# Megvii-CSG/MegReader

Measured on AMD Instinct MI355X. Metric: training images/sec, CRNN-CTC 32x128 crops, batch 256 per GPU, higher is better.
Workload: dtype bf16; 1 GPU; CRNN + 1D-CTC training step (BASELINE.json configs[1]): 32x128 crops, T=33, C=38, Adam; global_batch=256, per_gpu_batch=256, parallelism=dp1, launch=hipGraph replay

## Files before the change

### include/megreader_hip.h

```cpp
#ifndef MEGREADER_HIP_H
#define MEGREADER_HIP_H

#include <hip/hip_runtime_api.h>

#ifdef __cplusplus
extern "C" {
#endif

#define MR_ABI_VERSION 3
#define MR_DTYPE_F32 0
#define MR_DTYPE_BF16 1

const char* mr_last_error(void);
int mr_abi_version(void);
int mr_phase_timer(int on);
int mr_phase_read(int id, double* total_ms, double* total_work);
int mr_init(void);

typedef struct mr_tuning {
  int nt_variant;
  int nt_deep;
  int nt_big;
  int nt_p8;
  int nt_force_bm;
  int nt_force_bn;
  int gemm_skinny;
  int tn_big;
  int tn_buf;
  int tn_taps;
  int tn_taps_group;
  int tn_group;
  int tn_fin;
  int tn_taps_fin;
  int tn_taps_w8;
  int tn_model;
  int tn_splits;
  int bn_fused;
  int lstm_persist;
  int lstm_fwd_bn;
  int lstm_bwd_bn;
  int dcn_fused;
  int dcn_v1_bwd;
  int bn_onepass;
  int skinny_depth;
  int nt_big_min_k;
  int tn_taps_min_p;
  int tn_defer;
  int pool_fixed;
  int ctc_linear;
  int nt_wide8;
  int nt_ksplit;
  int nt_m32;
  int nt_m32_opt;
  int dcn_gcol;
  int dcn_col_fwd;
  int decode_persist;
  int reserved[3];
} mr_tuning;
int mr_tuning_get(mr_tuning* out);
int mr_tuning_defaults(mr_tuning* out);
int mr_tuning_set(const mr_tuning* in);

int mr_gemm_nt(int dtype, const void* A, long long lda, const void* B, int ldb, void* C, long long ldc,
               const float* bias, int relu, int M, int N, int K, hipStream_t stream);
int mr_set_tn_taps_workspace(void* ws, long long bytes);
int mr_tn_taps_would_run(int N, int H, int W, int Cin, int ldx, int Cout, int lddy, int R, int S, int sh, int sw,
                         int ph, int pw, int dh, int dw, int Ho, int Wo);
int mr_nt_tile_code(int M, int N);
int mr_nt_kernel_code(int dtype, int M, int N, int K, int cg);
int mr_gemm_tn(int dtype, const void* A, long long lda, const void* B, long long ldb, float* C, int ldc, int P,
               int NA, int NB, int row_perm_h, float* colsum, hipStream_t stream);
int mr_gemm_tn2(int dtype, const void* A, long long lda, const void* B, long long ldb, float* C, int ldc, int P,
                int NA, int NB, int row_perm_h, float* colsum, float* colsum2, hipStream_t stream);

int mr_tn_defer(int on);
int mr_tn_pending(void);
int mr_tn_discard(void);
int mr_tn_flush(hipStream_t stream);
int mr_tn_flush_beside(hipStream_t stream);

int mr_conv2d_fwd(int dtype, const void* x, const void* w_krsc, const float* bias, void* y, int relu, int Nimg,
                  int H, int W, int Cin, int ldx, int Cout, int ldy, int R, int S, int sh, int sw, int ph, int pw,
                  int dh, int dw, int Ho, int Wo, hipStream_t stream);
int mr_conv2d_fwd_pool_ok(int dtype, int Nimg, int H, int W, int Cin, int ldx, int Cout, int R, int S, int sh, int sw, int ph, int pw,
                          int dh, int dw, int Ho, int Wo, int pkh, int pkw, int psh, int psw, int pph, int ppw);
int mr_conv2d_fwd_pool(int dtype, const void* x, const void* w_krsc, const float* bias, void* y_pool, unsigned char* idx, int relu,
                       int Nimg, int H, int W, int Cin, int ldx, int Cout, int R, int S, int sh, int sw, int ph, int pw, int dh,
                       int dw, int Ho, int Wo, int pkh, int pkw, int psh, int psw, int pph, int ppw, int PHo, int PWo,
                       hipStream_t stream);
int mr_conv2d_fwd_stats(int dtype, const void* x, const void* w_krsc, const float* bias, void* y, double* bn_sums, int Nimg,
                        int H, int W, int Cin, int ldx, int Cout, int R, int S, int sh, int sw, int ph, int pw, int dh,
                        int dw, int Ho, int Wo, hipStream_t stream);
int mr_conv2d_dgrad(int dtype, const void* dy, const void* w_crsk, void* dx, int Nimg, int H, int W, int Cin,
                    int lddx, int Cout, int lddy, int R, int S, int sh, int sw, int ph, int pw, int dh, int dw,
                    int Ho, int Wo, hipStream_t stream);
int mr_conv2d_dgrad_add(int dtype, const void* dy, const void* w_crsk, void* dx, const void* addend, int Nimg, int H, int W,
                        int Cin, int lddx, int Cout, int lddy, int R, int S, int sh, int sw, int ph, int pw, int dh, int dw,
                        int Ho, int Wo, hipStream_t stream);
int mr_conv2d_dgrad_bnb(int dtype, const void* dy, const void* w_crsk, void* dx, const void* addend, const void* bn_x,
                        const void* bn_y, const float* bn_mean, const float* bn_rstd, double* bn_sums, int* produced,
                        int Nimg, int H, int W, int Cin, int lddx, int Cout, int lddy, int R, int S, int sh, int sw, int ph,
                        int pw, int dh, int dw, int Ho, int Wo, hipStream_t stream);
int mr_conv2d_wgrad(int dtype, const void* dy, const void* x, float* dw_krsc, float* dbias, int Nimg, int H, int W,
                    int Cin, int ldx, int Cout, int lddy, int R, int S, int sh, int sw, int ph, int pw, int dh,
                    int dw, int Ho, int Wo, hipStream_t stream);
int mr_conv2d_wgrad_tab(int dtype, const void* dy, const void* x, float* dw_krsc, float* dbias, int N, int H, int W,
                        int Cin, int ldx, int Cout, int lddy, int R, int S, int sh, int sw, int ph, int pw, int dh,
                        int dw, int Ho, int Wo, void* rowtab, int build, hipStream_t stream);

long long mr_db_loss_ws_bytes(void);
int mr_db_head_tail_fwd(int dtype, const void* xb, const void* xt, float* binary, float* thresh, float* tbinary, long long n,
                        float k, hipStream_t stream);
int mr_db_head_tail_bwd(int dtype, const float* binary, const float* thresh, const float* tbinary, const float* gb,
                        const float* gt, const float* gtb, void* dxb, void* dxt, long long n, float k, hipStream_t stream);
int mr_db_loss_fwd(const float* binary, const float* thresh, const float* tbinary, const float* gt, const float* mask,
                   const float* tmap, const float* tmask, float* negloss, void* ws, float* out, int N, long long HW,
                   float negative_ratio, float eps, float l1_scale, float bce_scale, hipStream_t stream);
int mr_db_loss_bwd(const float* binary, const float* thresh, const float* tbinary, const float* gt, const float* mask,
                   const float* tmap, const float* tmask, const float* out, const float* gloss, float* g_binary,
                   float* g_thresh, float* g_tbinary, int N, long long HW, float l1_scale, float bce_scale,
                   hipStream_t stream);

int mr_nchw_to_nhwc(int dtype, const float* src, void* dst, int N, int C, int H, int W, int Cpad,
                    hipStream_t stream);
int mr_nhwc_to_nchw(int dtype, const void* src, float* dst, int N, int C, int H, int W, int ld, hipStream_t stream);
int mr_cast(int src_dtype, const void* src, int dst_dtype, void* dst, long long n, hipStream_t stream);
int mr_relu_bwd(int dtype, const void* dy, const void* y, void* dx, long long n, hipStream_t stream);
int mr_add(int dtype, const void* a, const void* b, void* out, long long n, int relu, hipStream_t stream);
int mr_colsum(int dtype, const void* x, float* out, int P, int C, long long ld, int perm_h, hipStream_t stream);
int mr_permute_021(int dtype, const void* src, void* dst, int A, int B, int C, hipStream_t stream);
int mr_prep_conv_weight(int dtype, const float* src, long long sk, long long sc, long long sr, long long ss,
                        void* dst_krsc, void* dst_crsk, int K, int C, int R, int S, int Cpad, int ldk,
                        hipStream_t stream);
int mr_prep_matrix(int dtype, const float* src, int lds, void* dst_n, int ldn, void* dst_t, int ldt, int R, int C,
                   int perm_h, hipStream_t stream);
int mr_prep_bias(const float* a, const float* b, float* dst, int R, int perm_h, hipStream_t stream);

#define MR_PREP_CONV 0
#define MR_PREP_MATRIX 1
#define MR_PREP_BIAS 2
#define MR_PREP_STEM 3
typedef struct mr_prep_job {
  const float* src;
  const float* src2;
  void* dst_a;
  void* dst_b;
  long long s0, s1, s2, s3;
  int kind;
  int d0, d1, d2, d3;
  int pad, ld_b, perm_h;
  int block_start, reserved;
} mr_prep_job;
int mr_prep_batch(int dtype, const mr_prep_job* jobs_device, int njobs, long long total_blocks, float* tick,
                  hipStream_t stream);
int mr_sizeof_prep_job(void);

#define MR_MAX_SEGMENTS 8
int mr_accumulate_multi(int count, float* const* dst, const float* const* src, const long long* n,
                        hipStream_t stream);
int mr_zero_multi(int count, void* const* dst, const long long* bytes, hipStream_t stream);

int mr_opt_tick(float* hyper, hipStream_t stream);
int mr_adam_step(float* p, const float* g, float* m, float* v, long long n, float* hyper, hipStream_t stream);
int mr_sgd_step(float* p, const float* g, float* buf, long long n, float* hyper, hipStream_t stream);

long long mr_bn_scratch_doubles(int C);
int mr_bn_fwd_train(int dtype, const void* x, void* y, const float* gamma, const float* beta, float* running_mean,
                    float* running_var, float* save_mean, float* save_rstd, double* sums, const void* residual,
                    int relu, long long P, int C, float eps, float momentum, long long* num_batches_tracked,
                    hipStream_t stream);
int mr_bn_stats(int dtype, const void* x, double* sums, long long P, int C, hipStream_t stream);
int mr_bn_fwd_eval(int dtype, const void* x, void* y, const float* gamma, const float* beta,
                   const float* running_mean, const float* running_var, float* tmp_mean, float* tmp_rstd,
                   const void* residual, int relu, long long P, int C, float eps, hipStream_t stream);
int mr_bn_bwd(int dtype, const void* dy, const void* x, const void* y, const float* gamma, const float* save_mean,
              const float* save_rstd, double* sums, void* dx, void* dres, float* dgamma, float* dbeta, int flags,
              long long P, int C, hipStream_t stream);
int mr_maxpool_fwd(int dtype, const void* x, void* y, unsigned char* idx, int N, int H, int W, int C, int kh,
                   int kw, int sh, int sw, int ph, int pw, int Ho, int Wo, hipStream_t stream);
int mr_maxpool_bwd(int dtype, const void* dy, const unsigned char* idx, const void* relu_y, void* dx, int N, int H,
                   int W, int C, int kh, int kw, int sh, int sw, int ph, int pw, int Ho, int Wo,
                   hipStream_t stream);

long long mr_stem_bwd_workspace(int Cin);
int mr_stem_pack(const float* w, long long wsk, long long wsc, long long wsr, long long wss, void* wpack, int Cin,
                 hipStream_t stream);
int mr_stem_fwd(int dtype, const float* x, const float* w, long long wsk, long long wsc, long long wsr,
                long long wss, const void* wpack, const float* bias, void* y, unsigned char* code, int N, int Cin,
                int H, int W, hipStream_t stream);
int mr_stem_bwd(int dtype, const void* dy, const unsigned char* code, const float* x, float* workspace, float* dw,
                long long dsk, long long dsc, long long dsr, long long dss, float* dbias, int N, int Cin, int H,
                int W, hipStream_t stream);

int mr_lstm_fwd(int dtype, const void* xproj, const void* whh, void* out, float* cbuf, void* gates, int T, int N,
                int H, void* ws, long long ws_bytes, hipStream_t stream);
int mr_lstm_bwd(int dtype, const void* dout, const void* whhT, const float* cbuf, void* gates, float* dc, int T,
                int N, int H, void* ws, long long ws_bytes, hipStream_t stream);
long long mr_lstm_ws_bytes(int dtype, int T, int N, int H);
int mr_lstm_debug_buffer(float* p);

int mr_ctc_fwd(int dtype, const void* logits, int ldl, const void* targets, int targets_i64,
               const void* input_lengths, const void* target_lengths, int lengths_i64, int T, int N, int C, int S,
               int blank, int zero_infinity, float* log_probs, double* alpha, double* beta, double* nll,
               double* loss, double* log_probs_f64, hipStream_t stream);
int mr_ctc_bwd(int dtype, const float* log_probs, const double* alpha, const double* beta, const double* nll,
               const void* targets, int targets_i64, const void* input_lengths, const void* target_lengths,
               int lengths_i64, const double* grad_out, int T, int N, int C, int S, int blank, int zero_infinity,
               void* grad_logits, int ldg, hipStream_t stream);
int mr_ctc_wide(int C, int S);

int mr_ctc2d_fwd(int dtype, const void* log_probs, const long long* targets, const long long* input_lengths,
                 const long long* target_lengths, int T, int H, int N, int C, int S, int blank, float* nll,
                 float* alpha, hipStream_t stream);
int mr_ctc2d_bwd(int dtype, const float* grad_out, const void* log_probs, const long long* targets,
                 const long long* input_lengths, const long long* target_lengths, const float* nll,
                 const float* alpha, float* beta, void* grad, int T, int H, int N, int C, int S, int blank,
                 hipStream_t stream);

int mr_adaptive_avgpool_fwd(int dtype, const void* x, void* y, int N, int H, int W, int C, int OH, int OW,
                            hipStream_t stream);
int mr_adaptive_avgpool_bwd(int dtype, const void* dy, void* dx, int N, int H, int W, int C, int OH, int OW,
                            hipStream_t stream);
int mr_adaptive_avgpool_multi_fwd(int dtype, const void* x, void* const* ys, const int* oh, const int* ow, int nscales, int N,
                                  int H, int W, int C, hipStream_t stream);
int mr_adaptive_avgpool_multi_bwd(int dtype, void* const* dys, const int* oh, const int* ow, int nscales, void* dx, int N, int H,
                                  int W, int C, hipStream_t stream);
int mr_bilinear_fwd(int dtype, const void* x, void* y, int N, int H, int W, int C, int OH, int OW, int ldy, int coff,
                    int accumulate, hipStream_t stream);
int mr_bilinear_bwd(int dtype, const void* dy, void* dx, int N, int H, int W, int C, int OH, int OW, int lddy,
                    int coff, hipStream_t stream);
int mr_nearest_up_fwd(int dtype, const void* x, const void* add, void* y, int N, int H, int W, int C, int s, int ldy,
                      int coff, hipStream_t stream);
int mr_nearest_up_bwd(int dtype, const void* dy, void* dx, int N, int H, int W, int C, int s, int lddy, int coff,
                      hipStream_t stream);
int mr_deconv2x2_d2s(int dtype, const void* y2, int ld2, const float* bias, void* y, int N, int H, int W, int C,
                     hipStream_t stream);
int mr_deconv2x2_s2d(int dtype, const void* dy, void* dy2, int ld2, int N, int H, int W, int C, hipStream_t stream);
int mr_copy_channels(int dtype, const void* src, int lds, int soff, void* dst, int ldd, int doff, long long P, int C,
                     hipStream_t stream);
int mr_scatter_strided(int dtype, const void* dxs, void* dx, int N, int H, int W, int C, int sh, int sw, int Ho, int Wo,
                       hipStream_t stream);
int mr_scale_channels(int dtype, const void* x, const float* scale, void* y, int N, long long HW, int C,
                      hipStream_t stream);
int mr_ctc2d_head_fwd(int dtype, const void* mask_logits, int lda, const void* cls_logits, int ldz, float* lp,
                      float* mask_prob, float* cls_prob, int N, int H, int W, int C, float tiny, hipStream_t stream);
int mr_ctc2d_head_bwd(int dtype, const float* grad_lp, const float* mask_prob, const float* cls_prob, void* dmask,
                      int ldda, void* dcls, int lddz, int N, int H, int W, int C, float tiny, hipStream_t stream);

int mr_dcn2_im2col(int dtype, const void* x, const float* offset, long long off_bs, const float* mask,
                   long long msk_bs, void* col, int N, int H, int W, int C, int kh, int kw, int stride, int pad,
                   int dil, int Ho, int Wo, hipStream_t stream);
int mr_dcn2_coord_grad(int dtype, const void* gcol, const void* x, const float* offset, long long off_bs,
                       const float* mask, long long msk_bs, float* doffset, float* dmask, int N, int H, int W,
                       int C, int kh, int kw, int stride, int pad, int dil, int Ho, int Wo, hipStream_t stream);
int mr_dcn2_col2im(int dtype, const void* gcol, const float* offset, long long off_bs, const float* mask,
                   long long msk_bs, float* dx, int N, int H, int W, int C, int kh, int kw, int stride, int pad,
                   int dil, int Ho, int Wo, hipStream_t stream);

long long mr_dcn2_ws_bytes(int dtype, int N, int H, int W, int C, int Co, int kh, int kw, int Ho, int Wo, int backward);
int mr_dcn2_fwd(int dtype, const void* x, const void* w_n, const float* bias, const float* offset, long long off_bs,
                const float* mask, long long msk_bs, void* y, void* col_ws, int N, int H, int W, int C, int Co, int kh,
                int kw, int stride, int pad, int dil, int Ho, int Wo, hipStream_t stream);
int mr_dcn2_bwd(int dtype, const void* dy, const void* x, const void* w_t, const float* offset, long long off_bs,
                const float* mask, long long msk_bs, void* col_ws, float* dx32, float* doffset, float* dmask, float* dw,
                float* dbias, int N, int H, int W, int C, int Co, int kh, int kw, int stride, int pad, int dil, int Ho,
                int Wo, hipStream_t stream);
int mr_dcn2_fused(int dtype, int H, int W, int C, int Co, int kh, int kw);
int mr_dcn2_dx_direct(int dtype, int N, int H, int W, int C, int Co, int kh, int kw);
int mr_dcn2_bwd2(int dtype, const void* dy, const void* x, const void* w_t, const float* offset, long long off_bs,
                 const float* mask, long long msk_bs, void* col_ws, float* dx32, void* dx_t, int flags, float* doffset,
                 float* dmask, float* dw, float* dbias, int N, int H, int W, int C, int Co, int kh, int kw, int stride, int pad,
                 int dil, int Ho, int Wo, hipStream_t stream);
int mr_dcn2_col_saved(int dtype, int H, int W, int C, int Co, int kh, int kw);
int mr_dcn2_bwd3(int dtype, const void* dy, const void* x, const void* w_t, const float* offset, long long off_bs,
                 const float* mask, long long msk_bs, void* col_ws, float* dx32, void* dx_t, int flags, float* doffset,
                 float* dmask, float* dw, float* dbias, const void* col_saved, int N, int H, int W, int C, int Co, int kh, int kw,
                 int stride, int pad, int dil, int Ho, int Wo, hipStream_t stream);
int mr_dcn_unpack(int dtype, const void* raw, int ld, float* offset, float* mask, int N, int HW, int n_offset, int n_mask,
                  hipStream_t stream);
int mr_dcn_pack_grad(int dtype, const float* doffset, const float* dmask, const float* mask, void* graw, int ld, int N,
                     int HW, int n_offset, int n_mask, hipStream_t stream);

int mr_deform_psroi_fwd(const float* data, const float* rois, const float* trans, float* out, float* top_count, int B,
                        int C, int H, int W, int R, int channels_trans, int no_trans, float spatial_scale,
                        int output_dim, int group_size, int pooled_size, int part_size, int sample_per_part,
                        float trans_std, hipStream_t stream);
int mr_deform_psroi_bwd(const float* out_grad, const float* data, const float* rois, const float* trans,
                        const float* top_count, float* data_diff, float* trans_diff, int B, int C, int H, int W, int R,
                        int channels_trans, int no_trans, float spatial_scale, int output_dim, int group_size,
                        int pooled_size, int part_size, int sample_per_part, float trans_std, hipStream_t stream);

int mr_db_components(const float* prob, float thresh, int* labels, void* points, int* count, int cap, int N, int H, int W,
                     hipStream_t stream);
int mr_db_box_scores(const float* prob, const float* boxes, float* out, int B, int N, int H, int W, hipStream_t stream);

int mr_attn_step_fwd(int dtype, const void* hproj, const void* eproj, const float* v, const void* enc, float* weights,
                     void* context, int N, int T, int Hd, int Ep, hipStream_t stream);
int mr_attn_step_bwd(int dtype, const void* dcontext, const float* dweights, const void* hproj, const void* eproj,
                     const float* v, const void* enc, const float* weights, void* dhproj, float* deproj, float* dv,
                     float* denc, int N, int T, int Hd, int Ep, hipStream_t stream);
int mr_gru_gates_fwd(int dtype, const void* gi_a, const void* gi_b, const void* gh, const void* h, void* hnew,
                     float* save, int N, int H, hipStream_t stream);
int mr_gru_gates_bwd(int dtype, const void* dhnew, const float* save, const void* gh, const void* h, void* dgi,
                     void* dgh, void* dh, int N, int H, hipStream_t stream);
int mr_nll_step_fwd(int dtype, const void* logits, int ldl, const long long* target, long long tstride,
                    const float* mask, float* lp, float* loss, long long* argmax, int N, int C, int accumulate,
                    int softmax_out, hipStream_t stream);
int mr_nll_step_feed_fwd(int dtype, const void* logits, int ldl, const long long* target, long long tstride,
                         const float* mask, float* lp, float* loss, long long* argmax, const int* feed_flag,
                         long long* feed_idx, int N, int C, int accumulate, hipStream_t stream);
int mr_nll_step_bwd(int dtype, const float* gloss, const float* lp, const long long* target, long long tstride,
                    const float* mask, void* dlogits, int ldd, int N, int C, hipStream_t stream);
int mr_embed_rows_fwd(int dtype, const long long* idx, const float* table, void* out, int N, int V, int D, int ldo,
                      hipStream_t stream);
int mr_embed_rows_bwd(int dtype, const long long* idx, const void* dout, float* dtable, int N, int V, int D, int ldo,
                      hipStream_t stream);
int mr_attn_fwd2(int dtype, const void* hproj, long long ldh, const void* eproj, const float* v, const void* enc,
                 float* weights, void* context, int N, int Tn, int Hd, int Ep, hipStream_t stream);
int mr_attn_bwd2(int dtype, const void* dcontext, const float* dweights, long long ldw, const void* hproj, long long ldh,
                 const void* eproj, const float* v, const void* enc, const float* weights, void* dhproj, long long lddh,
                 float* deproj, float* dv, int N, int Tn, int Hd, int Ep, hipStream_t stream);
int mr_attn_denc(int dtype, const float* weights, const void* dcontext, void* denc, int S, int N, int Tn, int Ep,
                 hipStream_t stream);
int mr_gru_fwd2(int dtype, const void* gi_a, long long lda, const long long* idx, const void* gi_b, const void* gh,
                long long ldgh, const void* h, void* hnew, float* save, int N, int H, hipStream_t stream);
int mr_gru_bwd2(int dtype, const void* dh_a, const void* dh_b, const void* dh_c, const float* save, const void* gh,
                long long ldgh, const void* h, void* dgi, void* dgh, long long lddgh, void* dh_prev, int N, int H,
                hipStream_t stream);
int mr_rows_scatter_add(int dtype, const long long* idx, const void* rows, long long ldr, float* dtable, int R, int V,
                        int D, hipStream_t stream);

int mr_decode_persist_ok(int dtype, int N, int T, int H, int Ep);
long long mr_decode_persist_ws_bytes(int N);
int mr_decode_persist_fwd(const void* cat_w, const float* cat_b, const void* ic_w, long long ldic, const void* G, long long ldG,
                          long long* idx, const int* flags, const void* out_w, const float* out_b, int C, const void* eproj,
                          const void* enc, const float* v, void* H_all, void* HC_all, float* W_att, void* CTX_all,
                          float* SAVE_all, void* ws, long long ws_bytes, int S, int N, int T, int Ep, hipStream_t stream);
int mr_decode_persist_bwd_ok(int dtype, int N, int T, int H, int Ep);
long long mr_decode_persist_bwd_ws_bytes(int N);
int mr_decode_persist_bwd(const void* cat_wt, const void* ic_wt, long long ldict, const void* eproj, const void* enc,
                          const float* v, const void* H_all, const void* HC_all, const float* W_att, const float* SAVE_all,
                          const void* DHO_all, const float* ga, long long ldga, void* DGI_all, void* DHC_all, void* DCTX_all,
                          float* deproj, float* dv, void* denc, void* ws, long long ws_bytes, int S, int N, int T, int Ep,
                          hipStream_t stream);
int mr_decode_greedy_ok(int dtype, int N, int T, int H, int Ep, int C);
int mr_decode_greedy_fwd(const void* cat_w, const float* cat_b, const void* ic_w, long long ldic, const void* G, long long ldG,
                         const void* out_w, const float* out_b, int C, const void* eproj, const void* enc, const float* v,
                         const void* h0, int start_word, int* pred, long long ldp, void* H_all, void* ws, long long ws_bytes,
                         int S, int N, int T, int Ep, hipStream_t stream);
int mr_decode_greedy_trim(int* pred, long long ldp, int N, int S, int blank, hipStream_t stream);

int mr_gemm_gru_fwd(int dtype, const void* ctx, long long ldc, const void* w_ic, long long ldw, const void* G, long long ldG,
                    const long long* idx, const void* gh, long long ldgh, const void* h, void* hnew, float* save, int M, int H,
                    int K, hipStream_t stream);
int mr_gemm_gru_bwd(int dtype, const void* dhc, long long lda, const void* w_t, long long ldw, const void* dh_b,
                    const void* dh_c, const float* save, const void* gh, long long ldgh, const void* h, void* dgi, void* dgh,
                    long long lddgh, void* dh_prev, int M, int H, int K, hipStream_t stream);
int mr_out_nll_fwd(int dtype, const void* h, long long ldh, const void* W, long long ldw, const float* bias,
                   const long long* target, long long tstride, const float* mask, float* lp, float* loss, long long* argmax,
                   const int* feed_flag, long long* feed_idx, int N, int C, int K, int accumulate, hipStream_t stream);

int mr_softmax_nc1t(int dtype, const void* logits, int ldl, float* out, int T, int N, int C, hipStream_t stream);

int mr_ctc_greedy_decode(int dtype, const void* pred, long long sn, long long sc, long long st, int N, int C, int T,
                         int blank, int unknown, int* out, int* out_len, hipStream_t stream);
int mr_ctc2d_greedy_decode(const float* classify, long long cn, long long cc, long long ch, long long cw,
                           const float* mask, long long mn, long long mh, long long mw, int N, int C, int H, int W,
                           int blank, int unknown, int* out, int* out_len, hipStream_t stream);
int mr_seq_measure(const int* labels, int S, const int* preds, int S2, int N, int blank, int unknown, const int* fold,
                   int* acc, int* ed, int* label_len, double* score, hipStream_t stream);

int mr_sizeof_img_desc(void);
int mr_resize_normalize(const unsigned char* src, const void* desc, int N, int H, int W, double mean0, double mean1,
                        double mean2, float* dst, hipStream_t stream);
int mr_encode_labels(const int* codepoints, const long long* offsets, int N, int max_size, const int* table_cp,
                     const int* table_id, int ntab, int unknown, int* label, int* length, hipStream_t stream);

#ifdef __cplusplus
}
#endif
#endif
```

### megreader_amd/backbones/crnn.py

```python
import torch.nn as nn

from ..nn import Conv2d, BatchNorm2d, MaxPool2d, FusedReLU
from ..nn import functional as F


class _Stem(nn.Sequential):

    def forward(self, input):
        conv, pool = self[0][0], self[1]
        if F.stem_eligible(input, conv.weight, conv.stride, conv.padding, conv.dilation, _pair(pool.kernel_size),
                           _pair(pool.stride), _pair(pool.padding)):
            return F.stem_conv_relu_pool(input, conv.weight, conv.bias)
        return super().forward(input)


class _ConvReluPool(nn.Sequential):

    def forward(self, input):
        conv, pool = self[0][0], self[1]
        if F.conv_relu_pool_eligible(input, conv.weight, conv.stride, conv.padding, conv.dilation, _pair(pool.kernel_size),
                                     _pair(pool.stride), _pair(pool.padding)):
            return F.conv_relu_pool(input, conv.weight, conv.bias, conv.padding, _pair(pool.kernel_size), _pair(pool.stride),
                                    _pair(pool.padding))
        return super().forward(input)


def _pair(v):
    return tuple(v) if isinstance(v, (tuple, list)) else (v, v)


class CRNN(nn.Module):

    def __init__(self, imgH, nc, nclass, nh):
        super(CRNN, self).__init__()
        assert imgH % 16 == 0, 'imgH has to be a multiple of 16'

        self.kernels = [3, 3, 3, 3, 3, 3, 2]
        self.paddings = [1, 1, 1, 1, 1, 1, 0]
        self.strides = [1, 1, 1, 1, 1, 1, 1]
        self.channels = [64, 128, 256, 256, 512, 512, 512, nc]

        conv0 = _Stem(self._make_layer(0, pooled=True), MaxPool2d((2, 2), relu_input=True))
        conv1 = _ConvReluPool(self._make_layer(1, pooled=True), MaxPool2d((2, 2), relu_input=True))
        conv2 = self._make_layer(2, True)
        conv3 = _ConvReluPool(self._make_layer(3, pooled=True), MaxPool2d((2, 2), (2, 1), (0, 1), relu_input=True))
        conv4 = self._make_layer(4, True)
        conv5 = _ConvReluPool(self._make_layer(5, pooled=True), MaxPool2d((2, 2), (2, 1), (0, 1), relu_input=True))
        conv6 = self._make_layer(6, True)

        self.cnn = nn.Sequential(conv0, conv1, conv2, conv3, conv4, conv5, conv6)
        conv3[0][0].sole_consumer_of_bn = True
        conv5[0][0].sole_consumer_of_bn = True

    def _make_layer(self, i, batch_normalization=False, pooled=False):
        in_channel = self.channels[i - 1]
        out_channel = self.channels[i]
        layer = list()
        layer.append(Conv2d(in_channel, out_channel, self.kernels[i], self.strides[i], self.paddings[i],
                            fuse_relu=not batch_normalization,
                            relu_grad_downstream=pooled and not batch_normalization))
        if batch_normalization:
            layer.append(BatchNorm2d(out_channel))
        else:
            layer.append(FusedReLU())
        return nn.Sequential(*layer)

    def forward(self, input):
        return self.cnn(input)


def crnn_backbone(imgH=32, nc=3, nclass=37, nh=256):
    return CRNN(imgH, nc, nclass, nh)
```

### megreader_amd/csrc/norm_pool.hip

```cpp
#include "device.h"
#include "../../include/megreader_hip.h"


namespace mr {

template <typename T>
__global__ void bn_stats_kernel(const T* __restrict__ x, double* __restrict__ sums, int P, int C, long long ld,
                                int rows_per_block) {
  __shared__ float red[2][4][64];
  const int lane = threadIdx.x & 63, wave = threadIdx.x >> 6;
  const int c = blockIdx.x * 64 + lane;
  const int p0 = blockIdx.y * rows_per_block;
  const int p1 = min(P, p0 + rows_per_block);
  float s = 0.f, q = 0.f;
  if (c < C)
    for (int p = p0 + wave; p < p1; p += 4) {
      const float v = to_f32(x[(long long)p * ld + c]);
      s += v;
      q += v * v;
    }
  red[0][wave][lane] = s;
  red[1][wave][lane] = q;
  __syncthreads();
  if (wave == 0 && c < C) {
    const double ds = (double)red[0][0][lane] + red[0][1][lane] + red[0][2][lane] + red[0][3][lane];
    const double dq = (double)red[1][0][lane] + red[1][1][lane] + red[1][2][lane] + red[1][3][lane];
    atomicAdd(sums + c, ds);
    atomicAdd(sums + C + c, dq);
  }
}

template <typename T, int MODE>
__global__ __launch_bounds__(256) void bn_reduce_vec_kernel(const T* __restrict__ a, const T* __restrict__ xin,
                                                            const T* __restrict__ yin,
                                                            const float* __restrict__ mean,
                                                            const float* __restrict__ rstd,
                                                            double* __restrict__ sums, int relu, int P, int C,
                                                            int rows_per_block, int ncopy) {
  constexpr int VEC = VecOf<T>::N;
  __shared__ float red[2][256 * VEC];
  sums += (size_t)(blockIdx.x % ncopy) * 2 * C;
  const int cv = C / VEC;
  const int groups = 256 / cv;
  const int g = threadIdx.x / cv, v = threadIdx.x - g * cv;
  const int p0 = blockIdx.x * rows_per_block;
  const int p1 = min(P, p0 + rows_per_block);
  float s[VEC], q[VEC], mu[VEC], rs[VEC];
#pragma unroll
  for (int j = 0; j < VEC; ++j) {
    s[j] = q[j] = 0.f;
    mu[j] = 0.f;
    rs[j] = 1.f;
  }
  if (g < groups) {
    if (MODE == 1) {
#pragma unroll
      for (int j = 0; j < VEC; ++j) {
        mu[j] = mean[v * VEC + j];
        rs[j] = rstd[v * VEC + j];
      }
    }
#pragma unroll 4
    for (int p = p0 + g; p < p1; p += groups) {
      const long long i = (long long)p * cv + v;
      const uint4 av = ((const uint4*)a)[i];
      const T* pa = (const T*)&av;
      if (MODE == 0) {
#pragma unroll
        for (int j = 0; j < VEC; ++j) {
          const float x = to_f32(pa[j]);
          s[j] += x;
          q[j] += x * x;
        }
      } else {
        const uint4 xv = ((const uint4*)xin)[i];
        const T* px = (const T*)&xv;
        uint4 yv = make_uint4(0, 0, 0, 0);
        if (relu) yv = ((const uint4*)yin)[i];
        const T* py = (const T*)&yv;
#pragma unroll
        for (int j = 0; j < VEC; ++j) {
          float gd = to_f32(pa[j]);
          if (relu && !(to_f32(py[j]) > 0.f)) gd = 0.f;
          s[j] += gd;
          q[j] += gd * (to_f32(px[j]) - mu[j]) * rs[j];
        }
      }
    }
#pragma unroll
    for (int j = 0; j < VEC; ++j) {
      red[0][g * C + v * VEC + j] = s[j];
      red[1][g * C + v * VEC + j] = q[j];
    }
  }
  __syncthreads();
  for (int c = threadIdx.x; c < C; c += 256) {
    double ds = 0, dq = 0;
    for (int gg = 0; gg < groups; ++gg) {
      ds += (double)red[0][gg * C + c];
      dq += (double)red[1][gg * C + c];
    }
    atomicAdd(sums + c, ds);
    atomicAdd(sums + C + c, dq);
  }
}

__global__ void bn_finalize_kernel(const double* __restrict__ sums, int ncopy, int P, int C, float eps,
                                   float momentum, float* __restrict__ mean, float* __restrict__ rstd,
                                   float* __restrict__ running_mean, float* __restrict__ running_var,
                                   long long* __restrict__ num_batches_tracked) {
  const int c = blockIdx.x * blockDim.x + threadIdx.x;
  if (c == 0 && num_batches_tracked) *num_batches_tracked += 1;
  if (c >= C) return;
  double s1 = 0, s2 = 0;
  for (int k = 0; k < ncopy; ++k) {
    s1 += sums[(size_t)k * 2 * C + c];
    s2 += sums[(size_t)k * 2 * C + C + c];
  }
  const double m = s1 / P;
  double var = s2 / P - m * m;
  if (var < 0) var = 0;
  mean[c] = (float)m;
  rstd[c] = (float)(1.0 / sqrt(var + (double)eps));
  if (running_mean) {
    const double unb = P > 1 ? var * ((double)P / (P - 1)) : var;
    running_mean[c] = (1.f - momentum) * running_mean[c] + momentum * (float)m;
    running_var[c] = (1.f - momentum) * running_var[c] + momentum * (float)unb;
  }
}

template <typename T>
__global__ void bn_apply_kernel(const T* __restrict__ x, T* __restrict__ y, const float* __restrict__ mean,
                                const float* __restrict__ rstd, const float* __restrict__ gamma,
                                const float* __restrict__ beta, const T* __restrict__ residual, int relu,
                                long long P, int C) {
  constexpr int VEC = VecOf<T>::N;
  const int cv = C / VEC;
  const long long total = P * cv;
  for (long long i = blockIdx.x * (long long)blockDim.x + threadIdx.x; i < total;
       i += (long long)gridDim.x * blockDim.x) {
    const int c0 = (int)(i % cv) * VEC;
    uint4 a = ((const uint4*)x)[i];
    T* pa = (T*)&a;
    uint4 r = make_uint4(0, 0, 0, 0);
    if (residual) r = ((const uint4*)residual)[i];
    const T* pr = (const T*)&r;
#pragma unroll
    for (int j = 0; j < VEC; ++j) {
      const int c = c0 + j;
      float v = (to_f32(pa[j]) - mean[c]) * rstd[c] * gamma[c] + beta[c];
      if (residual) v += to_f32(pr[j]);
      if (relu) v = fmaxf(v, 0.f);
      pa[j] = from_f32<T>(v);
    }
    ((uint4*)y)[i] = a;
  }
}

template <typename T>
__global__ void bn_bwd_reduce_kernel(const T* __restrict__ dy, const T* __restrict__ x, const T* __restrict__ y,
                                     const float* __restrict__ mean, const float* __restrict__ rstd,
                                     double* __restrict__ sums, int relu, int P, int C, int rows_per_block) {
  __shared__ float red[2][4][64];
  const int lane = threadIdx.x & 63, wave = threadIdx.x >> 6;
  const int c = blockIdx.x * 64 + lane;
  const int p0 = blockIdx.y * rows_per_block;
  const int p1 = min(P, p0 + rows_per_block);
  float s = 0.f, q = 0.f;
  if (c < C) {
    const float mu = mean[c], rs = rstd[c];
    for (int p = p0 + wave; p < p1; p += 4) {
      const long long idx = (long long)p * C + c;
      float g = to_f32(dy[idx]);
      if (relu && !(to_f32(y[idx]) > 0.f)) g = 0.f;
      s += g;
      q += g * (to_f32(x[idx]) - mu) * rs;
    }
  }
  red[0][wave][lane] = s;
  red[1][wave][lane] = q;
  __syncthreads();
  if (wave == 0 && c < C) {
    const double ds = (double)red[0][0][lane] + red[0][1][lane] + red[0][2][lane] + red[0][3][lane];
    const double dq = (double)red[1][0][lane] + red[1][1][lane] + red[1][2][lane] + red[1][3][lane];
    atomicAdd(sums + c, ds);
    atomicAdd(sums + C + c, dq);
  }
}

__global__ void bn_bwd_finalize_kernel(const double* __restrict__ sums, int ncopy, long long P, int C,
                                       float* __restrict__ sbg, float* __restrict__ dgamma,
                                       float* __restrict__ dbeta, int accumulate) {
  const int c = blockIdx.x * blockDim.x + threadIdx.x;
  if (c >= C) return;
  double s1 = 0, s2 = 0;
  for (int k = 0; k < ncopy; ++k) {
    s1 += sums[(size_t)k * 2 * C + c];
    s2 += sums[(size_t)k * 2 * C + C + c];
  }
  const float invP = 1.f / (float)P;
  sbg[c] = (float)s1 * invP;
  sbg[C + c] = (float)s2 * invP;
  dbeta[c] = (accumulate ? dbeta[c] : 0.f) + (float)s1;
  dgamma[c] = (accumulate ? dgamma[c] : 0.f) + (float)s2;
}

template <typename T>
__global__ void bn_bwd_apply_kernel(const T* __restrict__ dy, const T* __restrict__ x, const T* __restrict__ y,
                                    const float* __restrict__ mean, const float* __restrict__ rstd,
                                    const float* __restrict__ gamma, const float* __restrict__ sbg,
                                    T* __restrict__ dx, T* __restrict__ dres, int relu, long long P, int C) {
  constexpr int VEC = VecOf<T>::N;
  const int cv = C / VEC;
  const long long total = P * cv;
  for (long long i = blockIdx.x * (long long)blockDim.x + threadIdx.x; i < total;
       i += (long long)gridDim.x * blockDim.x) {
    const int c0 = (int)(i % cv) * VEC;
    uint4 g = ((const uint4*)dy)[i];
    uint4 a = ((const uint4*)x)[i];
    uint4 o = make_uint4(0, 0, 0, 0);
    if (relu) o = ((const uint4*)y)[i];
    T* pg = (T*)&g;
    const T* pa = (const T*)&a;
    const T* po = (const T*)&o;
    uint4 out;
    T* pout = (T*)&out;
#pragma unroll
    for (int j = 0; j < VEC; ++j) {
      const int c = c0 + j;
      float gv = to_f32(pg[j]);
      if (relu && !(to_f32(po[j]) > 0.f)) gv = 0.f;
      pg[j] = from_f32<T>(gv);
      const float xh = (to_f32(pa[j]) - mean[c]) * rstd[c];
      const float sb = sbg[c], sg = sbg[C + c];
      pout[j] = from_f32<T>(gamma[c] * rstd[c] * (gv - sb - xh * sg));
    }
    ((uint4*)dx)[i] = out;
    if (dres) ((uint4*)dres)[i] = g;
  }
}

template <typename T>
__global__ __launch_bounds__(256) void bn_apply_fused_kernel(
    const T* __restrict__ x, T* __restrict__ y, const double* __restrict__ sums, int ncopy, float eps, float momentum,
    float* __restrict__ save_mean, float* __restrict__ save_rstd, float* __restrict__ running_mean,
    float* __restrict__ running_var, long long* __restrict__ num_batches_tracked, const float* __restrict__ gamma,
    const float* __restrict__ beta, const T* __restrict__ residual, int relu, int P, int C) {
  constexpr int VEC = VecOf<T>::N, LANES = 64 / VEC, ROWS = 256 / LANES;
  __shared__ float s_mean[64], s_rstd[64], s_gamma[64], s_beta[64];
  const int cbase = blockIdx.y * 64;
  if (threadIdx.x < 64) {
    const int c = cbase + threadIdx.x;
    double s1 = 0, s2 = 0;
    for (int k = 0; k < ncopy; ++k) {
      s1 += sums[(size_t)k * 2 * C + c];
      s2 += sums[(size_t)k * 2 * C + C + c];
    }
    const double m = s1 / P;
    double var = s2 / P - m * m;
    if (var < 0) var = 0;
    const float mf = (float)m, rf = (float)(1.0 / sqrt(var + (double)eps));
    s_mean[threadIdx.x] = mf;
    s_rstd[threadIdx.x] = rf;
    s_gamma[threadIdx.x] = gamma[c];
    s_beta[threadIdx.x] = beta[c];
    if (blockIdx.x == 0) {
      if (c == 0 && num_batches_tracked) *num_batches_tracked += 1;
      save_mean[c] = mf;
      save_rstd[c] = rf;
      if (running_mean) {
        const double unb = P > 1 ? var * ((double)P / (P - 1)) : var;
        running_mean[c] = (1.f - momentum) * running_mean[c] + momentum * (float)m;
        running_var[c] = (1.f - momentum) * running_var[c] + momentum * (float)unb;
      }
    }
  }
  __syncthreads();
  const int v = threadIdx.x % LANES, r0 = threadIdx.x / LANES;
  const int cv = C / VEC;
  float mu[VEC], rs[VEC], ga[VEC], be[VEC];
#pragma unroll
  for (int j = 0; j < VEC; ++j) {
    mu[j] = s_mean[v * VEC + j];
    rs[j] = s_rstd[v * VEC + j];
    ga[j] = s_gamma[v * VEC + j];
    be[j] = s_beta[v * VEC + j];
  }
  for (int p = blockIdx.x * ROWS + r0; p < P; p += gridDim.x * ROWS) {
    const long long i = (long long)p * cv + blockIdx.y * LANES + v;
    uint4 a = ((const uint4*)x)[i];
    T* pa = (T*)&a;
    uint4 r = make_uint4(0, 0, 0, 0);
    if (residual) r = ((const uint4*)residual)[i];
    const T* pr = (const T*)&r;
#pragma unroll
    for (int j = 0; j < VEC; ++j) {
      float val = (to_f32(pa[j]) - mu[j]) * rs[j] * ga[j] + be[j];
      if (residual) val += to_f32(pr[j]);
      if (relu) val = fmaxf(val, 0.f);
      pa[j] = from_f32<T>(val);
    }
    ((uint4*)y)[i] = a;
  }
}

template <typename T>
__global__ __launch_bounds__(256) void bn_bwd_apply_fused_kernel(
    const T* __restrict__ dy, const T* __restrict__ x, const T* __restrict__ y, const float* __restrict__ mean,
    const float* __restrict__ rstd, const float* __restrict__ gamma, const double* __restrict__ sums, int ncopy,
    float* __restrict__ dgamma, float* __restrict__ dbeta, int accumulate, T* __restrict__ dx, T* __restrict__ dres,
    int relu, int P, int C) {
  constexpr int VEC = VecOf<T>::N, LANES = 64 / VEC, ROWS = 256 / LANES;
  __shared__ float s_mean[64], s_k[64], s_rstd[64], s_sb[64], s_sg[64];
  const int cbase = blockIdx.y * 64;
  if (threadIdx.x < 64) {
    const int c = cbase + threadIdx.x;
    double s1 = 0, s2 = 0;
    for (int k = 0; k < ncopy; ++k) {
      s1 += sums[(size_t)k * 2 * C + c];
      s2 += sums[(size_t)k * 2 * C + C + c];
    }
    const float invP = 1.f / (float)P;
    s_sb[threadIdx.x] = (float)s1 * invP;
    s_sg[threadIdx.x] = (float)s2 * invP;
    s_mean[threadIdx.x] = mean[c];
    s_rstd[threadIdx.x] = rstd[c];
    s_k[threadIdx.x] = gamma[c] * rstd[c];
    if (blockIdx.x == 0) {
      dbeta[c] = (accumulate ? dbeta[c] : 0.f) + (float)s1;
      dgamma[c] = (accumulate ? dgamma[c] : 0.f) + (float)s2;
    }
  }
  __syncthreads();
  const int v = threadIdx.x % LANES, r0 = threadIdx.x / LANES;
  const int cv = C / VEC;
  float mu[VEC], rs[VEC], kk[VEC], sb[VEC], sg[VEC];
#pragma unroll
  for (int j = 0; j < VEC; ++j) {
    mu[j] = s_mean[v * VEC + j];
    rs[j] = s_rstd[v * VEC + j];
    kk[j] = s_k[v * VEC + j];
    sb[j] = s_sb[v * VEC + j];
    sg[j] = s_sg[v * VEC + j];
  }
  for (int p = blockIdx.x * ROWS + r0; p < P; p += gridDim.x * ROWS) {
    const long long i = (long long)p * cv + blockIdx.y * LANES + v;
    uint4 g = ((const uint4*)dy)[i];
    uint4 a = ((const uint4*)x)[i];
    uint4 o = make_uint4(0, 0, 0, 0);
    if (relu) o = ((const uint4*)y)[i];
    T* pg = (T*)&g;
    const T* pa = (const T*)&a;
    const T* po = (const T*)&o;
    uint4 out;
    T* pout = (T*)&out;
#pragma unroll
    for (int j = 0; j < VEC; ++j) {
      float gv = to_f32(pg[j]);
      if (relu && !(to_f32(po[j]) > 0.f)) gv = 0.f;
      pg[j] = from_f32<T>(gv);
      const float xh = (to_f32(pa[j]) - mu[j]) * rs[j];
      pout[j] = from_f32<T>(kk[j] * (gv - sb[j] - xh * sg[j]));
    }
    ((uint4*)dx)[i] = out;
    if (dres) ((uint4*)dres)[i] = g;
  }
}

template <typename T, int R>
__global__ __launch_bounds__(256) void bn_bwd_onepass_kernel(
    const T* __restrict__ dy, const T* __restrict__ x, const T* __restrict__ y, const float* __restrict__ mean,
    const float* __restrict__ rstd, const float* __restrict__ gamma, double* __restrict__ sums, int ncopy,
    unsigned* __restrict__ counters, float* __restrict__ dgamma, float* __restrict__ dbeta, int accumulate,
    T* __restrict__ dx, T* __restrict__ dres, int relu, int P, int C) {
  constexpr int VEC = VecOf<T>::N, LANES = 64 / VEC, ROWS = 256 / LANES;
  typedef __attribute__((ext_vector_type(4))) unsigned u32x4;
  __shared__ float red[2][ROWS][64];
  __shared__ float s_sb[64], s_sg[64];
  __shared__ int s_dead;
  const int tid = threadIdx.x;
  const int cbase = blockIdx.y * 64;
  const int v = tid % LANES, r0 = tid / LANES;
  const int cv = C / VEC;
  const int bytes = (int)((long long)P * C * (long long)sizeof(T));
  const __amdgpu_buffer_rsrc_t r_g = __builtin_amdgcn_make_buffer_rsrc((void*)dy, (short)0, bytes, 0x00020000);
  const __amdgpu_buffer_rsrc_t r_x = __builtin_amdgcn_make_buffer_rsrc((void*)x, (short)0, bytes, 0x00020000);
  const __amdgpu_buffer_rsrc_t r_y = __builtin_amdgcn_make_buffer_rsrc((void*)(relu ? y : x), (short)0, bytes, 0x00020000);
  const __amdgpu_buffer_rsrc_t r_dx = __builtin_amdgcn_make_buffer_rsrc((void*)dx, (short)0, bytes, 0x00020000);
  const __amdgpu_buffer_rsrc_t r_dr = __builtin_amdgcn_make_buffer_rsrc((void*)(dres ? dres : dx), (short)0, bytes, 0x00020000);
  const int voff = (r0 * cv + blockIdx.y * LANES + v) * 16;
  const int row_bytes = cv * 16;
  const int sbase = blockIdx.x * (ROWS * R) * row_bytes;
  float mu[VEC], rs[VEC];
#pragma unroll
  for (int j = 0; j < VEC; ++j) {
    mu[j] = mean[cbase + v * VEC + j];
    rs[j] = rstd[cbase + v * VEC + j];
  }
  u32x4 gq[R], xq[R];
#pragma unroll
  for (int k = 0; k < R; ++k) {
    gq[k] = __builtin_amdgcn_raw_buffer_load_b128(r_g, voff + sbase + k * ROWS * row_bytes, 0, 0);
    xq[k] = __builtin_amdgcn_raw_buffer_load_b128(r_x, voff + sbase + k * ROWS * row_bytes, 0, 0);
  }
  float s[VEC], q[VEC];
#pragma unroll
  for (int j = 0; j < VEC; ++j) s[j] = q[j] = 0.f;
  constexpr int RB = R < 4 ? R : 4;
#pragma unroll
  for (int kb = 0; kb < R; kb += RB) {
    u32x4 yq[RB];
    if (relu) {
#pragma unroll
      for (int u = 0; u < RB; ++u)
        yq[u] = __builtin_amdgcn_raw_buffer_load_b128(r_y, voff + sbase + (kb + u) * ROWS * row_bytes, 0, 0);
    }
#pragma unroll
    for (int u = 0; u < RB; ++u) {
      const int k = kb + u;
      T* pg = (T*)&gq[k];
      const T* pa = (const T*)&xq[k];
      const T* po = (const T*)&yq[u];
#pragma unroll
      for (int j = 0; j < VEC; ++j) {
        float gd = to_f32(pg[j]);
        if (relu && !(to_f32(po[j]) > 0.f)) {
          gd = 0.f;
          pg[j] = from_f32<T>(0.f);
        }
        s[j] += gd;
        q[j] += gd * (to_f32(pa[j]) - mu[j]) * rs[j];
      }
      __builtin_amdgcn_sched_barrier(0);
    }
  }
#pragma unroll
  for (int k = 0; k < R; ++k) asm volatile("" : "+v"(gq[k]), "+v"(xq[k]));
#pragma unroll
  for (int j = 0; j < VEC; ++j) {
    red[0][r0][v * VEC + j] = s[j];
    red[1][r0][v * VEC + j] = q[j];
  }
  if (tid == 0) s_dead = 0;
  __syncthreads();
  double* mine = sums + (size_t)(blockIdx.x % ncopy) * 2 * C;
  if (tid < 128) {
    const int c = tid & 63, which = tid >> 6;
    double d = 0;
#pragma unroll 8
    for (int r = 0; r < ROWS; ++r) d += (double)red[which][r][c];
    atomicAdd(mine + which * C + cbase + c, d);
  }
  asm volatile("s_waitcnt vmcnt(0)" ::: "memory");
  __syncthreads();
  unsigned* ctr = counters + blockIdx.y * 128;
  if (tid == 0) {
    __hip_atomic_fetch_add(ctr, 1u, __ATOMIC_RELAXED, __HIP_MEMORY_SCOPE_AGENT);
    const unsigned want = gridDim.x;
    const long long t0 = wall_clock64();
    unsigned spins = 0;
    while (__hip_atomic_load(ctr, __ATOMIC_RELAXED, __HIP_MEMORY_SCOPE_AGENT) < want) {
      __builtin_amdgcn_s_sleep(2);
      if ((++spins & 255u) == 0 && wall_clock64() - t0 > 200000000ll) {
        s_dead = 1;
        break;
      }
    }
  }
  __syncthreads();
  const bool dead = s_dead != 0;
  if (tid < 64) {
    const int c = cbase + tid;
    double s1 = 0, s2 = 0;
    for (int k = 0; k < ncopy; ++k) {
      s1 += __hip_atomic_load(sums + (size_t)k * 2 * C + c, __ATOMIC_RELAXED, __HIP_MEMORY_SCOPE_AGENT);
      s2 += __hip_atomic_load(sums + (size_t)k * 2 * C + C + c, __ATOMIC_RELAXED, __HIP_MEMORY_SCOPE_AGENT);
    }
    if (dead) s1 = s2 = (double)__builtin_nanf("");
    const float invP = 1.f / (float)P;
    s_sb[tid] = (float)s1 * invP;
    s_sg[tid] = (float)s2 * invP;
    if (blockIdx.x == 0) {
      dbeta[c] = (accumulate ? dbeta[c] : 0.f) + (float)s1;
      dgamma[c] = (accumulate ? dgamma[c] : 0.f) + (float)s2;
    }
  }
  __syncthreads();
  float sb[VEC], sg[VEC];
#pragma unroll
  for (int j = 0; j < VEC; ++j) {
    sb[j] = s_sb[v * VEC + j];
    sg[j] = s_sg[v * VEC + j];
  }
#pragma unroll
  for (int k = 0; k < R; ++k) {
    const T* pg = (const T*)&gq[k];
    const T* pa = (const T*)&xq[k];
    u32x4 out;
    T* pout = (T*)&out;
#pragma unroll
    for (int j = 0; j < VEC; ++j) {
      const float xh = (to_f32(pa[j]) - mu[j]) * rs[j];
      const float kj = gamma[cbase + v * VEC + j] * rs[j];
      pout[j] = from_f32<T>(kj * (to_f32(pg[j]) - sb[j] - xh * sg[j]));
    }
    __builtin_amdgcn_raw_buffer_store_b128(out, r_dx, voff + sbase + k * ROWS * row_bytes, 0, 0);
    if (dres) __builtin_amdgcn_raw_buffer_store_b128(gq[k], r_dr, voff + sbase + k * ROWS * row_bytes, 0, 0);
    __builtin_amdgcn_sched_barrier(0);
  }
}

__global__ void bn_eval_coeff_kernel(const float* __restrict__ rm, const float* __restrict__ rv, float eps,
                                     float* __restrict__ mean, float* __restrict__ rstd, int C) {
  const int c = blockIdx.x * blockDim.x + threadIdx.x;
  if (c >= C) return;
  mean[c] = rm[c];
  rstd[c] = 1.f / sqrtf(rv[c] + eps);
}

template <typename T>
__global__ void maxpool_fwd_kernel(const T* __restrict__ x, T* __restrict__ y, unsigned char* __restrict__ idx,
                                   int N, int H, int W, int C, int kh, int kw, int sh, int sw, int ph, int pw,
                                   int Ho, int Wo) {
  constexpr int VEC = VecOf<T>::N;
  const int cv = C / VEC;
  const long long total = (long long)N * Ho * Wo * cv;
  for (long long t = blockIdx.x * (long long)blockDim.x + threadIdx.x; t < total;
       t += (long long)gridDim.x * blockDim.x) {
    const int c = (int)(t % cv);
    long long q = t / cv;
    const int wo = (int)(q % Wo);
    q /= Wo;
    const int ho = (int)(q % Ho);
    const int n = (int)(q / Ho);
    float best[VEC];
    unsigned char bi[VEC];
#pragma unroll
    for (int j = 0; j < VEC; ++j) { best[j] = -INFINITY; bi[j] = 0; }
    bool first = true;
    for (int i = 0; i < kh; ++i) {
      const int h = ho * sh - ph + i;
      if ((unsigned)h >= (unsigned)H) continue;
      for (int jx = 0; jx < kw; ++jx) {
        const int w = wo * sw - pw + jx;
        if ((unsigned)w >= (unsigned)W) continue;
        const uint4 v = ((const uint4*)x)[(((long long)n * H + h) * W + w) * cv + c];
        const T* pv = (const T*)&v;
        const unsigned char code = (unsigned char)(i * kw + jx);
#pragma unroll
        for (int j = 0; j < VEC; ++j) {
          const float f = to_f32(pv[j]);
          if (first || f > best[j] || f != f) { best[j] = f; bi[j] = code; }
        }
        first = false;
      }
    }
    uint4 o;
    T* po = (T*)&o;
#pragma unroll
    for (int j = 0; j < VEC; ++j) po[j] = from_f32<T>(best[j]);
    ((uint4*)y)[t] = o;
    unsigned char* pi = idx + t * VEC;
#pragma unroll
    for (int j = 0; j < VEC; ++j) pi[j] = bi[j];
  }
}

template <typename T>
__global__ void maxpool_bwd_kernel(const T* __restrict__ dy, const unsigned char* __restrict__ idx,
                                   const T* __restrict__ relu_y, T* __restrict__ dx, int N, int H, int W, int C,
                                   int kh, int kw, int sh, int sw, int ph, int pw, int Ho, int Wo) {
  constexpr int VEC = VecOf<T>::N;
  const int cv = C / VEC;
  const long long total = (long long)N * H * W * cv;
  for (long long t = blockIdx.x * (long long)blockDim.x + threadIdx.x; t < total;
       t += (long long)gridDim.x * blockDim.x) {
    const int c = (int)(t % cv);
    long long q = t / cv;
    const int w = (int)(q % W);
    q /= W;
    const int h = (int)(q % H);
    const int n = (int)(q / H);
    float acc[VEC];
#pragma unroll
    for (int j = 0; j < VEC; ++j) acc[j] = 0.f;
    for (int i = 0; i < kh; ++i) {
      const int hn = h + ph - i;
      if (hn < 0) continue;
      const int ho = hn / sh;
      if (ho * sh != hn || ho >= Ho) continue;
      for (int jx = 0; jx < kw; ++jx) {
        const int wn = w + pw - jx;
        if (wn < 0) continue;
        const int wo = wn / sw;
        if (wo * sw != wn || wo >= Wo) continue;
        const long long o = (((long long)n * Ho + ho) * Wo + wo) * cv + c;
        const uint4 g = ((const uint4*)dy)[o];
        const T* pg = (const T*)&g;
        const unsigned char* pi = idx + o * VEC;
        const unsigned char code = (unsigned char)(i * kw + jx);
        if (relu_y) {
          const uint4 yv = ((const uint4*)relu_y)[o];
          const T* py = (const T*)&yv;
#pragma unroll
          for (int j = 0; j < VEC; ++j)
            if (pi[j] == code && to_f32(py[j]) > 0.f) acc[j] += to_f32(pg[j]);
        } else {
#pragma unroll
          for (int j = 0; j < VEC; ++j)
            if (pi[j] == code) acc[j] += to_f32(pg[j]);
        }
      }
    }
    uint4 out;
    T* po = (T*)&out;
#pragma unroll
    for (int j = 0; j < VEC; ++j) po[j] = from_f32<T>(acc[j]);
    ((uint4*)dx)[t] = out;
  }
}

template <typename T, int KH, int KW, int SH, int SW>
__global__ __launch_bounds__(256) void maxpool_bwd_fixed_kernel(const T* __restrict__ dy,
                                                                 const unsigned char* __restrict__ idx,
                                                                 const T* __restrict__ relu_y, T* __restrict__ dx,
                                                                 int H, int W, int cv, int ph, int pw, int Ho,
                                                                 int Wo) {
  constexpr int VEC = VecOf<T>::N;
  const int t = blockIdx.x * 256 + threadIdx.x;
  if (t >= W * cv) return;
  const int w = t / cv, c = t - w * cv;
  const int n = blockIdx.y / H, h = blockIdx.y - n * H;
  float acc[VEC];
#pragma unroll
  for (int j = 0; j < VEC; ++j) acc[j] = 0.f;
#pragma unroll
  for (int i = 0; i < KH; ++i) {
    const int hn = h + ph - i;
    const int ho = hn / SH;
    if (hn < 0 || ho * SH != hn || ho >= Ho) continue;
#pragma unroll
    for (int jx = 0; jx < KW; ++jx) {
      const int wn = w + pw - jx;
      const int wo = wn / SW;
      if (wn < 0 || wo * SW != wn || wo >= Wo) continue;
      const long long o = (((long long)n * Ho + ho) * Wo + wo) * cv + c;
      const uint4 g = ((const uint4*)dy)[o];
      const T* pg = (const T*)&g;
      unsigned char code[8];
      if (VEC == 8) *(uint2*)code = *(const uint2*)(idx + o * VEC);
      else *(unsigned*)code = *(const unsigned*)(idx + o * VEC);
      const unsigned char want = (unsigned char)(i * KW + jx);
      if (relu_y) {
        const uint4 yv = ((const uint4*)relu_y)[o];
        const T* py = (const T*)&yv;
#pragma unroll
        for (int j = 0; j < VEC; ++j)
          if (code[j] == want && to_f32(py[j]) > 0.f) acc[j] += to_f32(pg[j]);
      } else {
#pragma unroll
        for (int j = 0; j < VEC; ++j)
          if (code[j] == want) acc[j] += to_f32(pg[j]);
      }
    }
  }
  uint4 out;
  T* po = (T*)&out;
#pragma unroll
  for (int j = 0; j < VEC; ++j) po[j] = from_f32<T>(acc[j]);
  ((uint4*)dx)[((long long)blockIdx.y * W + w) * cv + c] = out;
}

template <typename T, int KH, int KW, int SH, int SW>
__global__ __launch_bounds__(256) void maxpool_fwd_fixed_kernel(const T* __restrict__ x, T* __restrict__ y,
                                                                 unsigned char* __restrict__ idx, int H, int W, int cv,
                                                                 int ph, int pw, int Ho, int Wo) {
  constexpr int VEC = VecOf<T>::N;
  const int t = blockIdx.x * 256 + threadIdx.x;
  if (t >= Wo * cv) return;
  const int wo = t / cv, c = t - wo * cv;
  const int n = blockIdx.y / Ho, ho = blockIdx.y - n * Ho;
  uint4 v[KH * KW];
  bool ok[KH * KW];
#pragma unroll
  for (int i = 0; i < KH; ++i)
#pragma unroll
    for (int jx = 0; jx < KW; ++jx) {
      const int h = ho * SH - ph + i, w = wo * SW - pw + jx;
      ok[i * KW + jx] = (unsigned)h < (unsigned)H && (unsigned)w < (unsigned)W;
      v[i * KW + jx] = ok[i * KW + jx] ? ((const uint4*)x)[(((long long)n * H + h) * W + w) * cv + c] : make_uint4(0, 0, 0, 0);
    }
  float best[VEC];
  unsigned char bi[8] = {0, 0, 0, 0, 0, 0, 0, 0};
#pragma unroll
  for (int j = 0; j < VEC; ++j) best[j] = -INFINITY;
  bool first = true;
#pragma unroll
  for (int k = 0; k < KH * KW; ++k) {
    if (!ok[k]) continue;
    const T* pv = (const T*)&v[k];
#pragma unroll
    for (int j = 0; j < VEC; ++j) {
      const float f = to_f32(pv[j]);
      if (first || f > best[j] || f != f) { best[j] = f; bi[j] = (unsigned char)k; }
    }
    first = false;
  }
  uint4 o;
  T* po = (T*)&o;
#pragma unroll
  for (int j = 0; j < VEC; ++j) po[j] = from_f32<T>(best[j]);
  const long long q = (((long long)n * Ho + ho) * Wo + wo) * cv + c;
  ((uint4*)y)[q] = o;
  if (VEC == 8) *(uint2*)(idx + q * VEC) = *(const uint2*)bi;
  else *(unsigned*)(idx + q * VEC) = *(const unsigned*)bi;
}

template <typename T>
__global__ __launch_bounds__(256) void maxpool_bwd_2x2s2_kernel(const T* __restrict__ dy,
                                                                 const unsigned char* __restrict__ idx,
                                                                 const T* __restrict__ relu_y, T* __restrict__ dx, int H,
                                                                 int W, int cv, int Ho, int Wo) {
  constexpr int VEC = VecOf<T>::N;
  const int t = blockIdx.x * 256 + threadIdx.x;
  if (t >= Wo * cv) return;
  const int wo = t / cv, c = t - wo * cv;
  const int n = blockIdx.y / Ho, ho = blockIdx.y - n * Ho;
  const long long o = (((long long)n * Ho + ho) * Wo + wo) * cv + c;
  const uint4 g = ((const uint4*)dy)[o];
  unsigned char code[8];
  if (VEC == 8) *(uint2*)code = *(const uint2*)(idx + o * VEC);
  else *(unsigned*)code = *(const unsigned*)(idx + o * VEC);
  const T* pg = (const T*)&g;
  T gm[VEC];
  if (relu_y) {
    const uint4 yv = ((const uint4*)relu_y)[o];
    const T* py = (const T*)&yv;
#pragma unroll
    for (int j = 0; j < VEC; ++j) gm[j] = to_f32(py[j]) > 0.f ? pg[j] : from_f32<T>(0.f);
  } else {
#pragma unroll
    for (int j = 0; j < VEC; ++j) gm[j] = pg[j];
  }
#pragma unroll
  for (int k = 0; k < 4; ++k) {
    uint4 out;
    T* po = (T*)&out;
#pragma unroll
    for (int j = 0; j < VEC; ++j) po[j] = code[j] == k ? from_f32<T>(0.f + to_f32(gm[j])) : from_f32<T>(0.f);
    ((uint4*)dx)[(((long long)n * H + 2 * ho + (k >> 1)) * W + 2 * wo + (k & 1)) * cv + c] = out;
  }
}

template <typename T>
__global__ __launch_bounds__(256) void maxpool_bwd_2x2s21_kernel(const T* __restrict__ dy,
                                                                  const unsigned char* __restrict__ idx,
                                                                  const T* __restrict__ relu_y, T* __restrict__ dx, int H,
                                                                  int W, int cv, int pw, int Ho, int Wo) {
  constexpr int VEC = VecOf<T>::N;
  const int t = blockIdx.x * 256 + threadIdx.x;
  if (t >= W * cv) return;
  const int w = t / cv, c = t - w * cv;
  const int n = blockIdx.y / Ho, ho = blockIdx.y - n * Ho;
  float acc[2][VEC];
#pragma unroll
  for (int j = 0; j < VEC; ++j) acc[0][j] = acc[1][j] = 0.f;
#pragma unroll
  for (int jx = 0; jx < 2; ++jx) {
    const int wo = w + pw - jx;
    if (wo < 0 || wo >= Wo) continue;
    const long long o = (((long long)n * Ho + ho) * Wo + wo) * cv + c;
    const uint4 g = ((const uint4*)dy)[o];
    const T* pg = (const T*)&g;
    unsigned char code[8];
    if (VEC == 8) *(uint2*)code = *(const uint2*)(idx + o * VEC);
    else *(unsigned*)code = *(const unsigned*)(idx + o * VEC);
    uint4 yv = make_uint4(0, 0, 0, 0);
    if (relu_y) yv = ((const uint4*)relu_y)[o];
    const T* py = (const T*)&yv;
#pragma unroll
    for (int j = 0; j < VEC; ++j) {
      const bool live = !relu_y || to_f32(py[j]) > 0.f;
      if (live && code[j] == jx) acc[0][j] += to_f32(pg[j]);
      if (live && code[j] == 2 + jx) acc[1][j] += to_f32(pg[j]);
    }
  }
#pragma unroll
  for (int i = 0; i < 2; ++i) {
    uint4 out;
    T* po = (T*)&out;
#pragma unroll
    for (int j = 0; j < VEC; ++j) po[j] = from_f32<T>(acc[i][j]);
    ((uint4*)dx)[(((long long)n * H + 2 * ho + i) * W + w) * cv + c] = out;
  }
}

#define g_bn_fused MR_TUNE(bn_fused)
static inline int bn_fused_grid_x(long long P, int rows, int slabs) {
  static int groups = 0, capw = 0;
  if (!groups) {
    const char* e = getenv("MEGREADER_BN_GROUPS");
    groups = e && atoi(e) > 0 ? atoi(e) : 4;
    const char* c = getenv("MEGREADER_BN_CAP");
    capw = c && atoi(c) > 0 ? atoi(c) : 4096;
  }
  long long gx = (P + (long long)rows * groups - 1) / ((long long)rows * groups);
  const long long cap = capw / slabs > 1 ? capw / slabs : 1;
  if (gx > cap) gx = cap;
  if (gx < 1) gx = 1;
  return (int)gx;
}

#define g_bn_onepass MR_TUNE(bn_onepass)
static int bn_onepass_cap() {
  static int cap = -1;
  if (cap >= 0) return cap;
  const int cus = device_cus();
  int occ_b = 0, occ_f = 0;
  if (cus == 0 ||
      hipOccupancyMaxActiveBlocksPerMultiprocessor(&occ_b, bn_bwd_onepass_kernel<bf16_t, 8>, 256, 0) != hipSuccess ||
      hipOccupancyMaxActiveBlocksPerMultiprocessor(&occ_f, bn_bwd_onepass_kernel<float, 8>, 256, 0) != hipSuccess) {
    (void)hipGetLastError();
    return cap = 0;
  }
  int occ = occ_b < occ_f ? occ_b : occ_f;
  if (occ > 4) occ = 4;
  cap = occ >= 1 ? cus * occ - cus / 4 : 0;
  return cap;
}

static inline int grid_for(long long n, int block, int max_blocks = 16384) {
  long long b = (n + block - 1) / block;
  if (b > max_blocks) b = max_blocks;
  if (b < 1) b = 1;
  return (int)b;
}

}

using namespace mr;

#define DISPATCH_T(dtype, ...)                                   \
  if ((dtype) == MR_F32) { typedef float T; __VA_ARGS__; }       \
  else if ((dtype) == MR_BF16) { typedef bf16_t T; __VA_ARGS__; } \
  else { mr::set_error("bad dtype %d", (dtype)); return MR_ERR_DTYPE; }

static int split_rows(int P, int C, int& rpb) {
  const int colg = cdiv(C, 64);
  int splits = 2048 / colg;
  if (splits < 1) splits = 1;
  if (splits > cdiv(P, 32)) splits = cdiv(P, 32);
  rpb = cdiv(P, splits);
  return cdiv(P, rpb);
}

static int split_rows_vec(int P, int cv, int& rpb) {
  const int groups = 256 / cv;
  int splits = 512;
  if (splits > cdiv(P, 4 * groups)) splits = cdiv(P, 4 * groups);
  if (splits < 1) splits = 1;
  rpb = cdiv(P, splits);
  return cdiv(P, rpb);
}

extern "C" {

long long mr_bn_scratch_doubles(int C) { return 2ll * C * MR_BN_COPIES + C; }


int mr_bn_stats(int dtype, const void* x, double* sums, long long P, int C, hipStream_t stream) {
  const int vec = dtype == MR_F32 ? 4 : 8;
  MR_CHECK_ARG(C % vec == 0, "mr_bn_stats: C (%d) must be a multiple of %d", C, vec);
  MR_CHECK_ARG(P > 0 && P < (1ll << 31), "mr_bn_stats: bad P");
  int rpb;
  if (C / vec <= 256 && 256 % (C / vec) == 0) {
    const int splits = split_rows_vec((int)P, C / vec, rpb);
    DISPATCH_T(dtype, hipLaunchKernelGGL((bn_reduce_vec_kernel<T, 0>), dim3(splits), dim3(256), 0, stream,
                                         (const T*)x, (const T*)nullptr, (const T*)nullptr, (const float*)nullptr,
                                         (const float*)nullptr, sums, 0, (int)P, C, rpb, MR_BN_COPIES));
  } else {
    const int splits = split_rows((int)P, C, rpb);
    DISPATCH_T(dtype, hipLaunchKernelGGL((bn_stats_kernel<T>), dim3(cdiv(C, 64), splits), dim3(256), 0, stream,
                                         (const T*)x, sums, (int)P, C, (long long)C, rpb));
  }
  MR_CHECK_LAUNCH();
  return MR_OK;
}

int mr_bn_fwd_train(int dtype, const void* x, void* y, const float* gamma, const float* beta, float* running_mean,
                    float* running_var, float* save_mean, float* save_rstd, double* sums, const void* residual,
                    int relu, long long P, int C, float eps, float momentum, long long* num_batches_tracked,
                    hipStream_t stream) {
  const int vec = dtype == MR_F32 ? 4 : 8;
  MR_CHECK_ARG(C % vec == 0, "mr_bn_fwd_train: C (%d) must be a multiple of %d", C, vec);
  MR_CHECK_ARG(P > 0 && P < (1ll << 31), "mr_bn_fwd_train: bad P");
  const int presum_zero = (relu >> 2) & 1;
  const int have_stats = (relu >> 3) & 1;
  relu &= 1;
  if (!presum_zero && !have_stats) (void)hipMemsetAsync(sums, 0, sizeof(double) * 2 * C * MR_BN_COPIES, stream);
  int rpb, ncopy = 1;
  if (have_stats) {
    ncopy = MR_BN_COPIES;
  } else if (C / vec <= 256 && 256 % (C / vec) == 0) {
    const int splits = split_rows_vec((int)P, C / vec, rpb);
    ncopy = MR_BN_COPIES;
    DISPATCH_T(dtype, hipLaunchKernelGGL((bn_reduce_vec_kernel<T, 0>), dim3(splits), dim3(256), 0, stream,
                                         (const T*)x, (const T*)nullptr, (const T*)nullptr, (const float*)nullptr,
                                         (const float*)nullptr, sums, 0, (int)P, C, rpb, ncopy));
  } else {
    const int splits = split_rows((int)P, C, rpb);
    DISPATCH_T(dtype, hipLaunchKernelGGL((bn_stats_kernel<T>), dim3(cdiv(C, 64), splits), dim3(256), 0, stream,
                                         (const T*)x, sums, (int)P, C, (long long)C, rpb));
  }
  if (g_bn_fused && C % 64 == 0) {
    const int rows = 256 / (64 / vec);
    const dim3 grid(bn_fused_grid_x(P, rows, C / 64), C / 64);
    DISPATCH_T(dtype, hipLaunchKernelGGL((bn_apply_fused_kernel<T>), grid, dim3(256), 0, stream, (const T*)x, (T*)y,
                                         (const double*)sums, ncopy, eps, momentum, save_mean, save_rstd, running_mean,
                                         running_var, num_batches_tracked, gamma, beta, (const T*)residual, relu,
                                         (int)P, C));
    MR_CHECK_LAUNCH();
    return MR_OK;
  }
  hipLaunchKernelGGL(bn_finalize_kernel, dim3(cdiv(C, 256)), dim3(256), 0, stream, (const double*)sums, ncopy, (int)P, C,
                     eps, momentum, save_mean, save_rstd, running_mean, running_var, num_batches_tracked);
  DISPATCH_T(dtype, hipLaunchKernelGGL((bn_apply_kernel<T>), dim3(grid_for(P * (C / vec), 256)), dim3(256), 0,
                                       stream, (const T*)x, (T*)y, (const float*)save_mean, (const float*)save_rstd,
                                       gamma, beta, (const T*)residual, relu, P, C));
  MR_CHECK_LAUNCH();
  return MR_OK;
}

int mr_bn_fwd_eval(int dtype, const void* x, void* y, const float* gamma, const float* beta,
                   const float* running_mean, const float* running_var, float* tmp_mean, float* tmp_rstd,
                   const void* residual, int relu, long long P, int C, float eps, hipStream_t stream) {
  const int vec = dtype == MR_F32 ? 4 : 8;
  MR_CHECK_ARG(C % vec == 0, "mr_bn_fwd_eval: C (%d) must be a multiple of %d", C, vec);
  hipLaunchKernelGGL(bn_eval_coeff_kernel, dim3(cdiv(C, 256)), dim3(256), 0, stream, running_mean, running_var, eps,
                     tmp_mean, tmp_rstd, C);
  DISPATCH_T(dtype, hipLaunchKernelGGL((bn_apply_kernel<T>), dim3(grid_for(P * (C / vec), 256)), dim3(256), 0,
                                       stream, (const T*)x, (T*)y, (const float*)tmp_mean, (const float*)tmp_rstd,
                                       gamma, beta, (const T*)residual, relu, P, C));
  MR_CHECK_LAUNCH();
  return MR_OK;
}

int mr_bn_bwd(int dtype, const void* dy, const void* x, const void* y, const float* gamma, const float* save_mean,
              const float* save_rstd, double* sums, void* dx, void* dres, float* dgamma, float* dbeta, int flags,
              long long P, int C, hipStream_t stream) {
  const int relu = flags & 1, accumulate = (flags >> 1) & 1, presum_zero = (flags >> 2) & 1;
  const int have_stats = (flags >> 3) & 1;
  const int vec = dtype == MR_F32 ? 4 : 8;
  MR_CHECK_ARG(C % vec == 0, "mr_bn_bwd: C (%d) must be a multiple of %d", C, vec);
  MR_CHECK_ARG(P > 0 && P < (1ll << 31), "mr_bn_bwd: bad P");
  if (!have_stats && g_bn_onepass && C % 64 == 0) {
    const int rows = 256 / (64 / vec);
    const int slabs = C / 64;
    const int cap = bn_onepass_cap();
    const long long g8 = (P + rows * 8 - 1) / (rows * 8), g2 = (P + rows * 2 - 1) / (rows * 2);
    const int rr = (g8 * slabs >= 256 || g2 * slabs > cap) ? 8 : 2;
    const long long gx = rr == 8 ? g8 : g2;
    if (cap > 0 && gx * slabs <= cap && P * C * (dtype == MR_F32 ? 4 : 2) < (1ll << 31)) {
      unsigned* counters = (unsigned*)(sums + (size_t)2 * C * MR_BN_COPIES);
      if (!presum_zero) (void)hipMemsetAsync(sums, 0, sizeof(double) * (2 * C * MR_BN_COPIES + C), stream);
      const dim3 grid((unsigned)gx, slabs);
      if (rr == 8) {
        DISPATCH_T(dtype, hipLaunchKernelGGL((bn_bwd_onepass_kernel<T, 8>), grid, dim3(256), 0, stream, (const T*)dy,
                                             (const T*)x, (const T*)y, save_mean, save_rstd, gamma, sums, MR_BN_COPIES,
                                             counters, dgamma, dbeta, accumulate, (T*)dx, (T*)dres, relu, (int)P, C));
      } else {
        DISPATCH_T(dtype, hipLaunchKernelGGL((bn_bwd_onepass_kernel<T, 2>), grid, dim3(256), 0, stream, (const T*)dy,
                                             (const T*)x, (const T*)y, save_mean, save_rstd, gamma, sums, MR_BN_COPIES,
                                             counters, dgamma, dbeta, accumulate, (T*)dx, (T*)dres, relu, (int)P, C));
      }
      MR_CHECK_LAUNCH();
      return MR_OK;
    }
  }
  if (!presum_zero && !have_stats) (void)hipMemsetAsync(sums, 0, sizeof(double) * 2 * C * MR_BN_COPIES, stream);
  int rpb, ncopy = 1;
  if (have_stats) {
    ncopy = MR_BN_COPIES;
  } else if (C / vec <= 256 && 256 % (C / vec) == 0) {
    const int splits = split_rows_vec((int)P, C / vec, rpb);
    ncopy = MR_BN_COPIES;
    DISPATCH_T(dtype, hipLaunchKernelGGL((bn_reduce_vec_kernel<T, 1>), dim3(splits), dim3(256), 0, stream,
                                         (const T*)dy, (const T*)x, (const T*)y, save_mean, save_rstd, sums, relu,
                                         (int)P, C, rpb, ncopy));
  } else {
    const int splits = split_rows((int)P, C, rpb);
    DISPATCH_T(dtype, hipLaunchKernelGGL((bn_bwd_reduce_kernel<T>), dim3(cdiv(C, 64), splits), dim3(256), 0, stream,
                                         (const T*)dy, (const T*)x, (const T*)y, save_mean, save_rstd, sums, relu,
                                         (int)P, C, rpb));
  }
  if (g_bn_fused && C % 64 == 0) {
    const int rows = 256 / (64 / vec);
    const dim3 grid(bn_fused_grid_x(P, rows, C / 64), C / 64);
    DISPATCH_T(dtype, hipLaunchKernelGGL((bn_bwd_apply_fused_kernel<T>), grid, dim3(256), 0, stream, (const T*)dy,
                                         (const T*)x, (const T*)y, save_mean, save_rstd, gamma, (const double*)sums, ncopy,
                                         dgamma, dbeta, accumulate, (T*)dx, (T*)dres, relu, (int)P, C));
    MR_CHECK_LAUNCH();
    return MR_OK;
  }
  float* sbg = (float*)(sums + (size_t)2 * C * MR_BN_COPIES);
  hipLaunchKernelGGL(bn_bwd_finalize_kernel, dim3(cdiv(C, 256)), dim3(256), 0, stream, (const double*)sums, ncopy, P, C,
                     sbg, dgamma, dbeta, accumulate);
  DISPATCH_T(dtype, hipLaunchKernelGGL((bn_bwd_apply_kernel<T>), dim3(grid_for(P * (C / vec), 256)), dim3(256), 0,
                                       stream, (const T*)dy, (const T*)x, (const T*)y, save_mean, save_rstd, gamma,
                                       (const float*)sbg, (T*)dx, (T*)dres, relu, P, C));
  MR_CHECK_LAUNCH();
  return MR_OK;
}

int mr_maxpool_fwd(int dtype, const void* x, void* y, unsigned char* idx, int N, int H, int W, int C, int kh,
                   int kw, int sh, int sw, int ph, int pw, int Ho, int Wo, hipStream_t stream) {
  const int vec = dtype == MR_F32 ? 4 : 8;
  MR_CHECK_ARG(C % vec == 0, "mr_maxpool_fwd: C (%d) must be a multiple of %d", C, vec);
  MR_CHECK_ARG(kh * kw <= 255, "mr_maxpool_fwd: window too large");
  MR_CHECK_ARG(Ho == (H + 2 * ph - kh) / sh + 1 && Wo == (W + 2 * pw - kw) / sw + 1,
               "mr_maxpool_fwd: output size inconsistent");
  const long long total = (long long)N * Ho * Wo * (C / vec);
  if ((long long)N * Ho <= 65535 && MR_TUNE(pool_fixed)) {
    const int cv = C / vec;
    const dim3 grid(cdiv(Wo * cv, 256), N * Ho);
#define MR_POOL_FIXED(KH_, KW_, SH_, SW_)                                                                            \
  if (kh == KH_ && kw == KW_ && sh == SH_ && sw == SW_) {                                                            \
    DISPATCH_T(dtype, hipLaunchKernelGGL((maxpool_fwd_fixed_kernel<T, KH_, KW_, SH_, SW_>), grid, dim3(256), 0,       \
                                         stream, (const T*)x, (T*)y, idx, H, W, cv, ph, pw, Ho, Wo));                \
    MR_CHECK_LAUNCH();                                                                                               \
    return MR_OK;                                                                                                    \
  }
    MR_POOL_FIXED(2, 2, 2, 2) MR_POOL_FIXED(2, 2, 2, 1) MR_POOL_FIXED(3, 3, 2, 2)
#undef MR_POOL_FIXED
  }
  DISPATCH_T(dtype, hipLaunchKernelGGL((maxpool_fwd_kernel<T>), dim3(grid_for(total, 256)), dim3(256), 0, stream,
                                       (const T*)x, (T*)y, idx, N, H, W, C, kh, kw, sh, sw, ph, pw, Ho, Wo));
  MR_CHECK_LAUNCH();
  return MR_OK;
}

int mr_maxpool_bwd(int dtype, const void* dy, const unsigned char* idx, const void* relu_y, void* dx, int N, int H,
                   int W, int C, int kh, int kw, int sh, int sw, int ph, int pw, int Ho, int Wo,
                   hipStream_t stream) {
  const int vec = dtype == MR_F32 ? 4 : 8;
  MR_CHECK_ARG(C % vec == 0, "mr_maxpool_bwd: C (%d) must be a multiple of %d", C, vec);
  const long long total = (long long)N * H * W * (C / vec);
  const int cv = C / vec;
  if (kh == 2 && kw == 2 && sh == 2 && sw == 2 && ph == 0 && pw == 0 && H == 2 * Ho && W == 2 * Wo &&
      (long long)N * Ho <= 65535 && MR_TUNE(pool_fixed)) {
    DISPATCH_T(dtype, hipLaunchKernelGGL((maxpool_bwd_2x2s2_kernel<T>), dim3(cdiv(Wo * cv, 256), N * Ho), dim3(256), 0, stream,
                                         (const T*)dy, idx, (const T*)relu_y, (T*)dx, H, W, cv, Ho, Wo));
    MR_CHECK_LAUNCH();
    return MR_OK;
  }
  if (kh == 2 && kw == 2 && sh == 2 && sw == 1 && ph == 0 && (pw == 0 || pw == 1) && H == 2 * Ho && Wo == W + 2 * pw - 1 &&
      (long long)N * Ho <= 65535 && MR_TUNE(pool_fixed)) {
    DISPATCH_T(dtype, hipLaunchKernelGGL((maxpool_bwd_2x2s21_kernel<T>), dim3(cdiv(W * cv, 256), N * Ho), dim3(256), 0, stream,
                                         (const T*)dy, idx, (const T*)relu_y, (T*)dx, H, W, cv, pw, Ho, Wo));
    MR_CHECK_LAUNCH();
    return MR_OK;
  }
  if ((long long)N * H <= 65535) {
    const dim3 grid(cdiv(W * cv, 256), N * H);
#define MR_POOL_FIXED(KH_, KW_, SH_, SW_)                                                                            \
  if (kh == KH_ && kw == KW_ && sh == SH_ && sw == SW_) {                                                            \
    DISPATCH_T(dtype, hipLaunchKernelGGL((maxpool_bwd_fixed_kernel<T, KH_, KW_, SH_, SW_>), grid, dim3(256), 0,       \
                                         stream, (const T*)dy, idx, (const T*)relu_y, (T*)dx, H, W, cv, ph, pw, Ho,  \
                                         Wo));                                                                       \
    MR_CHECK_LAUNCH();                                                                                               \
    return MR_OK;                                                                                                    \
  }
    MR_POOL_FIXED(2, 2, 2, 2) MR_POOL_FIXED(2, 2, 2, 1) MR_POOL_FIXED(3, 3, 2, 2)
#undef MR_POOL_FIXED
  }
  DISPATCH_T(dtype, hipLaunchKernelGGL((maxpool_bwd_kernel<T>), dim3(grid_for(total, 256)), dim3(256), 0, stream,
                                       (const T*)dy, idx, (const T*)relu_y, (T*)dx, N, H, W, C, kh, kw, sh, sw, ph,
                                       pw, Ho, Wo));
  MR_CHECK_LAUNCH();
  return MR_OK;
}

}
```

### megreader_amd/nn/functional.py

```python
import ctypes
import os

import torch
from torch.autograd import Function

from .. import get_compute_dtype
from . import prep
from .._lib import call, dtype_code, load, ptr, require_cuda, vec_of

_ESIZE = {torch.float32: 4, torch.bfloat16: 2}


def _ceil_to(x, m):
    return (x + m - 1) // m * m


def grad_sink(param, physical_shape=None):
    sink = getattr(param, "_mr_grad_sink", None)
    if sink is None or sink.dtype != torch.float32 or not sink.is_cuda:
        return None
    if param.grad is None or param.grad.data_ptr() != sink.data_ptr():
        return None
    if physical_shape == "strided":
        return sink
    if physical_shape is not None:
        if len(physical_shape) == 4:
            phys = sink.permute(0, 2, 3, 1)
            if tuple(phys.shape) != tuple(physical_shape) or not phys.is_contiguous():
                return None
        elif tuple(sink.shape) != tuple(physical_shape) or not sink.is_contiguous():
            return None
    elif not sink.is_contiguous():
        return None
    return sink


def notify_grad_ready(param):
    for hook in getattr(param, "_mr_grad_ready_hooks", ()):
        hook(param)


class ZeroArena(object):
    SIZE = 1 << 24
    arenas = {}

    def __init__(self, device):
        self.buf = torch.zeros((ZeroArena.SIZE,), dtype=torch.float64, device=device)
        self.offset = 0

    @staticmethod
    def take(device, n):
        a = ZeroArena.arenas.get(device)
        if a is None:
            a = ZeroArena.arenas[device] = ZeroArena(device)
        n = (n + 31) // 32 * 32
        if a.offset + n > ZeroArena.SIZE:
            return None
        out = a.buf[a.offset:a.offset + n]
        a.offset += n
        return out

    @staticmethod
    def reset(device):
        a = ZeroArena.arenas.get(device)
        if a is not None and a.offset:
            a.buf[:a.offset].zero_()
            a.offset = 0

    @staticmethod
    def rewind(device):
        a = ZeroArena.arenas.get(device)
        if a is None or not a.offset:
            return None
        used = a.offset
        a.offset = 0
        return a.buf.data_ptr(), used * 8


def zero_segments(segments):
    for i in range(0, len(segments), 8):
        chunk = segments[i:i + 8]
        n = len(chunk)
        call("mr_zero_multi", n, (ctypes.c_void_p * n)(*[p for p, _ in chunk]), (ctypes.c_longlong * n)(*[b for _, b in chunk]))


def accumulate_multi(pairs):
    for i in range(0, len(pairs), 8):
        chunk = pairs[i:i + 8]
        n = len(chunk)
        dst = (ctypes.c_void_p * n)(*[d.data_ptr() for d, _ in chunk])
        src = (ctypes.c_void_p * n)(*[s.data_ptr() for _, s in chunk])
        cnt = (ctypes.c_longlong * n)(*[s.numel() for _, s in chunk])
        call("mr_accumulate_multi", n, dst, src, cnt)


class _TnDefer(object):
    enabled = os.environ.get("MEGREADER_TN_DEFER", "1") != "0"
    MAX = 12
    keep = []
    notify = []
    queued = False
    task = -1
    mark = 0

    @staticmethod
    def _task_id():
        fn = getattr(torch._C, "_current_graph_task_id", None)
        return fn() if fn is not None else -1

    @staticmethod
    def abort():
        lib = load()
        lib.mr_tn_defer(0)
        lib.mr_tn_discard()
        del _TnDefer.keep[:]
        del _TnDefer.notify[:]
        _TnDefer.queued = False
        _TnDefer.task = -1

    @staticmethod
    def begin():
        if not _TnDefer.enabled:
            return False
        tid = _TnDefer._task_id()
        if _TnDefer.queued and tid != _TnDefer.task:
            _TnDefer.abort()
        if not _TnDefer.queued:
            try:
                torch.autograd.Variable._execution_engine.queue_callback(_TnDefer.flush)
            except RuntimeError:
                return False
            _TnDefer.queued = True
            _TnDefer.task = tid
        lib = load()
        _TnDefer.mark = lib.mr_tn_pending()
        lib.mr_tn_defer(1)
        return True

    @staticmethod
    def record(launch, tensors, params):
        try:
            launch()
        except BaseException:
            _TnDefer.abort()
            raise
        return _TnDefer.end(tensors, params)

    @staticmethod
    def end(tensors, params):
        lib = load()
        lib.mr_tn_defer(0)
        n = lib.mr_tn_pending()
        if n == _TnDefer.mark:
            return False
        _TnDefer.keep.extend(t for t in tensors if t is not None)
        _TnDefer.notify.extend(params)
        if n >= _TnDefer.MAX:
            _TnDefer.flush(final=False)
        return True

    @staticmethod
    def flush(final=True):
        if load().mr_tn_pending():
            call("mr_tn_flush")
        ready, _TnDefer.notify = _TnDefer.notify, []
        del _TnDefer.keep[:]
        if final:
            _TnDefer.queued = False
            _TnDefer.task = -1
        for p in ready:
            notify_grad_ready(p)


def _wgrad(launch, may_defer, keep, params, immediate=None):
    if may_defer and _TnDefer.begin():
        return _TnDefer.record(launch, keep, params)
    (immediate or launch)()
    return False


def discard_deferred_wgrads():
    _TnDefer.abort()


def flush_deferred_wgrads():
    _TnDefer.flush(final=False)


def to_internal(x, dtype):
    N, C, H, W = x.shape
    v = vec_of(dtype)
    xp = x.permute(0, 2, 3, 1)
    if x.dtype == dtype and xp.is_contiguous() and C % v == 0:
        return xp
    if xp.is_contiguous() and C % v == 0 and x.dtype in _ESIZE:
        out = torch.empty(xp.shape, dtype=dtype, device=x.device)
        call("mr_cast", dtype_code(x.dtype), ptr(xp), dtype_code(dtype), ptr(out), out.numel())
        return out
    xs = x.detach()
    if xs.dtype != torch.float32:
        xs = xs.float()
    xs = xs.contiguous()
    Cp = _ceil_to(C, v)
    out = torch.empty((N, H, W, Cp), dtype=dtype, device=x.device)
    call("mr_nchw_to_nhwc", dtype_code(dtype), ptr(xs), ptr(out), N, C, H, W, Cp)
    return out


def _grad_internal(g, dtype):
    gp = g.permute(0, 2, 3, 1)
    if g.dtype == dtype and gp.is_contiguous():
        return gp
    return to_internal(g, dtype)


def mark_zero_padded(t):
    t._mr_zero_padded = True
    return t


def _zero_padded_base(gy, shape, dtype):
    base = gy._base
    if base is None or not getattr(base, "_mr_zero_padded", False):
        return None
    N, Ho, Wo, Kp = shape
    if base.dtype != dtype or tuple(base.shape) != (N, Ho, Wo, Kp) or not base.is_contiguous():
        return None
    if gy.data_ptr() != base.data_ptr() or gy.shape[0] != N or tuple(gy.shape[2:]) != (Ho, Wo) or \
            tuple(gy.stride()) != (Ho * Wo * Kp, 1, Wo * Kp, Kp):
        return None
    return base


def _zero_padded_rows(gy, M, Nout, Np, dtype):
    base = gy._base
    if base is None or not getattr(base, "_mr_zero_padded", False):
        return None
    if base.dtype != dtype or not base.is_contiguous() or base.shape[-1] != Np or base.numel() != M * Np:
        return None
    if gy.data_ptr() != base.data_ptr() or gy.shape[-1] != Nout or tuple(gy.shape[:-1]) != tuple(base.shape[:-1]) or \
            tuple(gy.stride()) != tuple(base.stride()):
        return None
    return base.view(M, Np)


def _conv_out(size, k, s, p, d):
    return (size + 2 * p - d * (k - 1) - 1) // s + 1


_ROWTABS = {}


def _wgrad_rowtab(device, geom, vector_k=True):
    key = (device, geom, bool(vector_k))
    tab = _ROWTABS.get(key)
    if tab is not None:
        return tab, 0
    n, ho, wo = geom[0], geom[-2], geom[-1]
    if len(_ROWTABS) > 256:
        _ROWTABS.clear()
    tab = _ROWTABS[key] = torch.empty((n * ho * wo, 2), dtype=torch.int32, device=device)
    return tab, 1


from .._lib import ensure_tn_workspace as ensure_tn_taps_workspace


def set_tn_taps(mode):
    from .._lib import load
    old = load().mr_set_tn_taps(int(mode))
    _ROWTABS.clear()
    return old


def _conv_operands(weight, bias, dtype, Cp, Kp, need_dx):
    K, C, R, S = weight.shape
    dev = weight.device

    def build(old):
        if old is None:
            alloc = torch.zeros if Kp != K else torch.empty
            w_krsc = alloc((Kp, R, S, Cp), dtype=dtype, device=dev)
            w_crsk = alloc((C, R, S, Kp), dtype=dtype, device=dev) if need_dx else None
            bias_p = torch.zeros((Kp,), dtype=torch.float32, device=dev) if (bias is not None and Kp != K) else None
        else:
            w_krsc, w_crsk, bias_p = old
        jobs = [prep.conv_job(ptr(weight), weight.stride(), ptr(w_krsc), ptr(w_crsk), K, C, R, S, Cp, Kp)]
        if bias_p is not None:
            jobs.append(prep.bias_job(ptr(bias), 0, ptr(bias_p), K, 0))
        return (w_krsc, w_crsk, bias_p), jobs

    w_krsc, w_crsk, bias_p = prep.prepared((weight, bias), ("conv", Cp, Kp, bool(need_dx)), build, dtype)
    return w_krsc, w_crsk, (bias_p if bias_p is not None else bias)


class Conv2dFn(Function):
    @staticmethod
    def forward(ctx, x, weight, bias, stride, padding, dilation, relu, relu_grad_downstream=False, bn_sums=None,
                fork=False, bnb_link=None):
        require_cuda(x, weight, bias)
        ctx.bnb_link = bnb_link
        dtype = get_compute_dtype()
        dt = dtype_code(dtype)
        v = vec_of(dtype)
        xi = to_internal(x, dtype)
        N, H, W, Cp = xi.shape
        K, C, R, S = weight.shape
        if C > Cp or weight.dtype != torch.float32:
            raise RuntimeError("conv weight %s does not match input channels %d" % (tuple(weight.shape), Cp))
        Kp = _ceil_to(K, v)
        sh, sw = stride
        ph, pw = padding
        dh, dw = dilation
        Ho, Wo = _conv_out(H, R, sh, ph, dh), _conv_out(W, S, sw, pw, dw)
        need_dx = ctx.needs_input_grad[0]
        if need_dx and Cp != C:
            raise RuntimeError("input gradient requested for a channel-padded convolution input")
        w_krsc, w_crsk, bias_k = _conv_operands(weight, bias, dtype, Cp, Kp, need_dx)
        y = torch.empty((N, Ho, Wo, Kp), dtype=dtype, device=x.device)
        if bn_sums is not None and not relu and Kp == K:
            call("mr_conv2d_fwd_stats", dt, ptr(xi), ptr(w_krsc), ptr(bias_k), ptr(y), ptr(bn_sums), N, H, W, Cp, Cp, Kp,
                 R, S, sh, sw, ph, pw, dh, dw, Ho, Wo)
        else:
            call("mr_conv2d_fwd", dt, ptr(xi), ptr(w_krsc), ptr(bias_k), ptr(y), int(relu), N, H, W, Cp, Cp, Kp, Kp, R,
                 S, sh, sw, ph, pw, dh, dw, Ho, Wo)
        ctx.save_for_backward(xi, w_crsk, y if (relu and not relu_grad_downstream) else None)
        ctx.params = (weight, bias)
        ctx.geom = (N, H, W, Cp, C, K, Kp, R, S, sh, sw, ph, pw, dh, dw, Ho, Wo)
        ctx.relu = relu and not relu_grad_downstream
        ctx.has_bias = bias is not None
        ctx.dtype = dtype
        out = (y if Kp == K else y[..., :K]).permute(0, 3, 1, 2)
        if fork:
            return out, x.view_as(x)
        return out

    @staticmethod
    def backward(ctx, gy, g_fork=None):
        xi, w_crsk, y = ctx.saved_tensors
        N, H, W, Cp, C, K, Kp, R, S, sh, sw, ph, pw, dh, dw, Ho, Wo = ctx.geom
        dtype = ctx.dtype
        dt = dtype_code(dtype)
        if Kp == K:
            g = _grad_internal(gy, dtype)
        else:
            g = _zero_padded_base(gy, (N, Ho, Wo, Kp), dtype)
            if g is None:
                g = torch.zeros((N, Ho, Wo, Kp), dtype=dtype, device=gy.device)
                g[..., :K] = gy.permute(0, 2, 3, 1)
        if ctx.relu:
            gm = torch.empty_like(g)
            call("mr_relu_bwd", dt, ptr(g), ptr(y), ptr(gm), g.numel())
            g = gm
        dx = dwt = db = None
        if ctx.needs_input_grad[0]:
            dxi = torch.empty((N, H, W, C), dtype=dtype, device=g.device)
            ga = None
            if g_fork is not None:
                ga = _grad_internal(g_fork, dtype)
                if tuple(ga.shape) != (N, H, W, C) or not ga.is_contiguous():
                    ga = ga.contiguous()
            link = ctx.bnb_link
            fused_bnb = False
            if link is not None and link.xi is not None and link.dtype == dtype and tuple(link.xi.shape) == (N, H, W, C) and \
                    BNB_EPILOGUE:
                sums = ZeroArena.take(g.device, load().mr_bn_scratch_doubles(C))
                if sums is not None:
                    produced = ctypes.c_int(0)
                    call("mr_conv2d_dgrad_bnb", dt, ptr(g), ptr(w_crsk), ptr(dxi), ptr(ga), ptr(link.xi), ptr(link.y),
                         ptr(link.mean), ptr(link.rstd), ptr(sums), ctypes.byref(produced), N, H, W, C, C, Kp, Kp, R, S, sh,
                         sw, ph, pw, dh, dw, Ho, Wo)
                    fused_bnb = True
                    if produced.value:
                        link.sums, link.grad_ptr = sums, dxi.data_ptr()
            if fused_bnb:
                pass
            elif ga is not None:
                call("mr_conv2d_dgrad_add", dt, ptr(g), ptr(w_crsk), ptr(dxi), ptr(ga), N, H, W, C, C, Kp, Kp, R, S, sh, sw,
                     ph, pw, dh, dw, Ho, Wo)
            elif POINTWISE_STRIDED_DGRAD and R == 1 and S == 1 and (sh > 1 or sw > 1) and ph == 0 and pw == 0:
                dxs = torch.empty((N, Ho, Wo, C), dtype=dtype, device=g.device)
                call("mr_conv2d_dgrad", dt, ptr(g), ptr(w_crsk), ptr(dxs), N, Ho, Wo, C, C, Kp, Kp, 1, 1, 1, 1, 0, 0, 1, 1, Ho,
                     Wo)
                call("mr_scatter_strided", dt, ptr(dxs), ptr(dxi), N, H, W, C, sh, sw, Ho, Wo)
            else:
                call("mr_conv2d_dgrad", dt, ptr(g), ptr(w_crsk), ptr(dxi), N, H, W, C, C, Kp, Kp, R, S, sh, sw, ph, pw,
                     dh, dw, Ho, Wo)
            dx = dxi.permute(0, 3, 1, 2)
        elif g_fork is not None:
            raise RuntimeError("conv2d_fork: the forked input received a gradient but the convolution input needs none")
        weight_p, bias_p = ctx.params
        want_db = ctx.has_bias and ctx.needs_input_grad[2]
        w_sink = grad_sink(weight_p, (K, R, S, C)) if (ctx.needs_input_grad[1] and Cp == C) else None
        b_sink = grad_sink(bias_p, (K,)) if want_db else None
        Kw = K if (w_sink is not None or b_sink is not None) else Kp
        if want_db:
            db = b_sink if b_sink is not None else torch.zeros((Kp,), dtype=torch.float32, device=g.device)
        if ctx.needs_input_grad[1]:
            gw = w_sink if w_sink is not None else torch.zeros((Kp, R, S, Cp), dtype=torch.float32, device=g.device)
            tab, build = (None, 0)
            if dtype == torch.bfloat16 and R * S <= 32:
                tab, build = _wgrad_rowtab(g.device, (N, H, W, Cp, R, S, sh, sw, ph, pw, dh, dw, Ho, Wo), Kw % 8 == 0)
            def wgrad_launch():
                call("mr_conv2d_wgrad_tab", dt, ptr(g), ptr(xi), ptr(gw), ptr(db) if want_db else 0, N, H, W, Cp, Cp, Kw,
                     Kp, R, S, sh, sw, ph, pw, dh, dw, Ho, Wo, ptr(tab), build)
            if _wgrad(wgrad_launch, w_sink is not None and (not want_db or b_sink is not None), (g, xi, tab),
                      [weight_p] + ([bias_p] if want_db else [])):
                return dx, None, None, None, None, None, None, None, None, None, None
            if w_sink is not None:
                dwt = None
                notify_grad_ready(weight_p)
            else:
                if Cp != C or Kp != K:
                    gw = gw[:K, :, :, :C]
                dwt = gw.permute(0, 3, 1, 2)
        elif want_db:
            call("mr_colsum", dt, ptr(g), ptr(db), N * Ho * Wo, Kw, Kp, 0)
        if want_db:
            if b_sink is not None:
                db = None
                notify_grad_ready(bias_p)
            elif Kp != K:
                db = db[:K]
        return dx, dwt, db, None, None, None, None, None, None, None, None


POINTWISE_STRIDED_DGRAD = os.environ.get("MEGREADER_POINTWISE_STRIDED_DGRAD", "1") != "0"

BNB_EPILOGUE = os.environ.get("MEGREADER_BNB_EPILOGUE", "0") == "1"


_DIST_GUARD = {"done": False}


def _no_resident_grids_beside_collectives():
    if _DIST_GUARD["done"]:
        return
    import torch.distributed as dist
    if dist.is_available() and dist.is_initialized():
        from ..runtime import no_resident_grid_kernels_beside_collectives
        no_resident_grid_kernels_beside_collectives(dist.get_world_size())
        _DIST_GUARD["done"] = True


class BnBwdLink(object):
    __slots__ = ("xi", "y", "mean", "rstd", "dtype", "sums", "grad_ptr")

    def __init__(self):
        self.xi = self.y = self.mean = self.rstd = self.dtype = self.sums = self.grad_ptr = None


class BnStatsHandoff(object):
    __slots__ = ("sums", "data_ptr", "dtype", "P", "C")

    def __init__(self, sums, data_ptr, dtype, P, C):
        self.sums, self.data_ptr, self.dtype, self.P, self.C = sums, data_ptr, dtype, P, C


def conv2d(x, weight, bias=None, stride=(1, 1), padding=(0, 0), dilation=(1, 1), relu=False,
           relu_grad_downstream=False, bn_stats=False, fork=False, sole_consumer_of_bn=False):
    sums = None
    if bn_stats and not relu and x.is_cuda:
        K = weight.shape[0]
        if K % vec_of(get_compute_dtype()) == 0:
            sums = ZeroArena.take(x.device, load().mr_bn_scratch_doubles(K))
    want_fork = bool(fork)
    fork = want_fork and x.requires_grad and torch.is_grad_enabled()
    link = getattr(x, "_mr_bnb_link", None) if (sole_consumer_of_bn and x.requires_grad and torch.is_grad_enabled()) else None
    y = Conv2dFn.apply(x, weight, bias, tuple(stride), tuple(padding), tuple(dilation), bool(relu),
                       bool(relu_grad_downstream), sums, fork, link)
    x_fork = x
    if fork:
        y, x_fork = y
    if sums is not None:
        y._mr_bn_sums = BnStatsHandoff(sums, y.data_ptr(), get_compute_dtype(), y.shape[0] * y.shape[2] * y.shape[3],
                                       y.shape[1])
    return (y, x_fork) if want_fork else y


class BatchNormFn(Function):
    @staticmethod
    def forward(ctx, x, gamma, beta, running_mean, running_var, training, momentum, eps, relu, residual,
                num_batches_tracked=None, pre=None, link=None):
        require_cuda(x, gamma, beta)
        dtype = get_compute_dtype()
        dt = dtype_code(dtype)
        xi = to_internal(x, dtype)
        N, H, W, C = xi.shape
        if C != gamma.numel():
            raise RuntimeError("BatchNorm2d: channel mismatch (%d vs %d)" % (C, gamma.numel()))
        P = N * H * W
        ri = to_internal(residual, dtype) if residual is not None else None
        y = torch.empty_like(xi)
        mean = torch.empty((C,), dtype=torch.float32, device=x.device)
        rstd = torch.empty((C,), dtype=torch.float32, device=x.device)
        if training:
            nsum = load().mr_bn_scratch_doubles(C)
            have = (pre is not None and pre.data_ptr == xi.data_ptr() and pre.dtype == dtype and pre.P == P and
                    pre.C == C)
            if have:
                sums, prezeroed = pre.sums, True
            else:
                sums = ZeroArena.take(x.device, nsum)
                prezeroed = sums is not None
                if not prezeroed:
                    sums = torch.empty((nsum,), dtype=torch.float64, device=x.device)
            call("mr_bn_fwd_train", dt, ptr(xi), ptr(y), ptr(gamma), ptr(beta), ptr(running_mean),
                 ptr(running_var), ptr(mean), ptr(rstd), ptr(sums), ptr(ri),
                 int(relu) | (4 if prezeroed else 0) | (8 if have else 0), P, C, float(eps), float(momentum),
                 ptr(num_batches_tracked))
        else:
            call("mr_bn_fwd_eval", dt, ptr(xi), ptr(y), ptr(gamma), ptr(beta), ptr(running_mean), ptr(running_var),
                 ptr(mean), ptr(rstd), ptr(ri), int(relu), P, C, float(eps))
        ctx.save_for_backward(xi, y if relu else None, gamma, mean, rstd)
        ctx.params = (gamma, beta)
        ctx.relu = relu
        ctx.has_res = residual is not None
        ctx.dtype = dtype
        ctx.training_mode = training
        ctx.bnb_link = None
        if link is not None and training:
            link.xi, link.y, link.mean, link.rstd, link.dtype = xi, (y if relu else None), mean, rstd, dtype
            ctx.bnb_link = link
        return y.permute(0, 3, 1, 2)

    @staticmethod
    def backward(ctx, gy):
        if not ctx.training_mode:
            raise NotImplementedError("backward through eval-mode BatchNorm is not on the training hot path")
        _no_resident_grids_beside_collectives()
        xi, y, gamma, mean, rstd = ctx.saved_tensors
        dtype = ctx.dtype
        dt = dtype_code(dtype)
        g = _grad_internal(gy, dtype)
        N, H, W, C = xi.shape
        P = N * H * W
        dx = torch.empty_like(xi)
        dres = torch.empty_like(xi) if ctx.has_res else None
        nsum = load().mr_bn_scratch_doubles(C)
        link = ctx.bnb_link
        have = link is not None and link.sums is not None and link.grad_ptr == g.data_ptr()
        if have:
            sums, prezeroed = link.sums, True
        else:
            sums = ZeroArena.take(g.device, nsum)
            prezeroed = sums is not None
            if not prezeroed:
                sums = torch.empty((nsum,), dtype=torch.float64, device=g.device)
        if link is not None:
            link.xi = link.y = link.mean = link.rstd = link.sums = None
        gamma_p, beta_p = ctx.params
        g_sink, b_sink = grad_sink(gamma_p, (C,)), grad_sink(beta_p, (C,))
        sunk = g_sink is not None and b_sink is not None and ctx.needs_input_grad[1] and ctx.needs_input_grad[2]
        if sunk:
            dgamma, dbeta = g_sink, b_sink
        else:
            dgamma = torch.empty((C,), dtype=torch.float32, device=g.device)
            dbeta = torch.empty((C,), dtype=torch.float32, device=g.device)
        call("mr_bn_bwd", dt, ptr(g), ptr(xi), ptr(y), ptr(gamma), ptr(mean), ptr(rstd), ptr(sums), ptr(dx),
             ptr(dres), ptr(dgamma), ptr(dbeta),
             int(ctx.relu) | (2 if sunk else 0) | (4 if prezeroed else 0) | (8 if have else 0), P, C)
        gres = dres.permute(0, 3, 1, 2) if ctx.has_res else None
        if sunk:
            notify_grad_ready(gamma_p)
            notify_grad_ready(beta_p)
            dgamma = dbeta = None
        return dx.permute(0, 3, 1, 2), dgamma, dbeta, None, None, None, None, None, None, gres, None, None, None


def batch_norm(x, gamma, beta, running_mean, running_var, training, momentum, eps, relu=False, residual=None,
               num_batches_tracked=None):
    if num_batches_tracked is not None and (num_batches_tracked.dtype != torch.int64 or not training):
        num_batches_tracked = None
    pre = getattr(x, "_mr_bn_sums", None) if training else None
    link = BnBwdLink() if (training and BNB_EPILOGUE and torch.is_grad_enabled() and x.requires_grad) else None
    out = BatchNormFn.apply(x, gamma, beta, running_mean, running_var, bool(training), momentum, eps, bool(relu),
                            residual, num_batches_tracked, pre, link)
    if link is not None and link.xi is not None:
        out._mr_bnb_link = link
    return out


class SyncBatchNormFn(Function):
    @staticmethod
    def forward(ctx, x, gamma, beta, running_mean, running_var, momentum, eps, relu, residual, num_batches_tracked,
                all_reduce):
        require_cuda(x, gamma, beta)
        dtype = get_compute_dtype()
        dt = dtype_code(dtype)
        xi = to_internal(x, dtype)
        N, H, W, C = xi.shape
        P = N * H * W
        dev = x.device
        ri = to_internal(residual, dtype) if residual is not None else None
        sums = torch.zeros((load().mr_bn_scratch_doubles(C),), dtype=torch.float64, device=dev)
        call("mr_bn_stats", dt, ptr(xi), ptr(sums), P, C)
        packed = torch.cat([sums[:16 * C].view(8, 2 * C).sum(dim=0), torch.full((1,), float(P), dtype=torch.float64,
                                                                                 device=dev)])
        all_reduce(packed)
        total = packed[2 * C]
        mean64 = packed[:C] / total
        var64 = (packed[C:2 * C] / total - mean64 * mean64).clamp_(min=0.0)
        mean_g, var_g = mean64.float(), var64.float()
        if running_mean is not None:
            with torch.no_grad():
                unbiased = var64 * (total / (total - 1.0).clamp(min=1.0))
                running_mean.mul_(1.0 - momentum).add_(mean_g, alpha=momentum)
                running_var.mul_(1.0 - momentum).add_(unbiased.float(), alpha=momentum)
                if num_batches_tracked is not None:
                    num_batches_tracked.add_(1)
        y = torch.empty_like(xi)
        mean = torch.empty((C,), dtype=torch.float32, device=dev)
        rstd = torch.empty((C,), dtype=torch.float32, device=dev)
        call("mr_bn_fwd_eval", dt, ptr(xi), ptr(y), ptr(gamma), ptr(beta), ptr(mean_g), ptr(var_g), ptr(mean), ptr(rstd),
             ptr(ri), int(relu), P, C, float(eps))
        ctx.save_for_backward(xi, y if relu else None, gamma, mean, rstd)
        ctx.total = total
        ctx.relu = relu
        ctx.has_res = residual is not None
        ctx.dtype = dtype
        ctx.all_reduce = all_reduce
        return y.permute(0, 3, 1, 2)

    @staticmethod
    def backward(ctx, gy):
        xi, y, gamma, mean, rstd = ctx.saved_tensors
        dtype = ctx.dtype
        dt = dtype_code(dtype)
        g = _grad_internal(gy, dtype)
        N, H, W, C = xi.shape
        P = N * H * W
        dev = g.device
        dx = torch.empty_like(xi)
        dres = torch.empty_like(xi) if ctx.has_res else None
        sums = torch.zeros((load().mr_bn_scratch_doubles(C),), dtype=torch.float64, device=dev)
        dgamma = torch.empty((C,), dtype=torch.float32, device=dev)
        dbeta = torch.empty((C,), dtype=torch.float32, device=dev)
        call("mr_bn_bwd", dt, ptr(g), ptr(xi), ptr(y), ptr(gamma), ptr(mean), ptr(rstd), ptr(sums), ptr(dx), ptr(dres),
             ptr(dgamma), ptr(dbeta), int(ctx.relu) | 4, P, C)
        glob = torch.cat([dbeta, dgamma]).double()
        ctx.all_reduce(glob)
        total = ctx.total
        d1 = dbeta.double() / P - glob[:C] / total
        d2 = dgamma.double() / P - glob[C:] / total
        k = gamma.detach().double() * rstd.double()
        slope = (k * d2 * rstd.double())
        alpha = (k * d1 - slope * mean.double()).to(dtype)
        dx = torch.addcmul(dx + alpha, xi, slope.to(dtype))
        gres = dres.permute(0, 3, 1, 2) if ctx.has_res else None
        return dx.permute(0, 3, 1, 2), dgamma, dbeta, None, None, None, None, None, gres, None, None


def sync_batch_norm(x, gamma, beta, running_mean, running_var, momentum, eps, relu=False, residual=None,
                    num_batches_tracked=None, all_reduce=None):
    if all_reduce is None:
        import torch.distributed as dist

        def all_reduce(t):
            dist.all_reduce(t, op=dist.ReduceOp.SUM)
    return SyncBatchNormFn.apply(x, gamma, beta, running_mean, running_var, momentum, eps, bool(relu), residual,
                                 num_batches_tracked, all_reduce)


def stem_eligible(x, weight, stride, padding, dilation, pool_kernel, pool_stride, pool_padding):
    return (x.is_cuda and x.dim() == 4 and not x.requires_grad and x.shape[1] in (1, 3) and
            tuple(weight.shape) == (64, x.shape[1], 3, 3) and tuple(stride) == (1, 1) and tuple(padding) == (1, 1) and
            tuple(dilation) == (1, 1) and tuple(pool_kernel) == (2, 2) and tuple(pool_stride) == (2, 2) and
            tuple(pool_padding) == (0, 0) and x.shape[2] % 2 == 0 and x.shape[3] % 2 == 0 and
            16 * (x.shape[3] + 2) * x.shape[1] <= 48 * 1024)


class StemConvReluPoolFn(Function):
    @staticmethod
    def forward(ctx, x, weight, bias):
        require_cuda(x, weight, bias)
        dtype = get_compute_dtype()
        dt = dtype_code(dtype)
        if x.dtype != torch.float32 or not x.is_contiguous():
            x = x.float().contiguous()
        N, C, H, W = x.shape
        y = torch.empty((N, H // 2, W // 2, 64), dtype=dtype, device=x.device)
        code = torch.empty((N, H // 2, W // 2, 64), dtype=torch.uint8, device=x.device)
        sk, sc, sr, ss = weight.stride()
        wpack = None
        if dtype == torch.bfloat16:
            def build(old):
                buf = old[0] if old is not None else torch.empty((64, 32), dtype=dtype, device=x.device)
                return (buf,), [prep.stem_job(ptr(weight), (sk, sc, sr, ss), ptr(buf), C)]

            wpack = prep.prepared((weight,), ("stem", C), build, dtype)[0]
        call("mr_stem_fwd", dt, ptr(x), ptr(weight), sk, sc, sr, ss, ptr(wpack), ptr(bias), ptr(y), ptr(code), N, C,
             H, W)
        ctx.save_for_backward(x, code)
        ctx.params = (weight, bias)
        ctx.dtype = dtype
        return y.permute(0, 3, 1, 2)

    @staticmethod
    def backward(ctx, gy):
        x, code = ctx.saved_tensors
        weight_p, bias_p = ctx.params
        dtype = ctx.dtype
        N, C, H, W = x.shape
        g = _grad_internal(gy, dtype)
        want_dw = ctx.needs_input_grad[1]
        want_db = bias_p is not None and ctx.needs_input_grad[2]
        w_sink = grad_sink(weight_p, "strided") if want_dw else None
        b_sink = grad_sink(bias_p, (64,)) if want_db else None
        dw = db = None
        if want_dw:
            dw = w_sink if w_sink is not None else torch.zeros_like(weight_p)
        if want_db:
            db = b_sink if b_sink is not None else torch.zeros((64,), dtype=torch.float32, device=g.device)
        if dw is not None or db is not None:
            ws = torch.empty((load().mr_stem_bwd_workspace(C),), dtype=torch.float32, device=g.device)
            sk, sc, sr, ss = dw.stride() if dw is not None else (0, 0, 0, 0)
            call("mr_stem_bwd", dtype_code(dtype), ptr(g), ptr(code), ptr(x), ptr(ws), ptr(dw), sk, sc, sr, ss, ptr(db),
                 N, C, H, W)
        if w_sink is not None:
            notify_grad_ready(weight_p)
            dw = None
        if b_sink is not None:
            notify_grad_ready(bias_p)
            db = None
        return None, dw, db


def stem_conv_relu_pool(x, weight, bias):
    return StemConvReluPoolFn.apply(x, weight, bias)


class ConvReluPoolFn(Function):

    @staticmethod
    def forward(ctx, x, weight, bias, padding, pool_kernel, pool_stride, pool_padding):
        require_cuda(x, weight, bias)
        dtype = get_compute_dtype()
        dt = dtype_code(dtype)
        xi = to_internal(x, dtype)
        N, H, W, Cp = xi.shape
        K, C, R, S = weight.shape
        ph, pw = padding
        Ho, Wo = _conv_out(H, R, 1, ph, 1), _conv_out(W, S, 1, pw, 1)
        kh, kw = pool_kernel
        psh, psw = pool_stride
        pph, ppw = pool_padding
        PHo, PWo = (Ho + 2 * pph - kh) // psh + 1, (Wo + 2 * ppw - kw) // psw + 1
        need_dx = ctx.needs_input_grad[0]
        w_krsc, w_crsk, bias_k = _conv_operands(weight, bias, dtype, Cp, K, need_dx)
        y = torch.empty((N, PHo, PWo, K), dtype=dtype, device=x.device)
        idx = torch.empty((N, PHo, PWo, K), dtype=torch.uint8, device=x.device)
        call("mr_conv2d_fwd_pool", dt, ptr(xi), ptr(w_krsc), ptr(bias_k), ptr(y), ptr(idx), 1, N, H, W, Cp, Cp, K, R, S, 1, 1, ph, pw,
             1, 1, Ho, Wo, kh, kw, psh, psw, pph, ppw, PHo, PWo)
        ctx.save_for_backward(xi, w_crsk, idx, y)
        ctx.params = (weight, bias)
        ctx.geom = (N, H, W, Cp, C, K, K, R, S, 1, 1, ph, pw, 1, 1, Ho, Wo)
        ctx.pool = (kh, kw, psh, psw, pph, ppw, PHo, PWo)
        ctx.has_bias = bias is not None
        ctx.dtype = dtype
        return y.permute(0, 3, 1, 2)

    @staticmethod
    def backward(ctx, gy):
        xi, w_crsk, idx, y = ctx.saved_tensors
        N, H, W, Cp, C, K, Kp, R, S, sh, sw, ph, pw, dh, dw, Ho, Wo = ctx.geom
        kh, kw, psh, psw, pph, ppw, PHo, PWo = ctx.pool
        dtype = ctx.dtype
        g = _grad_internal(gy, dtype)
        dz = torch.empty((N, Ho, Wo, K), dtype=dtype, device=g.device)
        call("mr_maxpool_bwd", dtype_code(dtype), ptr(g), ptr(idx), ptr(y), ptr(dz), N, Ho, Wo, K, kh, kw, psh, psw, pph, ppw,
             PHo, PWo)

        class _ConvCtx(object):
            pass
        c = _ConvCtx()
        c.saved_tensors = (xi, w_crsk, None)
        c.geom, c.dtype, c.params, c.has_bias = ctx.geom, dtype, ctx.params, ctx.has_bias
        c.relu, c.bnb_link = False, None
        c.needs_input_grad = (ctx.needs_input_grad[0], ctx.needs_input_grad[1], ctx.needs_input_grad[2]) + (False,) * 8
        grads = Conv2dFn.backward(c, dz.permute(0, 3, 1, 2))
        return grads[0], grads[1], grads[2], None, None, None, None


def conv_relu_pool_eligible(x, weight, stride, padding, dilation, pool_kernel, pool_stride, pool_padding):
    if not x.is_cuda or get_compute_dtype() != torch.bfloat16 or tuple(stride) != (1, 1) or tuple(dilation) != (1, 1):
        return False
    if os.environ.get("MEGREADER_CONV_POOL", "1") == "0":
        return False
    N, C, H, W = x.shape
    K, Cw, R, S = weight.shape
    if C != Cw or C % 8 != 0 or K % 8 != 0:
        return False
    ph, pw = padding
    Ho, Wo = _conv_out(H, R, 1, ph, 1), _conv_out(W, S, 1, pw, 1)
    return bool(load().mr_conv2d_fwd_pool_ok(dtype_code(torch.bfloat16), N, H, W, C, C, K, R, S, 1, 1, ph, pw, 1, 1, Ho, Wo,
                                             pool_kernel[0], pool_kernel[1], pool_stride[0], pool_stride[1],
                                             pool_padding[0], pool_padding[1]))


def conv_relu_pool(x, weight, bias, padding, pool_kernel, pool_stride, pool_padding):
    return ConvReluPoolFn.apply(x, weight, bias, tuple(padding), tuple(pool_kernel), tuple(pool_stride), tuple(pool_padding))


class MaxPoolFn(Function):
    @staticmethod
    def forward(ctx, x, kernel, stride, padding, relu_input=False):
        require_cuda(x)
        dtype = get_compute_dtype()
        dt = dtype_code(dtype)
        xi = to_internal(x, dtype)
        N, H, W, C = xi.shape
        kh, kw = kernel
        sh, sw = stride
        ph, pw = padding
        Ho, Wo = (H + 2 * ph - kh) // sh + 1, (W + 2 * pw - kw) // sw + 1
        y = torch.empty((N, Ho, Wo, C), dtype=dtype, device=x.device)
        idx = torch.empty((N, Ho, Wo, C), dtype=torch.uint8, device=x.device)
        call("mr_maxpool_fwd", dt, ptr(xi), ptr(y), ptr(idx), N, H, W, C, kh, kw, sh, sw, ph, pw, Ho, Wo)
        ctx.save_for_backward(idx, y if relu_input else None)
        ctx.geom = (N, H, W, C, kh, kw, sh, sw, ph, pw, Ho, Wo)
        ctx.dtype = dtype
        return y.permute(0, 3, 1, 2)

    @staticmethod
    def backward(ctx, gy):
        idx, relu_y = ctx.saved_tensors
        N, H, W, C, kh, kw, sh, sw, ph, pw, Ho, Wo = ctx.geom
        dtype = ctx.dtype
        g = _grad_internal(gy, dtype)
        dx = torch.empty((N, H, W, C), dtype=dtype, device=g.device)
        call("mr_maxpool_bwd", dtype_code(dtype), ptr(g), ptr(idx), ptr(relu_y), ptr(dx), N, H, W, C, kh, kw, sh, sw,
             ph, pw, Ho, Wo)
        return dx.permute(0, 3, 1, 2), None, None, None, None


def max_pool2d(x, kernel, stride=None, padding=(0, 0), relu_input=False):
    stride = kernel if stride is None else stride
    return MaxPoolFn.apply(x, tuple(kernel), tuple(stride), tuple(padding), bool(relu_input))


class MapToSequenceFn(Function):
    @staticmethod
    def forward(ctx, x):
        require_cuda(x)
        dtype = get_compute_dtype()
        xi = to_internal(x, dtype)
        N, H, W, C = xi.shape
        if H != 1:
            raise AssertionError("the height of conv must be 1")
        out = torch.empty((W, N, C), dtype=dtype, device=x.device)
        call("mr_permute_021", dtype_code(dtype), ptr(xi), ptr(out), N, W, C)
        ctx.shape = (N, W, C)
        ctx.dtype = dtype
        return out

    @staticmethod
    def backward(ctx, g):
        N, W, C = ctx.shape
        dtype = ctx.dtype
        if g.dtype != dtype or not g.is_contiguous():
            g = g.to(dtype).contiguous()
        dx = torch.empty((N, 1, W, C), dtype=dtype, device=g.device)
        call("mr_permute_021", dtype_code(dtype), ptr(g), ptr(dx), W, N, C)
        return dx.permute(0, 3, 1, 2)


def map_to_sequence(x):
    return MapToSequenceFn.apply(x)


class LinearFn(Function):
    @staticmethod
    def forward(ctx, x, weight, bias):
        require_cuda(x, weight, bias)
        dtype = get_compute_dtype()
        dt = dtype_code(dtype)
        v = vec_of(dtype)
        lead = x.shape[:-1]
        K = x.shape[-1]
        x2 = x.reshape(-1, K)
        if x2.dtype != dtype or not x2.is_contiguous():
            x2 = x2.to(dtype).contiguous()
        M = x2.shape[0]
        Nout = weight.shape[0]
        Np = _ceil_to(Nout, v)
        if weight.dim() != 2 or weight.stride() != (K, 1):
            raise RuntimeError("linear: weight must be a dense row-major [out_features, in_features] tensor "
                               "(got strides %s); call .contiguous() on views" % (tuple(weight.stride()),))
        if K % v:
            raise RuntimeError("Linear: in_features (%d) must be a multiple of %d" % (K, v))
        def build(old):
            if old is None:
                w_n_ = torch.empty((Nout, K), dtype=dtype, device=x.device)
                w_t_ = (torch.zeros if Np != Nout else torch.empty)((K, Np), dtype=dtype, device=x.device)
            else:
                w_n_, w_t_ = old
            return (w_n_, w_t_), [prep.matrix_job(ptr(weight), K, ptr(w_n_), K, ptr(w_t_), Np, Nout, K, 0)]

        w_n, w_t = prep.prepared((weight,), ("linear", Np), build, dtype)
        y = torch.empty((M, Np), dtype=dtype, device=x.device)
        call("mr_gemm_nt", dt, ptr(x2), K, ptr(w_n), K, ptr(y), Np, ptr(bias), 0, M, Nout, K)
        ctx.save_for_backward(x2, w_t)
        ctx.params = (weight, bias)
        ctx.dims = (M, K, Nout, Np)
        ctx.lead = lead
        ctx.has_bias = bias is not None
        ctx.dtype = dtype
        return y[:, :Nout].view(*lead, Nout) if Np == Nout else y.view(*lead, Np)[..., :Nout]

    @staticmethod
    def backward(ctx, gy):
        x2, w_t = ctx.saved_tensors
        M, K, Nout, Np = ctx.dims
        dtype = ctx.dtype
        dt = dtype_code(dtype)
        g2 = gy.reshape(-1, Nout) if gy.shape[-1] == Nout else gy
        if Np != Nout:
            gp = _zero_padded_rows(gy, M, Nout, Np, dtype)
            if gp is None:
                gp = torch.zeros((M, Np), dtype=dtype, device=gy.device)
                gp[:, :Nout] = g2
        else:
            gp = g2 if (g2.dtype == dtype and g2.is_contiguous()) else g2.to(dtype).contiguous()
        dx = dw = db = None
        dx_fn = None
        if ctx.needs_input_grad[0]:
            dx2 = torch.empty((M, K), dtype=dtype, device=gy.device)
            dx_fn = lambda: call("mr_gemm_nt", dt, ptr(gp), Np, ptr(w_t), Np, ptr(dx2), K, 0, 0, M, K, Np)
            dx = dx2.view(*ctx.lead, K)
        weight_p, bias_p = ctx.params
        want_db = ctx.has_bias and ctx.needs_input_grad[2]
        w_sink = grad_sink(weight_p, (Nout, K)) if ctx.needs_input_grad[1] else None
        b_sink = grad_sink(bias_p, (Nout,)) if (want_db and (w_sink is not None or not ctx.needs_input_grad[1])) else None
        NA = Nout if (w_sink is not None or (not ctx.needs_input_grad[1] and b_sink is not None)) else Np
        gb = None
        if want_db:
            gb = b_sink if b_sink is not None else torch.zeros((Np,), dtype=torch.float32, device=gy.device)
        if ctx.needs_input_grad[1]:
            gw = w_sink if w_sink is not None else torch.zeros((Np, K), dtype=torch.float32, device=gy.device)
            def lin_launch():
                if dx_fn is not None:
                    dx_fn()
                call("mr_gemm_tn", dt, ptr(gp), Np, ptr(x2), K, ptr(gw), K, M, NA, K, 0, ptr(gb))
            if _wgrad(lin_launch, w_sink is not None and (gb is None or b_sink is not None) and dtype == torch.bfloat16,
                      (gp, x2), [weight_p] + ([bias_p] if want_db else [])):
                return dx, None, None
            dx_fn = None
            if w_sink is not None:
                notify_grad_ready(weight_p)
            else:
                dw = gw[:Nout]
        elif want_db:
            call("mr_colsum", dt, ptr(gp), ptr(gb), M, NA, Np, 0)
        if dx_fn is not None:
            dx_fn()
        if want_db:
            if b_sink is not None:
                notify_grad_ready(bias_p)
            else:
                db = gb[:Nout]
        return dx, dw, db


def linear(x, weight, bias=None):
    return LinearFn.apply(x, weight, bias)


class ConvTranspose2x2Fn(Function):
    @staticmethod
    def forward(ctx, x, weight, bias):
        require_cuda(x, weight, bias)
        dtype = get_compute_dtype()
        dt = dtype_code(dtype)
        v = vec_of(dtype)
        xi = to_internal(x, dtype)
        N, H, W, Cin = xi.shape
        if tuple(weight.shape[2:]) != (2, 2) or weight.shape[0] != Cin or not weight.is_contiguous():
            raise RuntimeError("conv_transpose2x2: weight must be a dense [Cin, Cout, 2, 2] tensor matching the input")
        Cout = weight.shape[1]
        K4 = 4 * Cout
        ld2 = _ceil_to(K4, v)
        P = N * H * W
        dev = x.device

        def build(old):
            if old is None:
                w_n_ = (torch.zeros if ld2 != K4 else torch.empty)((Cin, ld2), dtype=dtype, device=dev)
                w_t_ = torch.empty((K4, Cin), dtype=dtype, device=dev)
            else:
                w_n_, w_t_ = old
            return (w_n_, w_t_), [prep.matrix_job(ptr(weight), K4, ptr(w_n_), ld2, ptr(w_t_), Cin, Cin, K4, 0)]

        w_n, w_t = prep.prepared((weight,), ("deconv2x2", ld2), build, dtype)
        x2 = xi.reshape(P, Cin)
        y2 = torch.empty((P, ld2), dtype=dtype, device=dev)
        call("mr_gemm_nt", dt, ptr(x2), Cin, ptr(w_t), Cin, ptr(y2), ld2, 0, 0, P, K4, Cin)
        y = torch.empty((N, 2 * H, 2 * W, Cout), dtype=dtype, device=dev)
        call("mr_deconv2x2_d2s", dt, ptr(y2), ld2, ptr(bias), ptr(y), N, H, W, Cout)
        ctx.save_for_backward(x2, w_n)
        ctx.params = (weight, bias)
        ctx.geom = (N, H, W, Cin, Cout, ld2)
        ctx.dtype = dtype
        return y.permute(0, 3, 1, 2)

    @staticmethod
    def backward(ctx, gy):
        x2, w_n = ctx.saved_tensors
        N, H, W, Cin, Cout, ld2 = ctx.geom
        dtype = ctx.dtype
        dt = dtype_code(dtype)
        P, K4 = N * H * W, 4 * Cout
        dev = gy.device
        if Cout % vec_of(dtype) == 0:
            g = _grad_internal(gy, dtype)
            if not g.is_contiguous():
                g = g.contiguous()
        else:
            g = gy.permute(0, 2, 3, 1).contiguous().to(dtype)
        dy2 = torch.empty((P, ld2), dtype=dtype, device=dev)
        call("mr_deconv2x2_s2d", dt, ptr(g), ptr(dy2), ld2, N, H, W, Cout)
        weight_p, bias_p = ctx.params
        dx = dw = db = None
        if ctx.needs_input_grad[0]:
            dxi = torch.empty((N, H, W, Cin), dtype=dtype, device=dev)
            call("mr_gemm_nt", dt, ptr(dy2), ld2, ptr(w_n), ld2, ptr(dxi), Cin, 0, 0, P, Cin, ld2)
            dx = dxi.permute(0, 3, 1, 2)
        want_db = bias_p is not None and ctx.needs_input_grad[2]
        if want_db:
            b_sink = grad_sink(bias_p, (Cout,))
            gb = b_sink if b_sink is not None else torch.zeros((Cout,), dtype=torch.float32, device=dev)
            call("mr_colsum", dt, ptr(g), ptr(gb), N * 4 * H * W, Cout, Cout, 0)
            if b_sink is not None:
                notify_grad_ready(bias_p)
            else:
                db = gb
        if ctx.needs_input_grad[1]:
            w_sink = grad_sink(weight_p)
            if ld2 != K4:
                tmp = torch.zeros((Cin, ld2), dtype=torch.float32, device=dev)
                call("mr_gemm_tn", dt, ptr(x2), Cin, ptr(dy2), ld2, ptr(tmp), ld2, P, Cin, ld2, 0, 0)
                if w_sink is not None:
                    w_sink.view(Cin, K4).add_(tmp[:, :K4])
                    notify_grad_ready(weight_p)
                else:
                    dw = tmp[:, :K4].reshape(Cin, Cout, 2, 2)
            else:
                gw = w_sink if w_sink is not None else torch.zeros((Cin, K4), dtype=torch.float32, device=dev)

                def deconv_launch():
                    call("mr_gemm_tn", dt, ptr(x2), Cin, ptr(dy2), ld2, ptr(gw), K4, P, Cin, K4, 0, 0)
                if _wgrad(deconv_launch, w_sink is not None and dtype == torch.bfloat16, (x2, dy2), [weight_p]):
                    pass
                elif w_sink is not None:
                    notify_grad_ready(weight_p)
                else:
                    dw = gw.view(Cin, Cout, 2, 2)
        return dx, dw, db


class DBHeadTailFn(Function):

    @staticmethod
    def forward(ctx, xb, xt, k):
        require_cuda(xb, xt)
        if xb.dtype != xt.dtype or xb.dtype not in _ESIZE or xb.shape != xt.shape:
            raise RuntimeError("db_head_tail: the two logit maps must share shape and dtype (float32 / bfloat16)")
        xbc = xb if xb.is_contiguous() or xb.permute(0, 2, 3, 1).is_contiguous() else xb.contiguous()
        xtc = xt if xt.is_contiguous() or xt.permute(0, 2, 3, 1).is_contiguous() else xt.contiguous()
        n = xb.numel()
        shape = tuple(xb.shape)
        binary = torch.empty(shape, dtype=torch.float32, device=xb.device)
        thresh = torch.empty(shape, dtype=torch.float32, device=xb.device)
        tbinary = torch.empty(shape, dtype=torch.float32, device=xb.device)
        call("mr_db_head_tail_fwd", dtype_code(xb.dtype), ptr(xbc), ptr(xtc), ptr(binary), ptr(thresh), ptr(tbinary), n, float(k))
        ctx.save_for_backward(binary, thresh, tbinary)
        ctx.meta = (xb.dtype, shape, float(k))
        ctx.set_materialize_grads(False)
        return binary, thresh, tbinary

    @staticmethod
    def backward(ctx, gb, gt, gtb):
        binary, thresh, tbinary = ctx.saved_tensors
        dtype, shape, k = ctx.meta
        gs = [None if g is None else (g if (g.dtype == torch.float32 and g.is_contiguous()) else g.float().contiguous())
              for g in (gb, gt, gtb)]
        dxb = torch.empty(shape, dtype=dtype, device=binary.device)
        dxt = torch.empty(shape, dtype=dtype, device=binary.device)
        call("mr_db_head_tail_bwd", dtype_code(dtype), ptr(binary), ptr(thresh), ptr(tbinary), ptr(gs[0]), ptr(gs[1]), ptr(gs[2]),
             ptr(dxb), ptr(dxt), binary.numel(), k)
        return dxb, dxt, None


def db_head_tail(xb, xt, k):
    return DBHeadTailFn.apply(xb, xt, k)


def conv_transpose2x2(x, weight, bias=None):
    return ConvTranspose2x2Fn.apply(x, weight, bias)


LSTM_STATUS = None
LSTM_LOCAL = None


def _lstm_workspace(dt, T, N, H, dev):
    nbytes = load().mr_lstm_ws_bytes(dt, T, N, H)
    if nbytes <= 0:
        return None, 0
    size = nbytes
    arena = ZeroArena.take(dev, (nbytes + 7) // 8)
    if arena is not None:
        ws = arena.view(torch.uint8)[:nbytes]
        size = -nbytes
    else:
        ws = torch.empty((nbytes,), dtype=torch.uint8, device=dev)
    if LSTM_STATUS is not None:
        LSTM_STATUS.append(ws[nbytes - 256:nbytes - 252])
    if LSTM_LOCAL is not None:
        LSTM_LOCAL.append(ws[nbytes - 252:nbytes - 248])
    return ws, size


class BiLSTMFn(Function):
    @staticmethod
    def forward(ctx, x, w_ih, w_hh, b_ih, b_hh, w_ih_r, w_hh_r, b_ih_r, b_hh_r):
        require_cuda(x, w_ih)
        dtype = get_compute_dtype()
        dt = dtype_code(dtype)
        v = vec_of(dtype)
        es = _ESIZE[dtype]
        if x.dtype != dtype or not x.is_contiguous():
            x = x.to(dtype).contiguous()
        T, N, I = x.shape
        H = w_hh.shape[1]
        if I % v or H % v:
            raise RuntimeError("LSTM: input (%d) and hidden (%d) sizes must be multiples of %d" % (I, H, v))
        dev = x.device
        sources = (w_ih, w_hh, b_ih, b_hh, w_ih_r, w_hh_r, b_ih_r, b_hh_r)

        def build(old):
            if old is None:
                wcat_ = torch.empty((8 * H, I), dtype=dtype, device=dev)
                wcat_t_ = torch.empty((I, 8 * H), dtype=dtype, device=dev)
                whh_ = torch.empty((2, 4 * H, H), dtype=dtype, device=dev)
                whh_t_ = torch.empty((2, H, 4 * H), dtype=dtype, device=dev)
                bcat_ = torch.empty((8 * H,), dtype=torch.float32, device=dev)
            else:
                wcat_, wcat_t_, whh_, whh_t_, bcat_ = old
            jobs = []
            for d, (wi, wh, bi, bh) in enumerate(((w_ih, w_hh, b_ih, b_hh), (w_ih_r, w_hh_r, b_ih_r, b_hh_r))):
                jobs.append(prep.matrix_job(ptr(wi), I, ptr(wcat_) + d * 4 * H * I * es, I,
                                            ptr(wcat_t_) + d * 4 * H * es, 8 * H, 4 * H, I, H))
                jobs.append(prep.matrix_job(ptr(wh), H, ptr(whh_) + d * 4 * H * H * es, H,
                                            ptr(whh_t_) + d * 4 * H * H * es, 4 * H, 4 * H, H, H))
                jobs.append(prep.bias_job(ptr(bi), ptr(bh), ptr(bcat_) + d * 4 * H * 4, 4 * H, H))
            return (wcat_, wcat_t_, whh_, whh_t_, bcat_), jobs

        wcat, wcat_t, whh, whh_t, bcat = prep.prepared(sources, ("bilstm",), build, dtype)
        xproj = torch.empty((T * N, 8 * H), dtype=dtype, device=dev)
        call("mr_gemm_nt", dt, ptr(x), I, ptr(wcat), I, ptr(xproj), 8 * H, ptr(bcat), 0, T * N, 8 * H, I)
        out = torch.empty((T, N, 2 * H), dtype=dtype, device=dev)
        cbuf = torch.empty((T, N, 2 * H), dtype=torch.float32, device=dev)
        gates = torch.empty((T, N, 8 * H), dtype=dtype, device=dev)
        ws, ws_size = _lstm_workspace(dt, T, N, H, dev)
        call("mr_lstm_fwd", dt, ptr(xproj), ptr(whh), ptr(out), ptr(cbuf), ptr(gates), T, N, H, ptr(ws), ws_size)
        ctx.save_for_backward(x, wcat_t, whh_t, out, cbuf, gates)
        ctx.params = sources
        ctx.dims = (T, N, I, H)
        ctx.dtype = dtype
        return out

    @staticmethod
    def backward(ctx, gout):
        x, wcat_t, whh_t, out, cbuf, gates = ctx.saved_tensors
        T, N, I, H = ctx.dims
        dtype = ctx.dtype
        dt = dtype_code(dtype)
        es = _ESIZE[dtype]
        dev = gout.device
        if gout.dtype != dtype or not gout.is_contiguous():
            gout = gout.to(dtype).contiguous()
        ws, ws_size = _lstm_workspace(dt, T, N, H, dev)
        dc = torch.empty((N, 2 * H), dtype=torch.float32, device=dev) if ws is None else None
        call("mr_lstm_bwd", dt, ptr(gout), ptr(whh_t), ptr(cbuf), ptr(gates), ptr(dc), T, N, H, ptr(ws), ws_size)
        dgates = gates
        sinks = [grad_sink(p, tuple(p.shape)) for p in ctx.params]
        use_sinks = all(s is not None for s in sinks)
        dx = dx_fn = None
        if ctx.needs_input_grad[0]:
            dx = torch.empty((T, N, I), dtype=dtype, device=dev)
            dx_fn = lambda: call("mr_gemm_nt", dt, ptr(dgates), 8 * H, ptr(wcat_t), 8 * H, ptr(dx), I, 0, 0, T * N, I,
                                 8 * H)
        P = (T - 1) * N
        grads = (None,) * 8

        def lstm_grouped():
            if dx_fn is not None:
                dx_fn()
            for d in range(2):
                call("mr_gemm_tn2", dt, ptr(dgates) + d * 4 * H * es, 8 * H, ptr(x), I, ptr(sinks[4 * d]), I, T * N, 4 * H, I,
                     H, ptr(sinks[4 * d + 2]), ptr(sinks[4 * d + 3]))
            call("mr_gemm_tn", dt, ptr(dgates) + N * 8 * H * es, 8 * H, ptr(out), 2 * H, ptr(sinks[1]), H, P, 4 * H, H, H, 0)
            call("mr_gemm_tn", dt, ptr(dgates) + 4 * H * es, 8 * H, ptr(out) + (N * 2 * H + H) * es, 2 * H, ptr(sinks[5]), H,
                 P, 4 * H, H, H, 0)

        def lstm_immediate():
            nonlocal grads
            if dx_fn is not None:
                dx_fn()
            nfl = 2 * 4 * H * (I + 1)
            arena = ZeroArena.take(dev, (nfl + 1) // 2) if use_sinks else None
            scratch = (arena.view(torch.float32)[:nfl] if arena is not None else
                       torch.zeros((nfl,), dtype=torch.float32, device=dev))
            gw_ih = scratch[:2 * 4 * H * I].view(2, 4 * H, I)
            gb = scratch[2 * 4 * H * I:].view(2, 4 * H)
            if use_sinks:
                g_hh = (sinks[1], sinks[5])
            else:
                gw_hh = torch.zeros((2, 4 * H, H), dtype=torch.float32, device=dev)
                g_hh = (gw_hh[0], gw_hh[1])
            call("mr_gemm_tn", dt, ptr(dgates), 8 * H, ptr(x), I, ptr(gw_ih), I, T * N, 8 * H, I, H, ptr(gb))
            if T > 1:
                call("mr_gemm_tn", dt, ptr(dgates) + N * 8 * H * es, 8 * H, ptr(out), 2 * H, ptr(g_hh[0]), H, P, 4 * H, H, H, 0)
                call("mr_gemm_tn", dt, ptr(dgates) + 4 * H * es, 8 * H, ptr(out) + (N * 2 * H + H) * es, 2 * H, ptr(g_hh[1]),
                     H, P, 4 * H, H, H, 0)
            if use_sinks:
                accumulate_multi([(sinks[0], gw_ih[0]), (sinks[4], gw_ih[1]), (sinks[2], gb[0]), (sinks[3], gb[0]),
                                  (sinks[6], gb[1]), (sinks[7], gb[1])])
            else:
                grads = (gw_ih[0], g_hh[0], gb[0], gb[0].clone(), gw_ih[1], g_hh[1], gb[1], gb[1].clone())

        if _wgrad(lstm_grouped, use_sinks and dtype == torch.bfloat16 and T > 1, (dgates, x, out), list(ctx.params),
                  immediate=lstm_immediate):
            _TnDefer.flush(final=False)
        elif use_sinks:
            for p in ctx.params:
                notify_grad_ready(p)
        return (dx,) + grads


def bilstm(x, w_ih, w_hh, b_ih, b_hh, w_ih_r, w_hh_r, b_ih_r, b_hh_r):
    return BiLSTMFn.apply(x, w_ih, w_hh, b_ih, b_hh, w_ih_r, w_hh_r, b_ih_r, b_hh_r)


_FULL_LENGTHS = {}


class CTCLossFn(Function):
    @staticmethod
    def forward(ctx, logits, targets, input_lengths, target_lengths, blank, zero_infinity, want_f64=False):
        require_cuda(logits, targets, target_lengths)
        T, N, C = logits.shape
        dtype = logits.dtype
        if dtype not in _ESIZE:
            raise TypeError("ctc_loss: logits must be float32 or bfloat16")
        if logits.stride(2) != 1 or logits.stride(1) * N != logits.stride(0):
            logits = logits.contiguous()
        ldl = logits.stride(1)
        if targets.dim() != 2 or targets.shape[0] != N:
            raise RuntimeError("ctc_loss: targets must be padded [N, S]")
        S = targets.shape[1]
        targets = targets.contiguous()
        if targets.dtype not in (torch.int32, torch.int64):
            targets = targets.long()
        if input_lengths is None:
            key = (N, T, logits.device)
            input_lengths = _FULL_LENGTHS.get(key)
            if input_lengths is None:
                if len(_FULL_LENGTHS) > 64:
                    _FULL_LENGTHS.clear()
                input_lengths = _FULL_LENGTHS[key] = torch.full((N,), T, dtype=torch.int64, device=logits.device)
        input_lengths = input_lengths.to(device=logits.device, dtype=torch.int64).contiguous()
        target_lengths = target_lengths.to(device=logits.device, dtype=torch.int64).contiguous()
        dev = logits.device
        lp = torch.empty((T, N, C), dtype=torch.float32, device=dev)
        lp64 = torch.empty((T, N, C), dtype=torch.float64, device=dev) if want_f64 else None
        alpha = torch.empty((N, T, 2 * S + 1), dtype=torch.float64, device=dev)
        beta = torch.empty((N, T, 2 * S + 1), dtype=torch.float64, device=dev) if ctx.needs_input_grad[0] else None
        nll = torch.empty((N,), dtype=torch.float64, device=dev)
        loss = torch.empty((), dtype=torch.float64, device=dev)
        t64 = int(targets.dtype == torch.int64)
        call("mr_ctc_fwd", dtype_code(dtype), ptr(logits), ldl, ptr(targets), t64, ptr(input_lengths),
             ptr(target_lengths), 1, T, N, C, S, int(blank), int(zero_infinity), ptr(lp), ptr(alpha), ptr(beta),
             ptr(nll), ptr(loss), ptr(lp64))
        ctx.save_for_backward(lp, alpha, beta, nll, targets, input_lengths, target_lengths)
        ctx.dims = (T, N, C, S, int(blank), int(zero_infinity), t64)
        ctx.dtype = dtype
        out_lp = lp64 if want_f64 else lp
        ctx.mark_non_differentiable(out_lp)
        ctx.set_materialize_grads(False)
        if int(zero_infinity) & 2:
            return nll / target_lengths.to(torch.float64), out_lp
        return loss, out_lp

    @staticmethod
    def backward(ctx, gloss, _glp):
        lp, alpha, beta, nll, targets, input_lengths, target_lengths = ctx.saved_tensors
        T, N, C, S, blank, zero_inf, t64 = ctx.dims
        dtype = ctx.dtype
        v = vec_of(dtype)
        Cp = _ceil_to(C, v)
        if gloss is None:
            return None, None, None, None, None, None, None
        g = gloss.to(torch.float64).contiguous()
        grad = torch.empty((T, N, Cp), dtype=dtype, device=lp.device)
        call("mr_ctc_bwd", dtype_code(dtype), ptr(lp), ptr(alpha), ptr(beta), ptr(nll), ptr(targets), t64,
             ptr(input_lengths),
             ptr(target_lengths), 1, ptr(g), T, N, C, S, blank, zero_inf, ptr(grad), Cp)
        if Cp != C:
            mark_zero_padded(grad)
        return grad[..., :C], None, None, None, None, None, None


def ctc_loss_logits(logits, targets, input_lengths, target_lengths, blank=0, zero_infinity=True, per_sample=False,
                    log_probs_f64=False):
    flags = int(bool(zero_infinity)) | (2 if per_sample else 0)
    return CTCLossFn.apply(logits, targets, input_lengths, target_lengths, blank, flags, bool(log_probs_f64))


def softmax_eval_nc1t(logits):
    require_cuda(logits)
    T, N, C = logits.shape
    lg = logits.detach()
    if lg.stride(2) != 1 or lg.stride(1) * N != lg.stride(0):
        lg = lg.contiguous()
    out = torch.empty((N, C, 1, T), dtype=torch.float32, device=lg.device)
    call("mr_softmax_nc1t", dtype_code(lg.dtype), ptr(lg), lg.stride(1), ptr(out), T, N, C)
    return out


class AdaptiveAvgPoolFn(Function):
    @staticmethod
    def forward(ctx, x, out_hw):
        require_cuda(x)
        dtype = get_compute_dtype()
        xi = to_internal(x, dtype)
        N, H, W, C = xi.shape
        OH, OW = out_hw
        y = torch.empty((N, OH, OW, C), dtype=dtype, device=x.device)
        call("mr_adaptive_avgpool_fwd", dtype_code(dtype), ptr(xi), ptr(y), N, H, W, C, OH, OW)
        ctx.geom = (N, H, W, C, OH, OW)
        ctx.dtype = dtype
        return y.permute(0, 3, 1, 2)

    @staticmethod
    def backward(ctx, gy):
        N, H, W, C, OH, OW = ctx.geom
        g = _grad_internal(gy, ctx.dtype)
        dx = torch.empty((N, H, W, C), dtype=ctx.dtype, device=g.device)
        call("mr_adaptive_avgpool_bwd", dtype_code(ctx.dtype), ptr(g), ptr(dx), N, H, W, C, OH, OW)
        return dx.permute(0, 3, 1, 2), None


def adaptive_avg_pool2d(x, output_size):
    if isinstance(output_size, int):
        output_size = (output_size, output_size)
    return AdaptiveAvgPoolFn.apply(x, tuple(output_size))


class AdaptiveAvgPoolMultiFn(Function):

    @staticmethod
    def forward(ctx, x, sizes):
        require_cuda(x)
        dtype = get_compute_dtype()
        xi = to_internal(x, dtype)
        N, H, W, C = xi.shape
        n = len(sizes)
        ys = [torch.empty((N, oh, ow, C), dtype=dtype, device=x.device) for oh, ow in sizes]
        oh = (ctypes.c_int * n)(*[s_[0] for s_ in sizes])
        ow = (ctypes.c_int * n)(*[s_[1] for s_ in sizes])
        call("mr_adaptive_avgpool_multi_fwd", dtype_code(dtype), ptr(xi), (ctypes.c_void_p * n)(*[y.data_ptr() for y in ys]),
             oh, ow, n, N, H, W, C)
        ctx.geom = (N, H, W, C, tuple(sizes))
        ctx.dtype = dtype
        return tuple(y.permute(0, 3, 1, 2) for y in ys)

    @staticmethod
    def backward(ctx, *gys):
        N, H, W, C, sizes = ctx.geom
        dtype = ctx.dtype
        n = len(sizes)
        dev = next(g for g in gys if g is not None).device
        gs = [_grad_internal(g, dtype) if g is not None else torch.zeros((N, oh, ow, C), dtype=dtype, device=dev)
              for g, (oh, ow) in zip(gys, sizes)]
        dx = torch.empty((N, H, W, C), dtype=dtype, device=dev)
        oh = (ctypes.c_int * n)(*[s_[0] for s_ in sizes])
        ow = (ctypes.c_int * n)(*[s_[1] for s_ in sizes])
        call("mr_adaptive_avgpool_multi_bwd", dtype_code(dtype), (ctypes.c_void_p * n)(*[g.data_ptr() for g in gs]), oh, ow, n,
             ptr(dx), N, H, W, C)
        return dx.permute(0, 3, 1, 2), None


def adaptive_avg_pool2d_multi(x, output_sizes):
    sizes = [(s_, s_) if isinstance(s_, int) else tuple(s_) for s_ in output_sizes]
    if not (1 <= len(sizes) <= 8) or x.shape[2] * x.shape[3] * 128 > 32768 or x.shape[1] % vec_of(get_compute_dtype()) \
            or sum(a * b for a, b in sizes) > 256 or max(x.shape[2], x.shape[3]) > 128:
        return tuple(adaptive_avg_pool2d(x, s_) for s_ in sizes)
    return AdaptiveAvgPoolMultiFn.apply(x, tuple(sizes))


class BilinearFn(Function):
    @staticmethod
    def forward(ctx, x, out_hw):
        require_cuda(x)
        dtype = get_compute_dtype()
        xi = to_internal(x, dtype)
        N, H, W, C = xi.shape
        OH, OW = out_hw
        y = torch.empty((N, OH, OW, C), dtype=dtype, device=x.device)
        call("mr_bilinear_fwd", dtype_code(dtype), ptr(xi), ptr(y), N, H, W, C, OH, OW, C, 0, 0)
        ctx.geom = (N, H, W, C, OH, OW)
        ctx.dtype = dtype
        return y.permute(0, 3, 1, 2)

    @staticmethod
    def backward(ctx, gy):
        N, H, W, C, OH, OW = ctx.geom
        g = _grad_internal(gy, ctx.dtype)
        dx = torch.empty((N, H, W, C), dtype=ctx.dtype, device=g.device)
        call("mr_bilinear_bwd", dtype_code(ctx.dtype), ptr(g), ptr(dx), N, H, W, C, OH, OW, C, 0)
        return dx.permute(0, 3, 1, 2), None


def interpolate_bilinear(x, size):
    return BilinearFn.apply(x, tuple(size))


class BilinearCatFn(Function):

    @staticmethod
    def forward(ctx, base, *branches):
        require_cuda(base)
        dtype = get_compute_dtype()
        dt = dtype_code(dtype)
        bi = to_internal(base, dtype)
        parts = [to_internal(b, dtype) for b in branches]
        N, OH, OW, C0 = bi.shape
        Ct = C0 + sum(p.shape[3] for p in parts)
        y = torch.empty((N, OH, OW, Ct), dtype=dtype, device=bi.device)
        call("mr_copy_channels", dt, ptr(bi), C0, 0, ptr(y), Ct, 0, N * OH * OW, C0)
        off = C0
        geoms = []
        for p in parts:
            _, H, W, C = p.shape
            call("mr_bilinear_fwd", dt, ptr(p), ptr(y), N, H, W, C, OH, OW, Ct, off, 0)
            geoms.append((H, W, C, off))
            off += C
        ctx.geom = (N, OH, OW, C0, Ct, tuple(geoms))
        ctx.dtype = dtype
        return y.permute(0, 3, 1, 2)

    @staticmethod
    def backward(ctx, gy):
        N, OH, OW, C0, Ct, geoms = ctx.geom
        g = _grad_internal(gy, ctx.dtype)
        dt = dtype_code(ctx.dtype)
        d0 = torch.empty((N, OH, OW, C0), dtype=ctx.dtype, device=g.device)
        call("mr_copy_channels", dt, ptr(g), Ct, 0, ptr(d0), C0, 0, N * OH * OW, C0)
        outs = [d0.permute(0, 3, 1, 2)]
        for H, W, C, off in geoms:
            d = torch.empty((N, H, W, C), dtype=ctx.dtype, device=g.device)
            call("mr_bilinear_bwd", dt, ptr(g), ptr(d), N, H, W, C, OH, OW, Ct, off)
            outs.append(d.permute(0, 3, 1, 2))
        return tuple(outs)


def cat_bilinear(base, branches):
    v = vec_of(get_compute_dtype())
    if base.shape[1] % v or any(b.shape[1] % v for b in branches):
        return cat_channels([base] + [interpolate_bilinear(b, base.shape[2:]) for b in branches])
    return BilinearCatFn.apply(base, *branches)


class UpsampleAddFn(Function):

    @staticmethod
    def forward(ctx, x, y):
        require_cuda(x, y)
        dtype = get_compute_dtype()
        dt = dtype_code(dtype)
        xi, yi = to_internal(x, dtype), to_internal(y, dtype)
        N, H, W, C = xi.shape
        _, OH, OW, C2 = yi.shape
        if C != C2:
            raise RuntimeError("upsample_add: channel mismatch")
        out = torch.empty_like(yi)
        call("mr_copy_channels", dt, ptr(yi), C, 0, ptr(out), C, 0, N * OH * OW, C)
        call("mr_bilinear_fwd", dt, ptr(xi), ptr(out), N, H, W, C, OH, OW, C, 0, 1)
        ctx.geom = (N, H, W, C, OH, OW)
        ctx.dtype = dtype
        return out.permute(0, 3, 1, 2)

    @staticmethod
    def backward(ctx, g_out):
        N, H, W, C, OH, OW = ctx.geom
        g = _grad_internal(g_out, ctx.dtype)
        dx = torch.empty((N, H, W, C), dtype=ctx.dtype, device=g.device)
        call("mr_bilinear_bwd", dtype_code(ctx.dtype), ptr(g), ptr(dx), N, H, W, C, OH, OW, C, 0)
        return dx.permute(0, 3, 1, 2), g_out


def upsample_add(x, y):
    return UpsampleAddFn.apply(x, y)


class NearestUpFn(Function):

    @staticmethod
    def forward(ctx, x, scale, add):
        require_cuda(x)
        dtype = get_compute_dtype()
        dt = dtype_code(dtype)
        xi = to_internal(x, dtype)
        N, H, W, C = xi.shape
        ai = to_internal(add, dtype) if add is not None else None
        out = torch.empty((N, H * scale, W * scale, C), dtype=dtype, device=xi.device)
        call("mr_nearest_up_fwd", dt, ptr(xi), ptr(ai), ptr(out), N, H, W, C, int(scale), C, 0)
        ctx.geom = (N, H, W, C, int(scale))
        ctx.dtype = dtype
        ctx.has_add = add is not None
        return out.permute(0, 3, 1, 2)

    @staticmethod
    def backward(ctx, g_out):
        N, H, W, C, s = ctx.geom
        g = _grad_internal(g_out, ctx.dtype)
        dx = torch.empty((N, H, W, C), dtype=ctx.dtype, device=g.device)
        call("mr_nearest_up_bwd", dtype_code(ctx.dtype), ptr(g), ptr(dx), N, H, W, C, s, C, 0)
        return dx.permute(0, 3, 1, 2), None, (g_out if ctx.has_add else None)


def upsample_nearest(x, scale, add=None):
    return NearestUpFn.apply(x, scale, add)


class CatChannelsFn(Function):

    @staticmethod
    def forward(ctx, *xs):
        dtype = get_compute_dtype()
        dt = dtype_code(dtype)
        parts = [to_internal(x, dtype) for x in xs]
        N, H, W, _ = parts[0].shape
        chans = [p.shape[3] for p in parts]
        Ct = sum(chans)
        y = torch.empty((N, H, W, Ct), dtype=dtype, device=parts[0].device)
        off = 0
        for p, c in zip(parts, chans):
            call("mr_copy_channels", dt, ptr(p), c, 0, ptr(y), Ct, off, N * H * W, c)
            off += c
        ctx.chans = chans
        ctx.dtype = dtype
        return y.permute(0, 3, 1, 2)

    @staticmethod
    def backward(ctx, gy):
        g = _grad_internal(gy, ctx.dtype)
        N, H, W, Ct = g.shape
        dt = dtype_code(ctx.dtype)
        outs, off = [], 0
        for c in ctx.chans:
            d = torch.empty((N, H, W, c), dtype=ctx.dtype, device=g.device)
            call("mr_copy_channels", dt, ptr(g), Ct, off, ptr(d), c, 0, N * H * W, c)
            outs.append(d.permute(0, 3, 1, 2))
            off += c
        return tuple(outs)


def cat_channels(tensors):
    return CatChannelsFn.apply(*tensors)


class ScaleChannelsFn(Function):

    @staticmethod
    def forward(ctx, x, scale):
        dtype = get_compute_dtype()
        xi = to_internal(x, dtype)
        N, H, W, C = xi.shape
        y = torch.empty_like(xi)
        call("mr_scale_channels", dtype_code(dtype), ptr(xi), ptr(scale), ptr(y), N, H * W, C)
        ctx.save_for_backward(scale)
        ctx.dtype = dtype
        return y.permute(0, 3, 1, 2)

    @staticmethod
    def backward(ctx, gy):
        (scale,) = ctx.saved_tensors
        g = _grad_internal(gy, ctx.dtype)
        N, H, W, C = g.shape
        dx = torch.empty_like(g)
        call("mr_scale_channels", dtype_code(ctx.dtype), ptr(g), ptr(scale), ptr(dx), N, H * W, C)
        return dx.permute(0, 3, 1, 2), None


def dropout2d(x, p, training):
    if not training or p == 0.0:
        return x
    N, C = x.shape[0], x.shape[1]
    keep = torch.empty((N, C), dtype=torch.float32, device=x.device).bernoulli_(1.0 - p)
    return ScaleChannelsFn.apply(x, keep / (1.0 - p))


class CTC2DHeadFn(Function):
    @staticmethod
    def forward(ctx, mask_logits, cls_logits, tiny):
        require_cuda(mask_logits, cls_logits)
        a = mask_logits.permute(0, 2, 3, 1)
        z = cls_logits.permute(0, 2, 3, 1)
        if a.stride(3) != 1 or z.stride(3) != 1 or a.dtype != z.dtype:
            raise RuntimeError("ctc2d head expects channel-contiguous NHWC logits")
        N, H, W, C = z.shape
        lda, ldz = a.stride(2), z.stride(2)
        for t, ld in ((a, lda), (z, ldz)):
            if t.stride(1) != W * ld or t.stride(0) != H * W * ld:
                raise RuntimeError("ctc2d head expects dense (row-padded) NHWC logits")
        dev = z.device
        lp = torch.empty((W, H, N, C), dtype=torch.float32, device=dev)
        m = torch.empty((N, H, W), dtype=torch.float32, device=dev)
        p = torch.empty((N, H, W, C), dtype=torch.float32, device=dev)
        call("mr_ctc2d_head_fwd", dtype_code(z.dtype), ptr(a), lda, ptr(z), ldz, ptr(lp), ptr(m), ptr(p), N, H, W, C,
             float(tiny))
        ctx.save_for_backward(m, p)
        ctx.geom = (N, H, W, C, float(tiny))
        ctx.dtype = z.dtype
        ctx.mark_non_differentiable(m, p)
        return lp, m.unsqueeze(1), p.permute(0, 3, 1, 2)

    @staticmethod
    def backward(ctx, glp, _gm, _gp):
        m, p = ctx.saved_tensors
        N, H, W, C, tiny = ctx.geom
        dtype = ctx.dtype
        v = vec_of(dtype)
        Cp = _ceil_to(C, v)
        g = glp.to(torch.float32).contiguous()
        da = torch.zeros((N, H, W, v), dtype=dtype, device=g.device)
        dz = torch.zeros((N, H, W, Cp), dtype=dtype, device=g.device) if Cp != C else \
            torch.empty((N, H, W, Cp), dtype=dtype, device=g.device)
        call("mr_ctc2d_head_bwd", dtype_code(dtype), ptr(g), ptr(m), ptr(p), ptr(da), v, ptr(dz), Cp, N, H, W, C, tiny)
        return da[..., :1].permute(0, 3, 1, 2), dz[..., :C].permute(0, 3, 1, 2), None


def ctc2d_head(mask_logits, cls_logits, tiny):
    return CTC2DHeadFn.apply(mask_logits, cls_logits, tiny)
```

### megreader_amd/nn/modules.py

```python
import math

import torch
import torch.nn as nn

from . import functional as F


BN_EPILOGUE = __import__("os").environ.get("MEGREADER_BN_EPILOGUE", "1") != "0"


FORK_RESIDUAL = __import__("os").environ.get("MEGREADER_FORK_RESIDUAL", "1") != "0"


def _pair(v):
    return tuple(v) if isinstance(v, (tuple, list)) else (v, v)


class Conv2d(nn.Conv2d):

    def __init__(self, *args, fuse_relu=False, relu_grad_downstream=False, **kwargs):
        super().__init__(*args, **kwargs)
        if self.groups != 1 or self.padding_mode != "zeros" or isinstance(self.padding, str):
            raise NotImplementedError("megreader_amd.nn.Conv2d supports groups=1 and explicit zero padding only")
        self.fuse_relu = fuse_relu
        self.relu_grad_downstream = relu_grad_downstream and fuse_relu
        self.weight.data = self.weight.data.contiguous(memory_format=torch.channels_last)

    feeds_batch_norm = False
    sole_consumer_of_bn = False
    sole_consumer_when_forked = False

    def forward(self, x):
        y = F.conv2d(x, self.weight, self.bias, self.stride, self.padding, self.dilation, self.fuse_relu,
                     self.relu_grad_downstream, bn_stats=self.feeds_batch_norm and self.training and BN_EPILOGUE,
                     sole_consumer_of_bn=self.sole_consumer_of_bn)
        y._mr_producer = self
        return y

    def forward_fork(self, x):
        if not FORK_RESIDUAL:
            y = F.conv2d(x, self.weight, self.bias, self.stride, self.padding, self.dilation, self.fuse_relu,
                         self.relu_grad_downstream, bn_stats=self.feeds_batch_norm and self.training and BN_EPILOGUE)
            y._mr_producer = self
            return y, x
        y, xr = F.conv2d(x, self.weight, self.bias, self.stride, self.padding, self.dilation, self.fuse_relu,
                         self.relu_grad_downstream, bn_stats=self.feeds_batch_norm and self.training and BN_EPILOGUE,
                         fork=True, sole_consumer_of_bn=self.sole_consumer_when_forked)
        y._mr_producer = self
        return y, xr


class FusedReLU(nn.Module):

    def forward(self, x):
        return x


class BatchNorm2d(nn.BatchNorm2d):
    def __init__(self, *args, fuse_relu=False, **kwargs):
        super().__init__(*args, **kwargs)
        if not (self.affine and self.track_running_stats):
            raise NotImplementedError("megreader_amd.nn.BatchNorm2d requires affine=True, track_running_stats=True")
        if self.momentum is None:
            raise NotImplementedError("megreader_amd.nn.BatchNorm2d: momentum=None (cumulative moving average) is not "
                                      "used by any reference model; pass a float")
        self.fuse_relu = fuse_relu

    def forward(self, x, residual=None):
        momentum = self.momentum
        if self.training:
            producer = getattr(x, "_mr_producer", None)
            if producer is not None and not producer.feeds_batch_norm and not producer.fuse_relu:
                producer.feeds_batch_norm = True
        return F.batch_norm(x, self.weight, self.bias, self.running_mean, self.running_var, self.training, momentum,
                            self.eps, self.fuse_relu, residual,
                            self.num_batches_tracked if self.training else None)


class MaxPool2d(nn.MaxPool2d):
    def __init__(self, *args, relu_input=False, **kwargs):
        super().__init__(*args, **kwargs)
        self.relu_input = relu_input

    def forward(self, x):
        if self.ceil_mode or _pair(self.dilation) != (1, 1) or self.return_indices:
            raise NotImplementedError("megreader_amd.nn.MaxPool2d: ceil_mode / dilation / return_indices unsupported")
        stride = self.kernel_size if self.stride is None else self.stride
        return F.max_pool2d(x, _pair(self.kernel_size), _pair(stride), _pair(self.padding), self.relu_input)


class Linear(nn.Linear):
    def forward(self, x):
        return F.linear(x, self.weight, self.bias)


class LSTM(nn.Module):

    def __init__(self, input_size, hidden_size, num_layers=1, bias=True, batch_first=False, dropout=0.0,
                 bidirectional=False):
        super().__init__()
        if num_layers != 1 or not bias or batch_first or dropout or not bidirectional:
            raise NotImplementedError("megreader_amd.nn.LSTM implements nn.LSTM(nIn, nHidden, bidirectional=True)")
        self.input_size, self.hidden_size = input_size, hidden_size
        self.num_layers, self.bidirectional = 1, True
        for suffix in ("", "_reverse"):
            self.register_parameter("weight_ih_l0" + suffix, nn.Parameter(torch.empty(4 * hidden_size, input_size)))
            self.register_parameter("weight_hh_l0" + suffix, nn.Parameter(torch.empty(4 * hidden_size, hidden_size)))
            self.register_parameter("bias_ih_l0" + suffix, nn.Parameter(torch.empty(4 * hidden_size)))
            self.register_parameter("bias_hh_l0" + suffix, nn.Parameter(torch.empty(4 * hidden_size)))
        self.reset_parameters()

    def reset_parameters(self):
        stdv = 1.0 / math.sqrt(self.hidden_size) if self.hidden_size > 0 else 0
        for w in self.parameters():
            nn.init.uniform_(w, -stdv, stdv)

    def flatten_parameters(self):
        pass

    def forward(self, x, hx=None):
        if hx is not None:
            raise NotImplementedError("initial states are not used on the reference path")
        out = F.bilstm(x, self.weight_ih_l0, self.weight_hh_l0, self.bias_ih_l0, self.bias_hh_l0,
                       self.weight_ih_l0_reverse, self.weight_hh_l0_reverse, self.bias_ih_l0_reverse,
                       self.bias_hh_l0_reverse)
        return out, None


class AdaptiveAvgPool2d(nn.AdaptiveAvgPool2d):
    def forward(self, x):
        size = self.output_size if isinstance(self.output_size, (tuple, list)) else (self.output_size,) * 2
        return F.adaptive_avg_pool2d(x, size)


class Dropout2d(nn.Dropout2d):
    def forward(self, x):
        return F.dropout2d(x, self.p, self.training)
```

Measured before the change: 105,000 images/s.

## Write final BN output in sequence layout and derive ReLU mask from input

The last backbone BatchNorm now writes its output directly in (W,N,C) sequence order, so map_to_sequence can return a view instead of running a separate transpose kernel. Backward reads the incoming gradient in that order too. Separately, when ReLU is fused and there is no residual or link, the backward pass recomputes the ReLU mask from x, gamma and beta instead of saving and re-reading y. This removes a transpose pass and a saved tensor read, at the cost of strided scatter/gather addressing and extra arithmetic in the BN kernels.

```diff
diff --git a/include/megreader_hip.h b/include/megreader_hip.h
--- a/include/megreader_hip.h
+++ b/include/megreader_hip.h
@@ -176,6 +176,13 @@
 int mr_bn_bwd(int dtype, const void* dy, const void* x, const void* y, const float* gamma, const float* save_mean,
               const float* save_rstd, double* sums, void* dx, void* dres, float* dgamma, float* dbeta, int flags,
               long long P, int C, hipStream_t stream);
+int mr_bn_bwd_x(int dtype, const void* dy, const void* x, const void* y, const float* gamma, const float* beta,
+                const float* save_mean, const float* save_rstd, double* sums, void* dx, void* dres, float* dgamma,
+                float* dbeta, int flags, long long P, int C, int seq_n, hipStream_t stream);
+int mr_bn_fwd_train_seq(int dtype, const void* x, void* y, const float* gamma, const float* beta, float* running_mean,
+                        float* running_var, float* save_mean, float* save_rstd, double* sums, const void* residual,
+                        int relu, long long P, int C, float eps, float momentum, long long* num_batches_tracked,
+                        int seq_n, hipStream_t stream);
 int mr_maxpool_fwd(int dtype, const void* x, void* y, unsigned char* idx, int N, int H, int W, int C, int kh,
                    int kw, int sh, int sw, int ph, int pw, int Ho, int Wo, hipStream_t stream);
 int mr_maxpool_bwd(int dtype, const void* dy, const unsigned char* idx, const void* relu_y, void* dx, int N, int H,
diff --git a/megreader_amd/backbones/crnn.py b/megreader_amd/backbones/crnn.py
--- a/megreader_amd/backbones/crnn.py
+++ b/megreader_amd/backbones/crnn.py
@@ -51,6 +51,7 @@
         self.cnn = nn.Sequential(conv0, conv1, conv2, conv3, conv4, conv5, conv6)
         conv3[0][0].sole_consumer_of_bn = True
         conv5[0][0].sole_consumer_of_bn = True
+        conv6[1].sequence_output = True
 
     def _make_layer(self, i, batch_normalization=False, pooled=False):
         in_channel = self.channels[i - 1]
diff --git a/megreader_amd/csrc/norm_pool.hip b/megreader_amd/csrc/norm_pool.hip
--- a/megreader_amd/csrc/norm_pool.hip
+++ b/megreader_amd/csrc/norm_pool.hip
@@ -3,6 +3,25 @@
 
 
 namespace mr {
+
+__device__ __forceinline__ float bn_affine(float x, float mu, float rs, float ga, float be) {
+  return __builtin_fmaf((x - mu) * rs, ga, be);
+}
+template <typename T>
+__device__ __forceinline__ T bn_out(float v, int relu) {
+  if (relu) v = fmaxf(v, 0.f);
+  return from_f32<T>(v);
+}
+template <typename T>
+__device__ __forceinline__ bool bn_live(float x, float mu, float rs, float ga, float be) {
+  return to_f32(bn_out<T>(bn_affine(x, mu, rs, ga, be), 1)) > 0.f;
+}
+enum { BN_RELU_NONE = 0, BN_RELU_Y = 1, BN_RELU_X = 2 };
+__device__ __forceinline__ int bn_seq_row(int p, int seq_n, int seq_w) {
+  if (!seq_n) return p;
+  const int n = p / seq_w;
+  return (p - n * seq_w) * seq_n + n;
+}
 
 template <typename T>
 __global__ void bn_stats_kernel(const T* __restrict__ x, double* __restrict__ sums, int P, int C, long long ld,
@@ -35,8 +54,10 @@
                                                             const T* __restrict__ yin,
                                                             const float* __restrict__ mean,
                                                             const float* __restrict__ rstd,
+                                                            const float* __restrict__ gamma,
+                                                            const float* __restrict__ beta,
                                                             double* __restrict__ sums, int relu, int P, int C,
-                                                            int rows_per_block, int ncopy) {
+                                                            int rows_per_block, int ncopy, int seq_n, int seq_w) {
   constexpr int VEC = VecOf<T>::N;
   __shared__ float red[2][256 * VEC];
   sums += (size_t)(blockIdx.x % ncopy) * 2 * C;
@@ -45,12 +66,13 @@
   const int g = threadIdx.x / cv, v = threadIdx.x - g * cv;
   const int p0 = blockIdx.x * rows_per_block;
   const int p1 = min(P, p0 + rows_per_block);
-  float s[VEC], q[VEC], mu[VEC], rs[VEC];
+  float s[VEC], q[VEC], mu[VEC], rs[VEC], ga[VEC], be[VEC];
 #pragma unroll
   for (int j = 0; j < VEC; ++j) {
     s[j] = q[j] = 0.f;
     mu[j] = 0.f;
     rs[j] = 1.f;
+    ga[j] = be[j] = 0.f;
   }
   if (g < groups) {
     if (MODE == 1) {
@@ -59,11 +81,18 @@
         mu[j] = mean[v * VEC + j];
         rs[j] = rstd[v * VEC + j];
       }
+      if (relu == BN_RELU_X) {
+#pragma unroll
+        for (int j = 0; j < VEC; ++j) {
+          ga[j] = gamma[v * VEC + j];
+          be[j] = beta[v * VEC + j];
+        }
+      }
     }
 #pragma unroll 4
     for (int p = p0 + g; p < p1; p += groups) {
       const long long i = (long long)p * cv + v;
-      const uint4 av = ((const uint4*)a)[i];
+      const uint4 av = ((const uint4*)a)[MODE == 1 ? (long long)bn_seq_row(p, seq_n, seq_w) * cv + v : i];
       const T* pa = (const T*)&av;
       if (MODE == 0) {
 #pragma unroll
@@ -76,14 +105,16 @@
         const uint4 xv = ((const uint4*)xin)[i];
         const T* px = (const T*)&xv;
         uint4 yv = make_uint4(0, 0, 0, 0);
-        if (relu) yv = ((const uint4*)yin)[i];
+        if (relu == BN_RELU_Y) yv = ((const uint4*)yin)[i];
         const T* py = (const T*)&yv;
 #pragma unroll
         for (int j = 0; j < VEC; ++j) {
           float gd = to_f32(pa[j]);
-          if (relu && !(to_f32(py[j]) > 0.f)) gd = 0.f;
+          const float xf = to_f32(px[j]);
+          if (relu == BN_RELU_Y && !(to_f32(py[j]) > 0.f)) gd = 0.f;
+          if (relu == BN_RELU_X && !bn_live<T>(xf, mu[j], rs[j], ga[j], be[j])) gd = 0.f;
           s[j] += gd;
-          q[j] += gd * (to_f32(px[j]) - mu[j]) * rs[j];
+          q[j] += gd * (xf - mu[j]) * rs[j];
         }
       }
     }
@@ -133,7 +164,7 @@
 __global__ void bn_apply_kernel(const T* __restrict__ x, T* __restrict__ y, const float* __restrict__ mean,
                                 const float* __restrict__ rstd, const float* __restrict__ gamma,
                                 const float* __restrict__ beta, const T* __restrict__ residual, int relu,
-                                long long P, int C) {
+                                long long P, int C, int seq_n, int seq_w) {
   constexpr int VEC = VecOf<T>::N;
   const int cv = C / VEC;
   const long long total = P * cv;
@@ -148,19 +179,20 @@
 #pragma unroll
     for (int j = 0; j < VEC; ++j) {
       const int c = c0 + j;
-      float v = (to_f32(pa[j]) - mean[c]) * rstd[c] * gamma[c] + beta[c];
+      float v = bn_affine(to_f32(pa[j]), mean[c], rstd[c], gamma[c], beta[c]);
       if (residual) v += to_f32(pr[j]);
-      if (relu) v = fmaxf(v, 0.f);
-      pa[j] = from_f32<T>(v);
-    }
-    ((uint4*)y)[i] = a;
+      pa[j] = bn_out<T>(v, relu);
+    }
+    ((uint4*)y)[seq_n ? (long long)bn_seq_row((int)(i / cv), seq_n, seq_w) * cv + i % cv : i] = a;
   }
 }
 
 template <typename T>
 __global__ void bn_bwd_reduce_kernel(const T* __restrict__ dy, const T* __restrict__ x, const T* __restrict__ y,
                                      const float* __restrict__ mean, const float* __restrict__ rstd,
-                                     double* __restrict__ sums, int relu, int P, int C, int rows_per_block) {
+                                     const float* __restrict__ gamma, const float* __restrict__ beta,
+                                     double* __restrict__ sums, int relu, int P, int C, int rows_per_block, int seq_n,
+                                     int seq_w) {
   __shared__ float red[2][4][64];
   const int lane = threadIdx.x & 63, wave = threadIdx.x >> 6;
   const int c = blockIdx.x * 64 + lane;
@@ -169,12 +201,15 @@
   float s = 0.f, q = 0.f;
   if (c < C) {
     const float mu = mean[c], rs = rstd[c];
+    const float ga = relu == BN_RELU_X ? gamma[c] : 0.f, be = relu == BN_RELU_X ? beta[c] : 0.f;
     for (int p = p0 + wave; p < p1; p += 4) {
       const long long idx = (long long)p * C + c;
-      float g = to_f32(dy[idx]);
-      if (relu && !(to_f32(y[idx]) > 0.f)) g = 0.f;
+      float g = to_f32(dy[(long long)bn_seq_row(p, seq_n, seq_w) * C + c]);
+      const float xf = to_f32(x[idx]);
+      if (relu == BN_RELU_Y && !(to_f32(y[idx]) > 0.f)) g = 0.f;
+      if (relu == BN_RELU_X && !bn_live<T>(xf, mu, rs, ga, be)) g = 0.f;
       s += g;
-      q += g * (to_f32(x[idx]) - mu) * rs;
+      q += g * (xf - mu) * rs;
     }
   }
   red[0][wave][lane] = s;
@@ -208,18 +243,19 @@
 template <typename T>
 __global__ void bn_bwd_apply_kernel(const T* __restrict__ dy, const T* __restrict__ x, const T* __restrict__ y,
                                     const float* __restrict__ mean, const float* __restrict__ rstd,
-                                    const float* __restrict__ gamma, const float* __restrict__ sbg,
-                                    T* __restrict__ dx, T* __restrict__ dres, int relu, long long P, int C) {
+                                    const float* __restrict__ gamma, const float* __restrict__ beta,
+                                    const float* __restrict__ sbg, T* __restrict__ dx, T* __restrict__ dres, int relu,
+                                    long long P, int C, int seq_n, int seq_w) {
   constexpr int VEC = VecOf<T>::N;
   const int cv = C / VEC;
   const long long total = P * cv;
   for (long long i = blockIdx.x * (long long)blockDim.x + threadIdx.x; i < total;
        i += (long long)gridDim.x * blockDim.x) {
     const int c0 = (int)(i % cv) * VEC;
-    uint4 g = ((const uint4*)dy)[i];
+    uint4 g = ((const uint4*)dy)[seq_n ? (long long)bn_seq_row((int)(i / cv), seq_n, seq_w) * cv + i % cv : i];
     uint4 a = ((const uint4*)x)[i];
     uint4 o = make_uint4(0, 0, 0, 0);
-    if (relu) o = ((const uint4*)y)[i];
+    if (relu == BN_RELU_Y) o = ((const uint4*)y)[i];
     T* pg = (T*)&g;
     const T* pa = (const T*)&a;
     const T* po = (const T*)&o;
@@ -229,9 +265,11 @@
     for (int j = 0; j < VEC; ++j) {
       const int c = c0 + j;
       float gv = to_f32(pg[j]);
-      if (relu && !(to_f32(po[j]) > 0.f)) gv = 0.f;
+      const float xf = to_f32(pa[j]);
+      if (relu == BN_RELU_Y && !(to_f32(po[j]) > 0.f)) gv = 0.f;
+      if (relu == BN_RELU_X && !bn_live<T>(xf, mean[c], rstd[c], gamma[c], beta[c])) gv = 0.f;
       pg[j] = from_f32<T>(gv);
-      const float xh = (to_f32(pa[j]) - mean[c]) * rstd[c];
+      const float xh = (xf - mean[c]) * rstd[c];
       const float sb = sbg[c], sg = sbg[C + c];
       pout[j] = from_f32<T>(gamma[c] * rstd[c] * (gv - sb - xh * sg));
     }
@@ -245,7 +283,7 @@
     const T* __restrict__ x, T* __restrict__ y, const double* __restrict__ sums, int ncopy, float eps, float momentum,
     float* __restrict__ save_mean, float* __restrict__ save_rstd, float* __restrict__ running_mean,
     float* __restrict__ running_var, long long* __restrict__ num_batches_tracked, const float* __restrict__ gamma,
-    const float* __restrict__ beta, const T* __restrict__ residual, int relu, int P, int C) {
+    const float* __restrict__ beta, const T* __restrict__ residual, int relu, int P, int C, int seq_n, int seq_w) {
   constexpr int VEC = VecOf<T>::N, LANES = 64 / VEC, ROWS = 256 / LANES;
   __shared__ float s_mean[64], s_rstd[64], s_gamma[64], s_beta[64];
   const int cbase = blockIdx.y * 64;
@@ -295,23 +333,22 @@
     const T* pr = (const T*)&r;
 #pragma unroll
     for (int j = 0; j < VEC; ++j) {
-      float val = (to_f32(pa[j]) - mu[j]) * rs[j] * ga[j] + be[j];
+      float val = bn_affine(to_f32(pa[j]), mu[j], rs[j], ga[j], be[j]);
       if (residual) val += to_f32(pr[j]);
-      if (relu) val = fmaxf(val, 0.f);
-      pa[j] = from_f32<T>(val);
-    }
-    ((uint4*)y)[i] = a;
+      pa[j] = bn_out<T>(val, relu);
+    }
+    ((uint4*)y)[seq_n ? (long long)bn_seq_row(p, seq_n, seq_w) * cv + blockIdx.y * LANES + v : i] = a;
   }
 }
 
 template <typename T>
 __global__ __launch_bounds__(256) void bn_bwd_apply_fused_kernel(
     const T* __restrict__ dy, const T* __restrict__ x, const T* __restrict__ y, const float* __restrict__ mean,
-    const float* __restrict__ rstd, const float* __restrict__ gamma, const double* __restrict__ sums, int ncopy,
-    float* __restrict__ dgamma, float* __restrict__ dbeta, int accumulate, T* __restrict__ dx, T* __restrict__ dres,
-    int relu, int P, int C) {
+    const float* __restrict__ rstd, const float* __restrict__ gamma, const float* __restrict__ beta,
+    const double* __restrict__ sums, int ncopy, float* __restrict__ dgamma, float* __restrict__ dbeta, int accumulate,
+    T* __restrict__ dx, T* __restrict__ dres, int relu, int P, int C, int seq_n, int seq_w) {
   constexpr int VEC = VecOf<T>::N, LANES = 64 / VEC, ROWS = 256 / LANES;
-  __shared__ float s_mean[64], s_k[64], s_rstd[64], s_sb[64], s_sg[64];
+  __shared__ float s_mean[64], s_k[64], s_rstd[64], s_sb[64], s_sg[64], s_gamma[64], s_beta[64];
   const int cbase = blockIdx.y * 64;
   if (threadIdx.x < 64) {
     const int c = cbase + threadIdx.x;
@@ -326,6 +363,8 @@
     s_mean[threadIdx.x] = mean[c];
     s_rstd[threadIdx.x] = rstd[c];
     s_k[threadIdx.x] = gamma[c] * rstd[c];
+    s_gamma[threadIdx.x] = gamma[c];
+    s_beta[threadIdx.x] = relu == BN_RELU_X ? beta[c] : 0.f;
     if (blockIdx.x == 0) {
       dbeta[c] = (accumulate ? dbeta[c] : 0.f) + (float)s1;
       dgamma[c] = (accumulate ? dgamma[c] : 0.f) + (float)s2;
@@ -334,7 +373,7 @@
   __syncthreads();
   const int v = threadIdx.x % LANES, r0 = threadIdx.x / LANES;
   const int cv = C / VEC;
-  float mu[VEC], rs[VEC], kk[VEC], sb[VEC], sg[VEC];
+  float mu[VEC], rs[VEC], kk[VEC], sb[VEC], sg[VEC], ga[VEC], be[VEC];
 #pragma unroll
   for (int j = 0; j < VEC; ++j) {
     mu[j] = s_mean[v * VEC + j];
@@ -342,13 +381,15 @@
     kk[j] = s_k[v * VEC + j];
     sb[j] = s_sb[v * VEC + j];
     sg[j] = s_sg[v * VEC + j];
+    ga[j] = s_gamma[v * VEC + j];
+    be[j] = s_beta[v * VEC + j];
   }
   for (int p = blockIdx.x * ROWS + r0; p < P; p += gridDim.x * ROWS) {
     const long long i = (long long)p * cv + blockIdx.y * LANES + v;
-    uint4 g = ((const uint4*)dy)[i];
+    uint4 g = ((const uint4*)dy)[seq_n ? (long long)bn_seq_row(p, seq_n, seq_w) * cv + blockIdx.y * LANES + v : i];
     uint4 a = ((const uint4*)x)[i];
     uint4 o = make_uint4(0, 0, 0, 0);
-    if (relu) o = ((const uint4*)y)[i];
+    if (relu == BN_RELU_Y) o = ((const uint4*)y)[i];
     T* pg = (T*)&g;
     const T* pa = (const T*)&a;
     const T* po = (const T*)&o;
@@ -357,9 +398,11 @@
 #pragma unroll
     for (int j = 0; j < VEC; ++j) {
       float gv = to_f32(pg[j]);
-      if (relu && !(to_f32(po[j]) > 0.f)) gv = 0.f;
+      const float xf = to_f32(pa[j]);
+      if (relu == BN_RELU_Y && !(to_f32(po[j]) > 0.f)) gv = 0.f;
+      if (relu == BN_RELU_X && !bn_live<T>(xf, mu[j], rs[j], ga[j], be[j])) gv = 0.f;
       pg[j] = from_f32<T>(gv);
-      const float xh = (to_f32(pa[j]) - mu[j]) * rs[j];
+      const float xh = (xf - mu[j]) * rs[j];
       pout[j] = from_f32<T>(kk[j] * (gv - sb[j] - xh * sg[j]));
     }
     ((uint4*)dx)[i] = out;
@@ -367,13 +410,15 @@
   }
 }
 
-template <typename T, int R>
-__global__ __launch_bounds__(256) void bn_bwd_onepass_kernel(
+template <typename T, int R, int RELU, bool SEQ>
+__global__ __launch_bounds__(256, (R > 8 ? 2 : sizeof(T) == 4 ? 4 : 3)) void bn_bwd_onepass_kernel(
     const T* __restrict__ dy, const T* __restrict__ x, const T* __restrict__ y, const float* __restrict__ mean,
-    const float* __restrict__ rstd, const float* __restrict__ gamma, double* __restrict__ sums, int ncopy,
-    unsigned* __restrict__ counters, float* __restrict__ dgamma, float* __restrict__ dbeta, int accumulate,
-    T* __restrict__ dx, T* __restrict__ dres, int relu, int P, int C) {
+    const float* __restrict__ rstd, const float* __restrict__ gamma, const float* __restrict__ beta,
+    double* __restrict__ sums, int ncopy, unsigned* __restrict__ counters, float* __restrict__ dgamma,
+    float* __restrict__ dbeta, int accumulate, T* __restrict__ dx, T* __restrict__ dres, int P, int C, int seq_n,
+    int seq_w) {
   constexpr int VEC = VecOf<T>::N, LANES = 64 / VEC, ROWS = 256 / LANES;
+  constexpr int relu = RELU;
   typedef __attribute__((ext_vector_type(4))) unsigned u32x4;
   __shared__ float red[2][ROWS][64];
   __shared__ float s_sb[64], s_sg[64];
@@ -385,62 +430,79 @@
   const int bytes = (int)((long long)P * C * (long long)sizeof(T));
   const __amdgpu_buffer_rsrc_t r_g = __builtin_amdgcn_make_buffer_rsrc((void*)dy, (short)0, bytes, 0x00020000);
   const __amdgpu_buffer_rsrc_t r_x = __builtin_amdgcn_make_buffer_rsrc((void*)x, (short)0, bytes, 0x00020000);
-  const __amdgpu_buffer_rsrc_t r_y = __builtin_amdgcn_make_buffer_rsrc((void*)(relu ? y : x), (short)0, bytes, 0x00020000);
+  const __amdgpu_buffer_rsrc_t r_y = __builtin_amdgcn_make_buffer_rsrc((void*)(relu == BN_RELU_Y ? y : x), (short)0, bytes, 0x00020000);
   const __amdgpu_buffer_rsrc_t r_dx = __builtin_amdgcn_make_buffer_rsrc((void*)dx, (short)0, bytes, 0x00020000);
   const __amdgpu_buffer_rsrc_t r_dr = __builtin_amdgcn_make_buffer_rsrc((void*)(dres ? dres : dx), (short)0, bytes, 0x00020000);
-  const int voff = (r0 * cv + blockIdx.y * LANES + v) * 16;
   const int row_bytes = cv * 16;
-  const int sbase = blockIdx.x * (ROWS * R) * row_bytes;
-  float mu[VEC], rs[VEC];
-#pragma unroll
-  for (int j = 0; j < VEC; ++j) {
-    mu[j] = mean[cbase + v * VEC + j];
-    rs[j] = rstd[cbase + v * VEC + j];
-  }
+  int off1 = (r0 * cv + blockIdx.y * LANES + v) * 16 + blockIdx.x * (ROWS * R) * row_bytes, off2 = off1;
+  asm volatile("" : "+v"(off1));
+  asm volatile("" : "+v"(off2));
   u32x4 gq[R], xq[R];
 #pragma unroll
   for (int k = 0; k < R; ++k) {
-    gq[k] = __builtin_amdgcn_raw_buffer_load_b128(r_g, voff + sbase + k * ROWS * row_bytes, 0, 0);
-    xq[k] = __builtin_amdgcn_raw_buffer_load_b128(r_x, voff + sbase + k * ROWS * row_bytes, 0, 0);
-  }
-  float s[VEC], q[VEC];
-#pragma unroll
-  for (int j = 0; j < VEC; ++j) s[j] = q[j] = 0.f;
+    int goff = off1 + k * ROWS * row_bytes;
+    if (SEQ) {
+      const int p = blockIdx.x * (ROWS * R) + k * ROWS + r0;
+      goff = p < P ? (bn_seq_row(p, seq_n, seq_w) * cv + blockIdx.y * LANES + v) * 16 : bytes;
+    }
+    gq[k] = __builtin_amdgcn_raw_buffer_load_b128(r_g, goff, 0, 0);
+    xq[k] = __builtin_amdgcn_raw_buffer_load_b128(r_x, off1 + k * ROWS * row_bytes, 0, 0);
+  }
+  constexpr int NP = R > 8 ? 2 : 1, HV = VEC / NP;
   constexpr int RB = R < 4 ? R : 4;
 #pragma unroll
-  for (int kb = 0; kb < R; kb += RB) {
-    u32x4 yq[RB];
-    if (relu) {
-#pragma unroll
-      for (int u = 0; u < RB; ++u)
-        yq[u] = __builtin_amdgcn_raw_buffer_load_b128(r_y, voff + sbase + (kb + u) * ROWS * row_bytes, 0, 0);
-    }
-#pragma unroll
-    for (int u = 0; u < RB; ++u) {
-      const int k = kb + u;
-      T* pg = (T*)&gq[k];
-      const T* pa = (const T*)&xq[k];
-      const T* po = (const T*)&yq[u];
-#pragma unroll
-      for (int j = 0; j < VEC; ++j) {
-        float gd = to_f32(pg[j]);
-        if (relu && !(to_f32(po[j]) > 0.f)) {
-          gd = 0.f;
-          pg[j] = from_f32<T>(0.f);
+  for (int h = 0; h < NP; ++h) {
+    const int cl = v * VEC + h * HV;
+    float s[HV], q[HV], mu[HV], rs[HV], ga[HV], be[HV];
+#pragma unroll
+    for (int j = 0; j < HV; ++j) {
+      s[j] = q[j] = 0.f;
+      mu[j] = mean[cbase + cl + j];
+      rs[j] = rstd[cbase + cl + j];
+      ga[j] = relu == BN_RELU_X ? gamma[cbase + cl + j] : 0.f;
+      be[j] = relu == BN_RELU_X ? beta[cbase + cl + j] : 0.f;
+      asm volatile("" : "+v"(mu[j]), "+v"(rs[j]));
+    }
+#pragma unroll
+    for (int kb = 0; kb < R; kb += RB) {
+      u32x4 yq[RB];
+      if (relu == BN_RELU_Y) {
+#pragma unroll
+        for (int u = 0; u < RB; ++u)
+          yq[u] = __builtin_amdgcn_raw_buffer_load_b128(r_y, off1 + (kb + u) * ROWS * row_bytes, 0, 0);
+      }
+#pragma unroll
+      for (int u = 0; u < RB; ++u) {
+        const int k = kb + u;
+        T* pg = (T*)&gq[k] + h * HV;
+        const T* pa = (const T*)&xq[k] + h * HV;
+        const T* po = (const T*)&yq[u] + h * HV;
+#pragma unroll
+        for (int j = 0; j < HV; ++j) {
+          float gd = to_f32(pg[j]);
+          const float xf = to_f32(pa[j]);
+          bool live = true;
+          if (relu == BN_RELU_Y) live = to_f32(po[j]) > 0.f;
+          if (relu == BN_RELU_X) live = bn_live<T>(xf, mu[j], rs[j], ga[j], be[j]);
+          if (!live) {
+            gd = 0.f;
+            pg[j] = from_f32<T>(0.f);
+          }
+          s[j] += gd;
+          q[j] += gd * (xf - mu[j]) * rs[j];
         }
-        s[j] += gd;
-        q[j] += gd * (to_f32(pa[j]) - mu[j]) * rs[j];
+        if (relu != BN_RELU_NONE) asm volatile("" : "+v"(gq[k]));
+        __builtin_amdgcn_sched_barrier(0);
       }
-      __builtin_amdgcn_sched_barrier(0);
+    }
+#pragma unroll
+    for (int j = 0; j < HV; ++j) {
+      red[0][r0][cl + j] = s[j];
+      red[1][r0][cl + j] = q[j];
     }
   }
 #pragma unroll
   for (int k = 0; k < R; ++k) asm volatile("" : "+v"(gq[k]), "+v"(xq[k]));
-#pragma unroll
-  for (int j = 0; j < VEC; ++j) {
-    red[0][r0][v * VEC + j] = s[j];
-    red[1][r0][v * VEC + j] = q[j];
-  }
   if (tid == 0) s_dead = 0;
   __syncthreads();
   double* mine = sums + (size_t)(blockIdx.x % ncopy) * 2 * C;
@@ -486,27 +548,33 @@
     }
   }
   __syncthreads();
-  float sb[VEC], sg[VEC];
-#pragma unroll
-  for (int j = 0; j < VEC; ++j) {
-    sb[j] = s_sb[v * VEC + j];
-    sg[j] = s_sg[v * VEC + j];
-  }
-#pragma unroll
-  for (int k = 0; k < R; ++k) {
-    const T* pg = (const T*)&gq[k];
-    const T* pa = (const T*)&xq[k];
-    u32x4 out;
-    T* pout = (T*)&out;
-#pragma unroll
-    for (int j = 0; j < VEC; ++j) {
-      const float xh = (to_f32(pa[j]) - mu[j]) * rs[j];
-      const float kj = gamma[cbase + v * VEC + j] * rs[j];
-      pout[j] = from_f32<T>(kj * (to_f32(pg[j]) - sb[j] - xh * sg[j]));
-    }
-    __builtin_amdgcn_raw_buffer_store_b128(out, r_dx, voff + sbase + k * ROWS * row_bytes, 0, 0);
-    if (dres) __builtin_amdgcn_raw_buffer_store_b128(gq[k], r_dr, voff + sbase + k * ROWS * row_bytes, 0, 0);
-    __builtin_amdgcn_sched_barrier(0);
+#pragma unroll
+  for (int h = 0; h < NP; ++h) {
+    const int cl = v * VEC + h * HV;
+    float mu[HV], rs[HV], kj[HV], sb[HV], sg[HV];
+#pragma unroll
+    for (int j = 0; j < HV; ++j) {
+      mu[j] = mean[cbase + cl + j];
+      rs[j] = rstd[cbase + cl + j];
+      kj[j] = gamma[cbase + cl + j] * rs[j];
+      sb[j] = s_sb[cl + j];
+      sg[j] = s_sg[cl + j];
+      asm volatile("" : "+v"(mu[j]), "+v"(rs[j]), "+v"(kj[j]), "+v"(sb[j]), "+v"(sg[j]));
+    }
+#pragma unroll
+    for (int k = 0; k < R; ++k) {
+      if (h == 0 && dres) __builtin_amdgcn_raw_buffer_store_b128(gq[k], r_dr, off2 + k * ROWS * row_bytes, 0, 0);
+      T* pg = (T*)&gq[k] + h * HV;
+      const T* pa = (const T*)&xq[k] + h * HV;
+#pragma unroll
+      for (int j = 0; j < HV; ++j) {
+        const float xh = (to_f32(pa[j]) - mu[j]) * rs[j];
+        pg[j] = from_f32<T>(kj[j] * (to_f32(pg[j]) - sb[j] - xh * sg[j]));
+      }
+      if (h == NP - 1) __builtin_amdgcn_raw_buffer_store_b128(gq[k], r_dx, off2 + k * ROWS * row_bytes, 0, 0);
+      else asm volatile("" : "+v"(gq[k]));
+      __builtin_amdgcn_sched_barrier(0);
+    }
   }
 }
 
@@ -812,21 +880,41 @@
 }
 
 #define g_bn_onepass MR_TUNE(bn_onepass)
+constexpr int BN_ONEPASS_RBIG = 20;
+template <typename T, int R, int RELU, bool SEQ>
 static int bn_onepass_cap() {
   static int cap = -1;
   if (cap >= 0) return cap;
   const int cus = device_cus();
-  int occ_b = 0, occ_f = 0;
+  int occ = 0;
   if (cus == 0 ||
-      hipOccupancyMaxActiveBlocksPerMultiprocessor(&occ_b, bn_bwd_onepass_kernel<bf16_t, 8>, 256, 0) != hipSuccess ||
-      hipOccupancyMaxActiveBlocksPerMultiprocessor(&occ_f, bn_bwd_onepass_kernel<float, 8>, 256, 0) != hipSuccess) {
+      hipOccupancyMaxActiveBlocksPerMultiprocessor(&occ, bn_bwd_onepass_kernel<T, R, RELU, SEQ>, 256, 0) != hipSuccess) {
     (void)hipGetLastError();
     return cap = 0;
   }
-  int occ = occ_b < occ_f ? occ_b : occ_f;
   if (occ > 4) occ = 4;
   cap = occ >= 1 ? cus * occ - cus / 4 : 0;
   return cap;
+}
+template <typename T, int RELU, bool SEQ>
+static void bn_onepass_caps(int& cap8, int& cap_big) {
+  cap8 = bn_onepass_cap<T, 8, RELU, SEQ>();
+  cap_big = 0;
+  if constexpr (RELU != BN_RELU_Y) cap_big = bn_onepass_cap<T, BN_ONEPASS_RBIG, RELU, SEQ>();
+}
+template <typename T, int RELU, bool SEQ>
+static void bn_onepass_launch(int rr, dim3 grid, hipStream_t stream, const void* dy, const void* x, const void* y,
+                              const float* mean, const float* rstd, const float* gamma, const float* beta, double* sums,
+                              unsigned* counters, float* dgamma, float* dbeta, int accumulate, void* dx, void* dres, int P,
+                              int C, int seq_n, int seq_w) {
+#define MR_BN_ONEPASS(R_)                                                                                                   \
+  hipLaunchKernelGGL((bn_bwd_onepass_kernel<T, R_, RELU, SEQ>), grid, dim3(256), 0, stream, (const T*)dy, (const T*)x,      \
+                     (const T*)y, mean, rstd, gamma, beta, sums, MR_BN_COPIES, counters, dgamma, dbeta, accumulate, (T*)dx, \
+                     (T*)dres, P, C, seq_n, seq_w)
+  if (rr == 8) MR_BN_ONEPASS(8);
+  else if (rr == 2) MR_BN_ONEPASS(2);
+  else if constexpr (RELU != BN_RELU_Y) MR_BN_ONEPASS(BN_ONEPASS_RBIG);
+#undef MR_BN_ONEPASS
 }
 
 static inline int grid_for(long long n, int block, int max_blocks = 16384) {
@@ -877,7 +965,8 @@
     const int splits = split_rows_vec((int)P, C / vec, rpb);
     DISPATCH_T(dtype, hipLaunchKernelGGL((bn_reduce_vec_kernel<T, 0>), dim3(splits), dim3(256), 0, stream,
                                          (const T*)x, (const T*)nullptr, (const T*)nullptr, (const float*)nullptr,
-                                         (const float*)nullptr, sums, 0, (int)P, C, rpb, MR_BN_COPIES));
+                                         (const float*)nullptr, (const float*)nullptr, (const float*)nullptr, sums, 0,
+                                         (int)P, C, rpb, MR_BN_COPIES, 0, 0));
   } else {
     const int splits = split_rows((int)P, C, rpb);
     DISPATCH_T(dtype, hipLaunchKernelGGL((bn_stats_kernel<T>), dim3(cdiv(C, 64), splits), dim3(256), 0, stream,
@@ -891,9 +980,19 @@
                     float* running_var, float* save_mean, float* save_rstd, double* sums, const void* residual,
                     int relu, long long P, int C, float eps, float momentum, long long* num_batches_tracked,
                     hipStream_t stream) {
+  return mr_bn_fwd_train_seq(dtype, x, y, gamma, beta, running_mean, running_var, save_mean, save_rstd, sums, residual, relu,
+                             P, C, eps, momentum, num_batches_tracked, 0, stream);
+}
+
+int mr_bn_fwd_train_seq(int dtype, const void* x, void* y, const float* gamma, const float* beta, float* running_mean,
+                        float* running_var, float* save_mean, float* save_rstd, double* sums, const void* residual,
+                        int relu, long long P, int C, float eps, float momentum, long long* num_batches_tracked,
+                        int seq_n, hipStream_t stream) {
   const int vec = dtype == MR_F32 ? 4 : 8;
   MR_CHECK_ARG(C % vec == 0, "mr_bn_fwd_train: C (%d) must be a multiple of %d", C, vec);
   MR_CHECK_ARG(P > 0 && P < (1ll << 31), "mr_bn_fwd_train: bad P");
+  MR_CHECK_ARG(seq_n >= 0 && (seq_n == 0 || (P % seq_n == 0 && x != y)), "mr_bn_fwd_train_seq: bad seq_n %d for P %lld", seq_n, P);
+  const int seq_w = seq_n ? (int)(P / seq_n) : 0;
   const int presum_zero = (relu >> 2) & 1;
   const int have_stats = (relu >> 3) & 1;
   relu &= 1;
@@ -906,7 +1005,8 @@
     ncopy = MR_BN_COPIES;
     DISPATCH_T(dtype, hipLaunchKernelGGL((bn_reduce_vec_kernel<T, 0>), dim3(splits), dim3(256), 0, stream,
                                          (const T*)x, (const T*)nullptr, (const T*)nullptr, (const float*)nullptr,
-                                         (const float*)nullptr, sums, 0, (int)P, C, rpb, ncopy));
+                                         (const float*)nullptr, (const float*)nullptr, (const float*)nullptr, sums, 0,
+                                         (int)P, C, rpb, ncopy, 0, 0));
   } else {
     const int splits = split_rows((int)P, C, rpb);
     DISPATCH_T(dtype, hipLaunchKernelGGL((bn_stats_kernel<T>), dim3(cdiv(C, 64), splits), dim3(256), 0, stream,
@@ -918,7 +1018,7 @@
     DISPATCH_T(dtype, hipLaunchKernelGGL((bn_apply_fused_kernel<T>), grid, dim3(256), 0, stream, (const T*)x, (T*)y,
                                          (const double*)sums, ncopy, eps, momentum, save_mean, save_rstd, running_mean,
                                          running_var, num_batches_tracked, gamma, beta, (const T*)residual, relu,
-                                         (int)P, C));
+                                         (int)P, C, seq_n, seq_w));
     MR_CHECK_LAUNCH();
     return MR_OK;
   }
@@ -926,7 +1026,7 @@
                      eps, momentum, save_mean, save_rstd, running_mean, running_var, num_batches_tracked);
   DISPATCH_T(dtype, hipLaunchKernelGGL((bn_apply_kernel<T>), dim3(grid_for(P * (C / vec), 256)), dim3(256), 0,
                                        stream, (const T*)x, (T*)y, (const float*)save_mean, (const float*)save_rstd,
-                                       gamma, beta, (const T*)residual, relu, P, C));
+                                       gamma, beta, (const T*)residual, relu, P, C, seq_n, seq_w));
   MR_CHECK_LAUNCH();
   return MR_OK;
 }
@@ -940,7 +1040,7 @@
                      tmp_mean, tmp_rstd, C);
   DISPATCH_T(dtype, hipLaunchKernelGGL((bn_apply_kernel<T>), dim3(grid_for(P * (C / vec), 256)), dim3(256), 0,
                                        stream, (const T*)x, (T*)y, (const float*)tmp_mean, (const float*)tmp_rstd,
-                                       gamma, beta, (const T*)residual, relu, P, C));
+                                       gamma, beta, (const T*)residual, relu, P, C, 0, 0));
   MR_CHECK_LAUNCH();
   return MR_OK;
 }
@@ -948,31 +1048,56 @@
 int mr_bn_bwd(int dtype, const void* dy, const void* x, const void* y, const float* gamma, const float* save_mean,
               const float* save_rstd, double* sums, void* dx, void* dres, float* dgamma, float* dbeta, int flags,
               long long P, int C, hipStream_t stream) {
-  const int relu = flags & 1, accumulate = (flags >> 1) & 1, presum_zero = (flags >> 2) & 1;
+  MR_CHECK_ARG(!(flags & 16), "mr_bn_bwd: flags bit 4 (ReLU mask from x) needs beta: mr_bn_bwd_x");
+  return mr_bn_bwd_x(dtype, dy, x, y, gamma, nullptr, save_mean, save_rstd, sums, dx, dres, dgamma, dbeta, flags, P, C, 0,
+                     stream);
+}
+
+int mr_bn_bwd_x(int dtype, const void* dy, const void* x, const void* y, const float* gamma, const float* beta,
+                const float* save_mean, const float* save_rstd, double* sums, void* dx, void* dres, float* dgamma,
+                float* dbeta, int flags, long long P, int C, int seq_n, hipStream_t stream) {
+  const int accumulate = (flags >> 1) & 1, presum_zero = (flags >> 2) & 1;
   const int have_stats = (flags >> 3) & 1;
+  const int prefer_big = (flags >> 5) & 1;
+  const int relu = !(flags & 1) ? BN_RELU_NONE : (flags & 16) ? BN_RELU_X : BN_RELU_Y;
   const int vec = dtype == MR_F32 ? 4 : 8;
   MR_CHECK_ARG(C % vec == 0, "mr_bn_bwd: C (%d) must be a multiple of %d", C, vec);
   MR_CHECK_ARG(P > 0 && P < (1ll << 31), "mr_bn_bwd: bad P");
-  if (!have_stats && g_bn_onepass && C % 64 == 0) {
+  MR_CHECK_ARG(relu != BN_RELU_X || beta, "mr_bn_bwd_x: the ReLU mask from x needs beta");
+  MR_CHECK_ARG(relu != BN_RELU_Y || y, "mr_bn_bwd: the ReLU mask needs y");
+  MR_CHECK_ARG(seq_n >= 0 && (seq_n == 0 || (P % seq_n == 0 && dy != dx && dy != dres)),
+               "mr_bn_bwd_x: bad seq_n %d for P %lld", seq_n, P);
+  const int seq_w = seq_n ? (int)(P / seq_n) : 0;
+  if (!have_stats && g_bn_onepass && C % 64 == 0 && P * C * (dtype == MR_F32 ? 4 : 2) < (1ll << 31)) {
     const int rows = 256 / (64 / vec);
     const int slabs = C / 64;
-    const int cap = bn_onepass_cap();
-    const long long g8 = (P + rows * 8 - 1) / (rows * 8), g2 = (P + rows * 2 - 1) / (rows * 2);
-    const int rr = (g8 * slabs >= 256 || g2 * slabs > cap) ? 8 : 2;
-    const long long gx = rr == 8 ? g8 : g2;
-    if (cap > 0 && gx * slabs <= cap && P * C * (dtype == MR_F32 ? 4 : 2) < (1ll << 31)) {
+    int cap = 0, cap_big = 0;
+#define MR_BN_MODE_(...)                                                                \
+  if (relu == BN_RELU_NONE) { constexpr int RELU = BN_RELU_NONE; __VA_ARGS__; }         \
+  else if (relu == BN_RELU_Y) { constexpr int RELU = BN_RELU_Y; __VA_ARGS__; }          \
+  else { constexpr int RELU = BN_RELU_X; __VA_ARGS__; }
+#define MR_BN_MODE(...)                                                                 \
+  if (seq_n) { constexpr bool SEQ = true; MR_BN_MODE_(__VA_ARGS__) }                    \
+  else { constexpr bool SEQ = false; MR_BN_MODE_(__VA_ARGS__) }
+    DISPATCH_T(dtype, MR_BN_MODE((bn_onepass_caps<T, RELU, SEQ>(cap, cap_big))));
+    const long long gbig = (P + rows * BN_ONEPASS_RBIG - 1) / (rows * BN_ONEPASS_RBIG), g8 = (P + rows * 8 - 1) / (rows * 8),
+                    g2 = (P + rows * 2 - 1) / (rows * 2);
+    int rr = (g8 * slabs >= 256 || g2 * slabs > cap) ? 8 : 2;
+    long long gx = rr == 8 ? g8 : g2;
+    if ((gx * slabs > cap || prefer_big) && gbig * slabs <= cap_big) {
+      rr = BN_ONEPASS_RBIG;
+      gx = gbig;
+      cap = cap_big;
+    }
+    if (cap > 0 && gx * slabs <= cap) {
       unsigned* counters = (unsigned*)(sums + (size_t)2 * C * MR_BN_COPIES);
       if (!presum_zero) (void)hipMemsetAsync(sums, 0, sizeof(double) * (2 * C * MR_BN_COPIES + C), stream);
       const dim3 grid((unsigned)gx, slabs);
-      if (rr == 8) {
-        DISPATCH_T(dtype, hipLaunchKernelGGL((bn_bwd_onepass_kernel<T, 8>), grid, dim3(256), 0, stream, (const T*)dy,
-                                             (const T*)x, (const T*)y, save_mean, save_rstd, gamma, sums, MR_BN_COPIES,
-                                             counters, dgamma, dbeta, accumulate, (T*)dx, (T*)dres, relu, (int)P, C));
-      } else {
-        DISPATCH_T(dtype, hipLaunchKernelGGL((bn_bwd_onepass_kernel<T, 2>), grid, dim3(256), 0, stream, (const T*)dy,
-                                             (const T*)x, (const T*)y, save_mean, save_rstd, gamma, sums, MR_BN_COPIES,
-                                             counters, dgamma, dbeta, accumulate, (T*)dx, (T*)dres, relu, (int)P, C));
-      }
+      DISPATCH_T(dtype, MR_BN_MODE((bn_onepass_launch<T, RELU, SEQ>(rr, grid, stream, dy, x, y, save_mean, save_rstd, gamma, beta,
+                                                               sums, counters, dgamma, dbeta, accumulate, dx, dres, (int)P, C,
+                                                               seq_n, seq_w))));
+#undef MR_BN_MODE
+#undef MR_BN_MODE_
       MR_CHECK_LAUNCH();
       return MR_OK;
     }
@@ -985,20 +1110,20 @@
     const int splits = split_rows_vec((int)P, C / vec, rpb);
     ncopy = MR_BN_COPIES;
     DISPATCH_T(dtype, hipLaunchKernelGGL((bn_reduce_vec_kernel<T, 1>), dim3(splits), dim3(256), 0, stream,
-                                         (const T*)dy, (const T*)x, (const T*)y, save_mean, save_rstd, sums, relu,
-                                         (int)P, C, rpb, ncopy));
+                                         (const T*)dy, (const T*)x, (const T*)y, save_mean, save_rstd, gamma, beta, sums,
+                                         relu, (int)P, C, rpb, ncopy, seq_n, seq_w));
   } else {
     const int splits = split_rows((int)P, C, rpb);
     DISPATCH_T(dtype, hipLaunchKernelGGL((bn_bwd_reduce_kernel<T>), dim3(cdiv(C, 64), splits), dim3(256), 0, stream,
-                                         (const T*)dy, (const T*)x, (const T*)y, save_mean, save_rstd, sums, relu,
-                                         (int)P, C, rpb));
+                                         (const T*)dy, (const T*)x, (const T*)y, save_mean, save_rstd, gamma, beta, sums,
+                                         relu, (int)P, C, rpb, seq_n, seq_w));
   }
   if (g_bn_fused && C % 64 == 0) {
     const int rows = 256 / (64 / vec);
     const dim3 grid(bn_fused_grid_x(P, rows, C / 64), C / 64);
     DISPATCH_T(dtype, hipLaunchKernelGGL((bn_bwd_apply_fused_kernel<T>), grid, dim3(256), 0, stream, (const T*)dy,
-                                         (const T*)x, (const T*)y, save_mean, save_rstd, gamma, (const double*)sums, ncopy,
-                                         dgamma, dbeta, accumulate, (T*)dx, (T*)dres, relu, (int)P, C));
+                                         (const T*)x, (const T*)y, save_mean, save_rstd, gamma, beta, (const double*)sums,
+                                         ncopy, dgamma, dbeta, accumulate, (T*)dx, (T*)dres, relu, (int)P, C, seq_n, seq_w));
     MR_CHECK_LAUNCH();
     return MR_OK;
   }
@@ -1006,8 +1131,8 @@
   hipLaunchKernelGGL(bn_bwd_finalize_kernel, dim3(cdiv(C, 256)), dim3(256), 0, stream, (const double*)sums, ncopy, P, C,
                      sbg, dgamma, dbeta, accumulate);
   DISPATCH_T(dtype, hipLaunchKernelGGL((bn_bwd_apply_kernel<T>), dim3(grid_for(P * (C / vec), 256)), dim3(256), 0,
-                                       stream, (const T*)dy, (const T*)x, (const T*)y, save_mean, save_rstd, gamma,
-                                       (const float*)sbg, (T*)dx, (T*)dres, relu, P, C));
+                                       stream, (const T*)dy, (const T*)x, (const T*)y, save_mean, save_rstd, gamma, beta,
+                                       (const float*)sbg, (T*)dx, (T*)dres, relu, P, C, seq_n, seq_w));
   MR_CHECK_LAUNCH();
   return MR_OK;
 }
diff --git a/megreader_amd/nn/functional.py b/megreader_amd/nn/functional.py
--- a/megreader_amd/nn/functional.py
+++ b/megreader_amd/nn/functional.py
@@ -481,7 +481,7 @@
 class BatchNormFn(Function):
     @staticmethod
     def forward(ctx, x, gamma, beta, running_mean, running_var, training, momentum, eps, relu, residual,
-                num_batches_tracked=None, pre=None, link=None):
+                num_batches_tracked=None, pre=None, link=None, seq=False):
         require_cuda(x, gamma, beta)
         dtype = get_compute_dtype()
         dt = dtype_code(dtype)
@@ -491,7 +491,8 @@
             raise RuntimeError("BatchNorm2d: channel mismatch (%d vs %d)" % (C, gamma.numel()))
         P = N * H * W
         ri = to_internal(residual, dtype) if residual is not None else None
-        y = torch.empty_like(xi)
+        seq_n = N if (seq and training and H == 1 and N > 1 and W > 1 and not (relu and link is not None)) else 0
+        y = torch.empty((W, N, C), dtype=dtype, device=x.device) if seq_n else torch.empty_like(xi)
         mean = torch.empty((C,), dtype=torch.float32, device=x.device)
         rstd = torch.empty((C,), dtype=torch.float32, device=x.device)
         if training:
@@ -505,16 +506,19 @@
                 prezeroed = sums is not None
                 if not prezeroed:
                     sums = torch.empty((nsum,), dtype=torch.float64, device=x.device)
-            call("mr_bn_fwd_train", dt, ptr(xi), ptr(y), ptr(gamma), ptr(beta), ptr(running_mean),
+            call("mr_bn_fwd_train_seq", dt, ptr(xi), ptr(y), ptr(gamma), ptr(beta), ptr(running_mean),
                  ptr(running_var), ptr(mean), ptr(rstd), ptr(sums), ptr(ri),
                  int(relu) | (4 if prezeroed else 0) | (8 if have else 0), P, C, float(eps), float(momentum),
-                 ptr(num_batches_tracked))
+                 ptr(num_batches_tracked), seq_n)
         else:
             call("mr_bn_fwd_eval", dt, ptr(xi), ptr(y), ptr(gamma), ptr(beta), ptr(running_mean), ptr(running_var),
                  ptr(mean), ptr(rstd), ptr(ri), int(relu), P, C, float(eps))
-        ctx.save_for_backward(xi, y if relu else None, gamma, mean, rstd)
+        mask_from_x = bool(relu) and training and residual is None and link is None
+        ctx.save_for_backward(xi, y if (relu and not mask_from_x) else None, gamma, beta, mean, rstd)
         ctx.params = (gamma, beta)
         ctx.relu = relu
+        ctx.mask_from_x = mask_from_x
+        ctx.seq_n = seq_n
         ctx.has_res = residual is not None
         ctx.dtype = dtype
         ctx.training_mode = training
@@ -522,6 +526,8 @@
         if link is not None and training:
             link.xi, link.y, link.mean, link.rstd, link.dtype = xi, (y if relu else None), mean, rstd, dtype
             ctx.bnb_link = link
+        if seq_n:
+            return y.permute(1, 2, 0).unsqueeze(2)
         return y.permute(0, 3, 1, 2)
 
     @staticmethod
@@ -529,10 +535,14 @@
         if not ctx.training_mode:
             raise NotImplementedError("backward through eval-mode BatchNorm is not on the training hot path")
         _no_resident_grids_beside_collectives()
-        xi, y, gamma, mean, rstd = ctx.saved_tensors
+        xi, y, gamma, beta, mean, rstd = ctx.saved_tensors
         dtype = ctx.dtype
         dt = dtype_code(dtype)
-        g = _grad_internal(gy, dtype)
+        seq_n = 0
+        if ctx.seq_n and gy.dtype == dtype and gy.squeeze(2).permute(2, 0, 1).is_contiguous():
+            g, seq_n = gy.squeeze(2).permute(2, 0, 1), ctx.seq_n
+        else:
+            g = _grad_internal(gy, dtype)
         N, H, W, C = xi.shape
         P = N * H * W
         dx = torch.empty_like(xi)
@@ -557,25 +567,26 @@
         else:
             dgamma = torch.empty((C,), dtype=torch.float32, device=g.device)
             dbeta = torch.empty((C,), dtype=torch.float32, device=g.device)
-        call("mr_bn_bwd", dt, ptr(g), ptr(xi), ptr(y), ptr(gamma), ptr(mean), ptr(rstd), ptr(sums), ptr(dx),
+        call("mr_bn_bwd_x", dt, ptr(g), ptr(xi), ptr(y), ptr(gamma), ptr(beta), ptr(mean), ptr(rstd), ptr(sums), ptr(dx),
              ptr(dres), ptr(dgamma), ptr(dbeta),
-             int(ctx.relu) | (2 if sunk else 0) | (4 if prezeroed else 0) | (8 if have else 0), P, C)
+             int(ctx.relu) | (2 if sunk else 0) | (4 if prezeroed else 0) | (8 if have else 0) |
+             (16 if ctx.mask_from_x else 0), P, C, seq_n)
         gres = dres.permute(0, 3, 1, 2) if ctx.has_res else None
         if sunk:
             notify_grad_ready(gamma_p)
             notify_grad_ready(beta_p)
             dgamma = dbeta = None
-        return dx.permute(0, 3, 1, 2), dgamma, dbeta, None, None, None, None, None, None, gres, None, None, None
+        return dx.permute(0, 3, 1, 2), dgamma, dbeta, None, None, None, None, None, None, gres, None, None, None, None
 
 
 def batch_norm(x, gamma, beta, running_mean, running_var, training, momentum, eps, relu=False, residual=None,
-               num_batches_tracked=None):
+               num_batches_tracked=None, sequence_output=False):
     if num_batches_tracked is not None and (num_batches_tracked.dtype != torch.int64 or not training):
         num_batches_tracked = None
     pre = getattr(x, "_mr_bn_sums", None) if training else None
     link = BnBwdLink() if (training and BNB_EPILOGUE and torch.is_grad_enabled() and x.requires_grad) else None
     out = BatchNormFn.apply(x, gamma, beta, running_mean, running_var, bool(training), momentum, eps, bool(relu),
-                            residual, num_batches_tracked, pre, link)
+                            residual, num_batches_tracked, pre, link, bool(sequence_output))
     if link is not None and link.xi is not None:
         out._mr_bnb_link = link
     return out
@@ -866,6 +877,10 @@
 
 
 def map_to_sequence(x):
+    if x.dim() == 4 and x.shape[2] == 1 and x.shape[0] > 1 and x.shape[3] > 1 and x.dtype == get_compute_dtype():
+        seq = x.squeeze(2).permute(2, 0, 1)
+        if seq.is_contiguous():
+            return seq
     return MapToSequenceFn.apply(x)
 
 
diff --git a/megreader_amd/nn/modules.py b/megreader_amd/nn/modules.py
--- a/megreader_amd/nn/modules.py
+++ b/megreader_amd/nn/modules.py
@@ -65,6 +65,7 @@
             raise NotImplementedError("megreader_amd.nn.BatchNorm2d: momentum=None (cumulative moving average) is not "
                                       "used by any reference model; pass a float")
         self.fuse_relu = fuse_relu
+        self.sequence_output = False
 
     def forward(self, x, residual=None):
         momentum = self.momentum
@@ -74,7 +75,7 @@
                 producer.feeds_batch_norm = True
         return F.batch_norm(x, self.weight, self.bias, self.running_mean, self.running_var, self.training, momentum,
                             self.eps, self.fuse_relu, residual,
-                            self.num_batches_tracked if self.training else None)
+                            self.num_batches_tracked if self.training else None, self.sequence_output)
 
 
 class MaxPool2d(nn.MaxPool2d):
```

Measured after the change: 105,800 images/s, median of 6. Within noise of the previous version (+0.7%).
